# go-distributed/gossip_simulator

Hardware: AMD Instinct MI355X
Metric: gossip messages delivered/sec (node) at N=1e9; rounds-to-coverage parity (higher is better)
Workload: dtype u32; 1 GPU; C5-reference-model: single push-flood broadcast per GPU; n=1000000000, fanout=5, fanin=6, delaylow=10, delayhigh=20, ticks=290, status=quiescent, parallelism=trials1

## Files before the change

gossip_simulator_amd/_lib.py:

```python
from __future__ import annotations

import ctypes as C
import os

PKG_DIR = os.path.dirname(os.path.abspath(__file__))
LIB_PATH = os.environ.get("GS_LIB_PATH") or os.path.join(PKG_DIR, "libgossip_hip.so")
CLI_PATH = os.path.join(PKG_DIR, "bin", "gossip_sim")

GS_OK, GS_EINVAL, GS_ELIVELOCK, GS_EREJECT, GS_ENOMEM, GS_EDEVICE, GS_EOVERFLOW = (
    0, -1, -2, -3, -4, -5, -6)
GS_FLAG_TIMING = 1
GS_FLAG_TICK_ENGINE = 2
GS_FLAG_PP_L2_ONLY = 4
GS_FLAG_PP_DENSE = 8
GS_FLAG_PP_EARLY = 16
GS_FLAG_PP_TOPDOWN = 32
GS_FLAG_PP_BOTTOM = 64
GS_FLAG_PP_ANSWER = 128
GS_MODEL_FLOOD, GS_MODEL_PUSHPULL, GS_MODEL_RUMOR = 0, 1, 2
GS_RUMOR_BLIND, GS_RUMOR_COIN, GS_RUMOR_PULL = 1, 2, 4
GS_RUN_COVERED, GS_RUN_QUIESCENT, GS_RUN_MAX_TICKS, GS_RUN_RUNNING = 0, 1, 2, -1
GS_COMM_ID_BYTES = 128

EXPORTS = (
    "gs_version", "gs_strerror", "gs_create", "gs_destroy", "gs_last_error",
    "gs_load_peers", "gs_load_peers_device", "gs_read_peers", "gs_build_overlay",
    "gs_set_failed", "gs_broadcast_begin", "gs_step", "gs_run", "gs_totals",
    "gs_read_received", "gs_read_crashed", "gs_timing_get", "gs_format_float32",
    "gs_format_float64", "gs_format_duration", "gs_threshold", "gs_philox",
    "gs_set_flags", "gs_reset", "gs_set_stream", "gs_create_multi", "gs_comm_unique_id",
    "gs_create_rank", "gs_shard_info", "gs_trial_results", "gs_set_trial",
    "gs_create_rank_exchange", "gs_shard_timing", "gs_trim", "gs_memory_stats",
    "gs_pp_trials_max_n", "gs_pp_trials_max_n_masked", "gs_read_removed",
    "gs_create_trials", "gs_rumor_trials_max_n",
)


class GossipError(RuntimeError):
    def __init__(self, code: int, msg: str):
        super().__init__(f"{msg} [code {code}]")
        self.code = code


class Params(C.Structure):
    _fields_ = [
        ("n", C.c_uint64),
        ("fanout", C.c_int32),
        ("fanin", C.c_int32),
        ("delay_low", C.c_int32),
        ("delay_high", C.c_int32),
        ("drop_rate", C.c_double),
        ("crash_rate", C.c_double),
        ("seed", C.c_uint64),
        ("trial", C.c_uint32),
        ("device", C.c_int32),
        ("flags", C.c_uint32),
        ("model", C.c_uint32),
        ("trials", C.c_uint32),
        ("rumor_k", C.c_uint32),
        ("rumor_mode", C.c_uint32),
        ("reserved32_", C.c_uint32),
        ("reserved_", C.c_uint64 * 4),
    ]


class TickStats(C.Structure):
    _fields_ = [(f, C.c_uint64) for f in
                ("tick", "fired", "sent", "messages", "received", "crashed", "pending")]


class TrialStats(C.Structure):
    _fields_ = [(f, C.c_uint64) for f in
                ("trial", "tick_99", "tick", "fired", "sent", "messages", "received", "crashed")] + \
        [("status", C.c_int32), ("reserved_", C.c_int32)]


class Window(C.Structure):
    _fields_ = [(f, C.c_uint64) for f in ("tick", "makeups", "breakups")]


class Timing(C.Structure):
    _fields_ = [("deliver_ms", C.c_double), ("resolve_ms", C.c_double),
                ("deliver_launches", C.c_uint64), ("resolve_launches", C.c_uint64),
                ("overlay_ms", C.c_double), ("expand_ms", C.c_double),
                ("part_ms", C.c_double), ("windows", C.c_uint64), ("exact_redos", C.c_uint64),
                ("prep_ms", C.c_double),
                ("pp_early_rounds", C.c_uint64), ("pp_bottom_rounds", C.c_uint64),
                ("pp_answer_rounds", C.c_uint64), ("dd_fallbacks", C.c_uint64), ("pp_rev_part", C.c_uint64),
                ("ov_part_ticks", C.c_uint64), ("ov_sort_ticks", C.c_uint64), ("ov_part_fallbacks", C.c_uint64),
                ("alloc_ms", C.c_double), ("largest_alloc_ms", C.c_double), ("free_ms", C.c_double),
                ("alloc_calls", C.c_uint64), ("alloc_cache_hits", C.c_uint64), ("cached_bytes", C.c_uint64),
                ("coarse_redos", C.c_uint64)]


ALL_GATHER_FN = C.CFUNCTYPE(C.c_int, C.c_void_p, C.c_void_p, C.c_void_p, C.c_size_t)
ALL_REDUCE_FN = C.CFUNCTYPE(C.c_int, C.c_void_p, C.POINTER(C.c_uint64), C.c_size_t)


ALL_TO_ALLV_FN = C.CFUNCTYPE(C.c_int, C.c_void_p, C.c_void_p, C.POINTER(C.c_size_t), C.c_void_p,
                             C.POINTER(C.c_size_t))


class Exchange(C.Structure):
    _fields_ = [("user", C.c_void_p), ("all_gather", ALL_GATHER_FN), ("all_reduce_sum_u64", ALL_REDUCE_FN),
                ("all_to_allv", ALL_TO_ALLV_FN)]


_lib = None


def load():
    global _lib
    if _lib is not None:
        return _lib
    if not os.path.exists(LIB_PATH):
        raise OSError(f"{LIB_PATH} is missing: run `python -c 'import __graft_entry__ as g; g.build()'`")
    L = C.CDLL(LIB_PATH)
    P, vp, sz = C.POINTER, C.c_void_p, C.c_size_t
    ctx = vp
    sig = {
        "gs_version": ([], C.c_int),
        "gs_strerror": ([C.c_int], C.c_char_p),
        "gs_create": ([P(Params), P(vp)], C.c_int),
        "gs_create_trials": ([P(Params), P(vp)], C.c_int),
        "gs_destroy": ([ctx], None),
        "gs_last_error": ([ctx], C.c_char_p),
        "gs_load_peers": ([ctx, vp, vp, C.c_uint32], C.c_int),
        "gs_load_peers_device": ([ctx, vp, vp, C.c_uint32], C.c_int),
        "gs_read_peers": ([ctx, vp, vp, P(C.c_uint32)], C.c_int),
        "gs_build_overlay": ([ctx, C.c_uint64, P(Window), sz, P(sz), P(C.c_uint64)], C.c_int),
        "gs_set_failed": ([ctx, vp, sz], C.c_int),
        "gs_broadcast_begin": ([ctx, C.c_int64], C.c_int),
        "gs_step": ([ctx, C.c_uint32, P(TickStats)], C.c_int),
        "gs_run": ([ctx, C.c_uint32, C.c_uint64, P(TickStats), sz, P(sz), P(C.c_int32)], C.c_int),
        "gs_totals": ([ctx, P(TickStats)], C.c_int),
        "gs_read_received": ([ctx, vp, sz], C.c_int),
        "gs_read_crashed": ([ctx, vp, sz], C.c_int),
        "gs_read_removed": ([ctx, vp, sz], C.c_int),
        "gs_timing_get": ([ctx, P(Timing)], C.c_int),
        "gs_shard_timing": ([ctx, C.c_uint32, P(Timing)], C.c_int),
        "gs_format_float32": ([C.c_float, C.c_char_p, sz], sz),
        "gs_format_float64": ([C.c_double, C.c_char_p, sz], sz),
        "gs_format_duration": ([C.c_int64, C.c_char_p, sz], sz),
        "gs_threshold": ([C.c_double], C.c_int32),
        "gs_philox": ([P(C.c_uint32), P(C.c_uint32), P(C.c_uint32)], None),
        "gs_set_flags": ([ctx, C.c_uint32], C.c_int),
        "gs_reset": ([ctx], C.c_int),
        "gs_set_stream": ([ctx, vp], C.c_int),
        "gs_create_multi": ([P(Params), P(C.c_int), C.c_int, P(vp)], C.c_int),
        "gs_comm_unique_id": ([C.c_char_p], C.c_int),
        "gs_create_rank": ([P(Params), C.c_int, C.c_int, C.c_int, C.c_char_p, P(vp)], C.c_int),
        "gs_create_rank_exchange": ([P(Params), C.c_int, C.c_int, C.c_int, P(Exchange), P(vp)], C.c_int),
        "gs_shard_info": ([ctx, C.c_uint32, P(C.c_uint32), P(C.c_uint64), P(C.c_uint64)], C.c_int),
        "gs_trial_results": ([ctx, P(TrialStats), sz, P(sz)], C.c_int),
        "gs_set_trial": ([ctx, C.c_uint32], C.c_int),
        "gs_trim": ([C.c_int, P(sz)], C.c_int),
        "gs_memory_stats": ([P(Timing)], C.c_int),
        "gs_pp_trials_max_n": ([C.c_int, P(C.c_uint64)], C.c_int),
        "gs_pp_trials_max_n_masked": ([C.c_int, P(C.c_uint64)], C.c_int),
        "gs_rumor_trials_max_n": ([C.c_int, C.c_uint32, P(C.c_uint64)], C.c_int),
    }
    for name, (args, res) in sig.items():
        fn = getattr(L, name)
        fn.argtypes = args
        fn.restype = res
    _lib = L
    return L


def format_float32(x: float) -> str:
    b = C.create_string_buffer(64)
    load().gs_format_float32(x, b, 64)
    return b.value.decode()


def format_float64(x: float) -> str:
    b = C.create_string_buffer(64)
    load().gs_format_float64(x, b, 64)
    return b.value.decode()


def format_duration(ns: int) -> str:
    b = C.create_string_buffer(64)
    load().gs_format_duration(ns, b, 64)
    return b.value.decode("utf-8")


def threshold(rate: float) -> int:
    return int(load().gs_threshold(rate))


def philox(ctr, key):
    c = (C.c_uint32 * 4)(*[int(x) & 0xFFFFFFFF for x in ctr])
    k = (C.c_uint32 * 2)(*[int(x) & 0xFFFFFFFF for x in key])
    o = (C.c_uint32 * 4)()
    load().gs_philox(c, k, o)
    return [int(x) for x in o]
```

gossip_simulator_amd/csrc/gs_api.cpp:

```cpp
#include "gs_ctx.h"

using namespace gs;

namespace {

void fill_devmem(gs_timing* out) {
  DevMemStats d;
  gs_devmem_stats(&d);
  out->alloc_ms = d.alloc_ms;
  out->largest_alloc_ms = d.largest_alloc_ms;
  out->free_ms = d.free_ms;
  out->alloc_calls = d.hip_allocs;
  out->alloc_cache_hits = d.cache_hits;
  out->cached_bytes = d.cached_bytes;
}

int is_failed(gs_ctx* c, uint64_t u, bool* out) {
  *out = false;
  if (!c->failed) return GS_OK;
  unsigned long long w = 0;
  CK(c, hipMemcpyAsync(&w, c->st.crash + u / 64, 8, hipMemcpyDeviceToHost, c->stream));
  CK(c, hipStreamSynchronize(c->stream));
  *out = (w >> (u & 63)) & 1;
  return GS_OK;
}

uint64_t keyed_sender(const gs_ctx* c) {
  return uniform(draw0(c->st.key, K_SENDER, 0, 0, 0), (uint32_t)c->p.n);
}

int read_started(gs_ctx* c, const uint32_t* started, uint32_t* count) {
  if (started) CK(c, hipMemcpyAsync(c->bt.h_tstat, started, (size_t)c->trials * 4, hipMemcpyDeviceToHost, c->stream));
  CK(c, hipStreamSynchronize(c->stream));
  *count = 0;
  for (uint32_t t = 0; t < c->trials; ++t) {
    c->tacc[t].start = started ? c->bt.h_tstat[t] : 1;
    *count += (uint32_t)c->tacc[t].start;
  }
  return GS_OK;
}

int begin_one(gs_ctx* c, uint64_t s, uint32_t* sched) {
  *sched = 0;
  CK(c, hipSetDevice(c->dev));
  if (c->trials > 1) {
    uint32_t* started = c->failed ? c->bt.d_tstat : nullptr;
    CK(c, win_schedule(c->ws, (uint32_t)s, 0, c->trials, (uint32_t)c->p.n, c->stream, started));
    RC(read_started(c, started, sched));
    return GS_OK;
  }
  if (s < c->lo || s >= (c->shard ? c->hi : c->p.n)) return GS_OK;
  const uint64_t u = s - c->lo;
  bool dead = false;
  RC(is_failed(c, u, &dead));
  if (dead) return GS_OK;
  if (c->win) CK(c, win_schedule(c->ws, (uint32_t)u, 0, 1, (uint32_t)c->p.n, c->stream));
  else CK(c, launch_schedule_one(c->st, (uint32_t)u, 0, c->stream));
  CK(c, hipStreamSynchronize(c->stream));
  *sched = 1;
  return GS_OK;
}

int read_bits(gs_ctx* c, int which, uint64_t* words, size_t nwords) {
  const uint64_t Wn = (c->p.n + 63) / 64;
  if (c->group && c->gtrials) {
    if (nwords < Wn * c->trials) return fail(c, GS_EINVAL, "need ceil(n/64) words per trial");
    uint64_t off = 0;
    for (gs_ctx* m : c->gr.mem) {
      if (read_bits(m, which, words + off * Wn, nwords - off * Wn)) return fail(c, GS_EINVAL, m->err);
      off += m->trials;
    }
    return GS_OK;
  }
  if (c->group) {
    std::fill(words, words + Wn, 0ull);
    std::vector<uint64_t> tmp(Wn);
    for (gs_ctx* m : c->gr.mem) {
      if (read_bits(m, which, tmp.data(), Wn)) return fail(c, GS_EINVAL, m->err);
      for (uint64_t i = 0; i < Wn; ++i) words[i] |= tmp[i];
    }
    return GS_OK;
  }
  if (nwords < Wn * c->trials) return fail(c, GS_EINVAL, "need ceil(n/64) words per trial");
  CK(c, hipSetDevice(c->dev));
  const unsigned long long* src = which ? c->st.crash : c->st.recv;
  if (c->trials > 1) {
    CK(c, hipMemcpy2DAsync(words, Wn * 8, src, ((size_t)1 << c->tlog) / 8, Wn * 8, c->trials,
                           hipMemcpyDeviceToHost, c->stream));
  } else if (c->shard) {
    std::fill(words, words + Wn, 0ull);
    CK(c, hipMemcpyAsync(words + c->lo / 64, src, c->st.W * 8, hipMemcpyDeviceToHost, c->stream));
  } else {
    CK(c, hipMemcpyAsync(words, src, c->st.W * 8, hipMemcpyDeviceToHost, c->stream));
  }
  CK(c, hipStreamSynchronize(c->stream));
  return GS_OK;
}

}

extern "C" {

int gs_version(void) { return GS_ABI_VERSION; }

const char* gs_strerror(int code) {
  switch (code) {
    case GS_OK: return "ok";
    case GS_EINVAL: return "invalid argument";
    case GS_ELIVELOCK: return "overlay livelock";
    case GS_EREJECT: return "replacement rejection exhausted";
    case GS_ENOMEM: return "out of memory";
    case GS_EDEVICE: return "HIP device error";
    case GS_EOVERFLOW: return "counter overflow";
    default: return "unknown error";
  }
}

const char* gs_last_error(const gs_ctx* c) {
  if (c) return c->err.c_str();
  return g_create_err.empty() ? "NULL context" : g_create_err.c_str();
}

static int pp_trials_limit(int device, bool masked, uint64_t* n_max) {
  g_create_err.clear();
  if (!n_max) return GS_EINVAL;
  *n_max = 0;
  int ndev = 0;
  std::string why;
  const hipError_t ce = hipGetDeviceCount(&ndev);
  if (ce != hipSuccess) {
    why = std::string("hipGetDeviceCount: ") + hipGetErrorString(ce);
  } else if (device < 0 || device >= ndev) {
    why = "device " + std::to_string(device) + " of " + std::to_string(ndev) + " visible";
  } else {
    uint64_t lim = 0;
    why = ppt_limit_error(device, masked, &lim);
    if (why.empty()) {
      *n_max = masked ? ppt_max_n_masked(lim) : ppt_max_n(lim);
      return GS_OK;
    }
  }
  (void)hipGetLastError();
  fprintf(stderr, "%s: %s\n", masked ? "gs_pp_trials_max_n_masked" : "gs_pp_trials_max_n", why.c_str());
  g_create_err = why;
  return GS_EDEVICE;
}

int gs_pp_trials_max_n(int device, uint64_t* n_max) { return pp_trials_limit(device, false, n_max); }

int gs_pp_trials_max_n_masked(int device, uint64_t* n_max) { return pp_trials_limit(device, true, n_max); }

int gs_create(const gs_params* params, gs_ctx** out) {
  g_create_err.clear();
  if (!out) return GS_EINVAL;
  *out = nullptr;
  return create_one(params, params ? params->device : 0, false, 1, 0, out);
}

int gs_create_trials(const gs_params* params, gs_ctx** out) {
  g_create_err.clear();
  if (!out) return GS_EINVAL;
  *out = nullptr;
  return create_one(params, params ? params->device : 0, false, 1, 0, out, true);
}

int gs_rumor_trials_max_n(int device, uint32_t rumor_mode, uint64_t* n_max) {
  g_create_err.clear();
  if (!n_max) return GS_EINVAL;
  *n_max = 0;
  int ndev = 0;
  int rc = GS_EDEVICE;
  std::string why;
  const hipError_t ce = hipGetDeviceCount(&ndev);
  if (rumor_mode & ~(GS_RUMOR_BLIND | GS_RUMOR_COIN | GS_RUMOR_PULL)) {
    why = "rumor_mode " + std::to_string(rumor_mode) + " has a bit that is none of GS_RUMOR_BLIND, GS_RUMOR_COIN, "
          "GS_RUMOR_PULL";
    rc = GS_EINVAL;
  } else if (ce != hipSuccess) {
    why = std::string("hipGetDeviceCount: ") + hipGetErrorString(ce);
  } else if (device < 0 || device >= ndev) {
    why = "device " + std::to_string(device) + " of " + std::to_string(ndev) + " visible";
  } else {
    uint64_t lim = 0;
    why = rmt_limit_error(device, rumor_mode, &lim);
    if (why.empty()) {
      *n_max = rmt_max_n(rumor_mode, lim);
      return GS_OK;
    }
  }
  (void)hipGetLastError();
  fprintf(stderr, "gs_rumor_trials_max_n: %s\n", why.c_str());
  g_create_err = why;
  return rc;
}

int gs_create_multi(const gs_params* params, const int* devices, int ndev, gs_ctx** out) {
  g_create_err.clear();
  if (!out || !params || !devices || ndev < 1) return GS_EINVAL;
  *out = nullptr;
  return create_multi(params, devices, ndev, out);
}

int gs_comm_unique_id(uint8_t id[GS_COMM_ID_BYTES]) {
  if (!id) return GS_EINVAL;
  const Rccl& r = rccl();
  if (!r.ok) {
    fprintf(stderr, "gs_comm_unique_id: %s\n", r.why.c_str());
    return GS_EDEVICE;
  }
  ncclUniqueId u;
  if (r.get_unique_id(&u) != ncclSuccess) return GS_EDEVICE;
  static_assert(sizeof(ncclUniqueId) == GS_COMM_ID_BYTES, "RCCL unique id size");
  memcpy(id, &u, GS_COMM_ID_BYTES);
  return GS_OK;
}

int gs_create_rank(const gs_params* params, int device, int nranks, int rank, const uint8_t* id, gs_ctx** out) {
  g_create_err.clear();
  if (!out || !params || nranks < 1 || rank < 0 || rank >= nranks) return GS_EINVAL;
  *out = nullptr;
  RC(rumor_refuse(params, "gs_create_rank"));
  const uint32_t T = std::max<uint32_t>(1, params->trials);
  if (T > 1) {
    gs_params mp = *params;
    const uint32_t t0 = (uint32_t)((uint64_t)T * rank / nranks), t1 = (uint32_t)((uint64_t)T * (rank + 1) / nranks);
    if (t1 == t0) {
      fprintf(stderr, "gs_create_rank: %u trials leave rank %d none\n", T, rank);
      return GS_EINVAL;
    }
    mp.trial = params->trial + t0;
    mp.trials = t1 - t0;
    return create_one(&mp, device, false, 1, 0, out);
  }
  if (!id) return GS_EINVAL;
  const Rccl& r = rccl();
  if (!r.ok) {
    fprintf(stderr, "gs_create_rank: %s\n", r.why.c_str());
    return GS_EDEVICE;
  }
  gs_ctx* c = nullptr;
  int rc = create_one(params, device, true, (uint32_t)nranks, (uint32_t)rank, &c);
  if (rc) return rc;
  ncclUniqueId u;
  memcpy(&u, id, GS_COMM_ID_BYTES);
  (void)hipSetDevice(device);
  ncclResult_t nr = r.comm_init_rank(&c->xc.comm, nranks, u, rank);
  if (nr != ncclSuccess) {
    fprintf(stderr, "gs_create_rank: ncclCommInitRank: %s\n", rccl_error((int)nr).c_str());
    c->xc.comm = nullptr;
    destroy_one(c);
    return GS_EDEVICE;
  }
  return finish_rank(c, out);
}

int gs_create_rank_exchange(const gs_params* params, int device, int nranks, int rank, const gs_exchange* ex,
                            gs_ctx** out) {
  g_create_err.clear();
  if (!out || !params || !ex || !ex->all_gather || !ex->all_reduce_sum_u64 || nranks < 1 || rank < 0 ||
      rank >= nranks)
    return GS_EINVAL;
  RC(rumor_refuse(params, "gs_create_rank_exchange"));
  if (params->model == GS_MODEL_FLOOD && std::max<uint32_t>(1, params->trials) == 1 && !ex->all_to_allv) {
    fprintf(stderr, "gs_create_rank_exchange: flood shards need the all_to_allv callback\n");
    return GS_EINVAL;
  }
  *out = nullptr;
  if (std::max<uint32_t>(1, params->trials) > 1) return gs_create_rank(params, device, nranks, rank, nullptr, out);
  gs_ctx* c = nullptr;
  int rc = create_one(params, device, true, (uint32_t)nranks, (uint32_t)rank, &c);
  if (rc) return rc;
  c->xc.hx = *ex;
  c->xc.has_hx = true;
  return finish_rank(c, out);
}

int gs_shard_info(const gs_ctx* c, uint32_t index, uint32_t* nshards, uint64_t* lo, uint64_t* hi) {
  if (!c) return GS_EINVAL;
  const bool sg = c->group && !c->gtrials;
  const uint32_t ns = sg ? (uint32_t)c->gr.mem.size() : c->shard ? c->G : 1u;
  if (nshards) *nshards = ns;
  if (index >= ns) return GS_EINVAL;
  const gs_ctx* s = sg ? c->gr.mem[0] : c;
  uint64_t a = 0, b = c->p.n;
  if (s->shard) {
    a = std::min<uint64_t>(index * s->seg_per, c->p.n);
    b = std::min<uint64_t>(a + s->seg_per, c->p.n);
  }
  if (lo) *lo = a;
  if (hi) *hi = b;
  return GS_OK;
}

void gs_destroy(gs_ctx* c) { destroy_one(c); }

int gs_load_peers(gs_ctx* c, const uint8_t* deg, const uint32_t* ids, uint32_t stride) {
  if (!c || !deg || !ids || stride == 0 || stride > 255) return fail(c, GS_EINVAL, "bad peer table");
  if (c->begun) return fail(c, GS_EINVAL, "peers must be loaded before gs_broadcast_begin");
  if (c->group && c->gtrials) {
    uint64_t off = 0;
    for (gs_ctx* m : c->gr.mem) {
      RC(gs_load_peers(m, deg + off * c->p.n, ids + off * c->p.n * stride, stride) ? fail(c, GS_EINVAL, m->err) : 0);
      off += m->trials;
    }
    c->peers = true;
    return GS_OK;
  }
  if (c->group) {
    for (size_t d = 0; d < c->gr.devs.size(); ++d) {
      std::vector<gs_ctx*> ms = on_device(c, d);
      int rc = upload_table(ms[0], deg, ids, stride);
      if (!rc) rc = seal_rows(ms[0], ms[0]->d_deg, ms[0]->d_ids, c->p.n);
      if (!rc) rc = partition_from(ms[0], ms);
      if (rc) return fail(c, rc, ms[0]->err);
    }
    c->peers = true;
    return GS_OK;
  }
  RC(upload_table(c, deg, ids, stride));
  RC(seal_rows(c, c->d_deg, c->d_ids, table_n(c)));
  if (c->shard) RC(partition_from(c, {c}));
  c->peers = true;
  return GS_OK;
}

int gs_load_peers_device(gs_ctx* c, const void* d_deg, const void* d_ids, uint32_t stride) {
  if (!c || !d_deg || !d_ids || stride < 2 || stride > 255)
    return fail(c, GS_EINVAL, "bad device peer table (stride must be in [2,255])");
  if (c->begun) return fail(c, GS_EINVAL, "peers must be loaded before gs_broadcast_begin");
  if (c->group || c->trials > 1)
    return fail(c, GS_EINVAL, "device tables load into one-device, one-trial contexts");
  CK(c, hipSetDevice(c->dev));
  c->row_slots = 0;
  RC(alloc_table(c, stride));
  const uint64_t n = table_n(c);
  CK(c, hipMemcpyAsync(c->d_deg, d_deg, n, hipMemcpyDeviceToDevice, c->stream));
  CK(c, hipMemcpyAsync(c->d_ids, d_ids, n * stride * 4ull, hipMemcpyDeviceToDevice, c->stream));
  RC(validate_table(c, c->d_deg, c->d_ids, n, c->p.n));
  RC(seal_rows(c, c->d_deg, c->d_ids, n));
  if (c->shard) RC(partition_from(c, {c}));
  c->peers = true;
  return GS_OK;
}

int gs_read_peers(gs_ctx* c, uint8_t* deg, uint32_t* ids, uint32_t* stride_out) {
  if (!c || !c->peers) return fail(c, GS_EINVAL, "no peer table");
  if (c->group && c->gtrials) {
    uint32_t s = 0;
    uint64_t off = 0;
    for (gs_ctx* m : c->gr.mem) {
      if (gs_read_peers(m, deg ? deg + off * c->p.n : nullptr, nullptr, &s)) return fail(c, GS_EINVAL, m->err);
      if (ids && gs_read_peers(m, nullptr, ids + off * c->p.n * s, &s)) return fail(c, GS_EINVAL, m->err);
      off += m->trials;
    }
    if (stride_out) *stride_out = s;
    return GS_OK;
  }
  if (c->group || c->shard)
    return fail(c, GS_EINVAL, "a sharded context keeps only its partition of the table");
  const uint32_t S = c->st.stride, So = c->row_slots && c->row_slots < S ? c->row_slots : S;
  if (stride_out) *stride_out = So;
  CK(c, hipSetDevice(c->dev));
  if (c->trials > 1) {
    const uint64_t np = c->p.n, per = 1ull << c->tlog;
    std::vector<uint8_t> hd(c->ntot);
    std::vector<uint32_t> hi;
    CK(c, hipMemcpyAsync(hd.data(), c->d_deg, c->ntot, hipMemcpyDeviceToHost, c->stream));
    if (ids) {
      hi.resize(c->ntot * S);
      CK(c, hipMemcpyAsync(hi.data(), c->d_ids, c->ntot * S * 4ull, hipMemcpyDeviceToHost, c->stream));
    }
    CK(c, hipStreamSynchronize(c->stream));
    for (uint32_t t = 0; t < c->trials; ++t)
      for (uint64_t v = 0; v < np; ++v) {
        const uint64_t src = t * per + v, dst = t * np + v;
        if (deg) deg[dst] = hd[src];
        if (ids)
          for (uint32_t j = 0; j < So; ++j) {
            const uint32_t x = hi[src * S + j];
            ids[dst * So + j] = x == kEmptyMsg ? x : (x & ((uint32_t)per - 1));
          }
      }
    return GS_OK;
  }
  if (deg) CK(c, hipMemcpyAsync(deg, c->d_deg, c->p.n, hipMemcpyDeviceToHost, c->stream));
  if (ids && So == S) CK(c, hipMemcpyAsync(ids, c->d_ids, c->p.n * S * 4ull, hipMemcpyDeviceToHost, c->stream));
  if (ids && So != S)
    CK(c, hipMemcpy2DAsync(ids, So * 4ull, c->d_ids, S * 4ull, So * 4ull, c->p.n, hipMemcpyDeviceToHost, c->stream));
  CK(c, hipStreamSynchronize(c->stream));
  return GS_OK;
}

int gs_build_overlay(gs_ctx* c, uint64_t max_ticks, gs_window* win, size_t cap, size_t* nwin,
                     uint64_t* final_tick) {
  if (!c) return GS_EINVAL;
  if (c->begun) return fail(c, GS_EINVAL, "overlay must be built before gs_broadcast_begin");
  if (c->group && c->gtrials) {
    std::vector<uint64_t> ft(c->gr.mem.size(), 0);
    std::vector<size_t> nw(c->gr.mem.size(), 0);
    RC(par_members(c, [&](gs_ctx* m, size_t i) {
      return gs_build_overlay(m, max_ticks, i == 0 ? win : nullptr, i == 0 ? cap : 0, &nw[i], &ft[i]);
    }));
    if (nwin) *nwin = nw[0];
    if (final_tick) *final_tick = *std::max_element(ft.begin(), ft.end());
    c->timing.overlay_ms = c->gr.mem[0]->timing.overlay_ms;
    c->peers = true;
    return GS_OK;
  }
  if (c->group) {
    for (size_t d = 0; d < c->gr.devs.size(); ++d) {
      std::vector<gs_ctx*> ms = on_device(c, d);
      int rc = overlay_into(ms[0], max_ticks, d == 0 ? win : nullptr, d == 0 ? cap : 0,
                            d == 0 ? nwin : nullptr, d == 0 ? final_tick : nullptr);
      if (!rc) rc = partition_from(ms[0], ms);
      if (rc) return fail(c, rc, ms[0]->err);
    }
    c->timing.overlay_ms = c->gr.mem[0]->timing.overlay_ms;
    c->peers = true;
    return GS_OK;
  }
  RC(overlay_into(c, max_ticks, win, cap, nwin, final_tick));
  if (c->shard) RC(partition_from(c, {c}));
  c->peers = true;
  return GS_OK;
}

int gs_set_failed(gs_ctx* c, const uint64_t* words, size_t nwords) { return set_failed(c, words, nwords); }


int gs_broadcast_begin(gs_ctx* c, int64_t sender) {
  if (!c) return GS_EINVAL;
  if (c->aborted) return fail(c, GS_EDEVICE, "this rank's exchange failed earlier; the run is over");
  if (!c->peers) return fail(c, GS_EINVAL, "load peers or build the overlay first");
  if (c->begun) return fail(c, GS_EINVAL, "broadcast already begun");
  if (sender >= 0 && (uint64_t)sender >= c->p.n) return fail(c, GS_EINVAL, "sender out of range");
  reset_counters(c);
  if (c->group && c->gtrials) {
    for (gs_ctx* m : c->gr.mem) {
      if (gs_broadcast_begin(m, sender)) return fail(c, GS_EINVAL, m->err);
      c->recv += m->recv;
      c->pending += m->pending;
    }
    c->begun = true;
    return GS_OK;
  }
  const bool batched = c->trials > 1;
  const uint64_t s = sender >= 0 ? (uint64_t)sender : batched ? ~0ull : keyed_sender(c->group ? c->gr.mem[0] : c);
  if (c->ppt) {
    CK(c, hipSetDevice(c->dev));
    uint32_t* started = c->failed ? c->bt.d_tstat : nullptr;
    uint32_t k = 0;
    CK(c, ppt_seed(c->pt, (uint32_t)s, started, c->stream));
    RC(read_started(c, started, &k));
    for (TrialAcc& a : c->tacc) a.recv = a.start;
    c->recv = c->pending = k;
    c->begun = true;
    return GS_OK;
  }
  if (c->rumor) return rumor_begin(c, s);
  if (c->pp && (c->group || c->pp_shard)) return pp_shard_begin(c, s);
  if (c->pp) {
    CK(c, hipSetDevice(c->dev));
    RC(pp_prepare(c));
    const uint64_t n = c->st.n;
    const unsigned long long thr = (c->p.flags & GS_FLAG_PP_EARLY) ? n : (n >> pp_shift());
    RC(pp_seed_ctx(c, c->d_next, (uint32_t)s, thr, pp_bottom_thr(c), pp_answer_thr(c)));
    uint32_t ok = 0;
    CK(c, hipMemcpyAsync(&ok, c->d_flag, 4, hipMemcpyDeviceToHost, c->stream));
    CK(c, hipStreamSynchronize(c->stream));
    c->recv = c->pending = ok;
    c->begun = true;
    return GS_OK;
  }
  unsigned long long scheduled = 0;
  if (c->group) {
    for (gs_ctx* m : c->gr.mem) {
      reset_counters(m);
      uint32_t k = 0;
      if (int rc = begin_one(m, s, &k)) return fail(c, rc, m->err);
      scheduled += k;
      m->begun = true;
    }
  } else {
    uint32_t k = 0;
    RC(begin_one(c, s, &k));
    scheduled = k;
    if (is_rank(c)) RC(rank_sum(c, &scheduled));
  }
  c->pending = scheduled;
  for (TrialAcc& a : c->tacc) a.sched = 0;
  c->begun = true;
  return GS_OK;
}

int gs_set_stream(gs_ctx* c, void* hip_stream) {
  if (!c) return GS_EINVAL;
  if (c->group || is_rank(c)) return fail(c, GS_EINVAL, "multi-device contexts keep their own streams");
  CK(c, hipSetDevice(c->dev));
  CK(c, hipStreamSynchronize(c->stream));
  c->stream = hip_stream ? (hipStream_t)hip_stream : c->own;
  return GS_OK;
}

int gs_memory_stats(gs_timing* out) {
  if (!out) return GS_EINVAL;
  *out = gs_timing{};
  fill_devmem(out);
  return GS_OK;
}

int gs_trim(int device, size_t* released) {
  const size_t b = gs_devmem_trim(device);
  if (released) *released = b;
  return GS_OK;
}

int gs_step(gs_ctx* c, uint32_t ticks, gs_tick_stats* out) {
  if (!c) return GS_EINVAL;
  if (c->aborted) return fail(c, GS_EDEVICE, "this rank's exchange failed earlier; the run is over");
  if (!c->begun) return fail(c, GS_EINVAL, "gs_broadcast_begin first");
  if (c->group && c->gtrials) {
    std::vector<std::vector<gs_tick_stats>> rows(c->gr.mem.size(), std::vector<gs_tick_stats>(ticks));
    RC(par_members(c, [&](gs_ctx* m, size_t i) {
      return gs_step(m, ticks, rows[i].data());
    }));
    std::vector<unsigned long long> s(kStatFields);
    for (uint32_t k = 0; k < ticks; ++k) {
      std::fill(s.begin(), s.end(), 0ull);
      uint64_t pend = 0;
      for (auto& r : rows) {
        s[ST_FIRED] += r[k].fired;
        s[ST_SENT] += r[k].sent;
        s[ST_MSGS] += r[k].messages;
        pend += r[k].pending;
      }
      uint64_t recv = 0, cr = 0;
      for (auto& r : rows) { recv += r[k].received; cr += r[k].crashed; }
      c->t = rows[0][k].tick;
      c->fired += s[ST_FIRED]; c->sent += s[ST_SENT]; c->msgs += s[ST_MSGS];
      c->recv = recv; c->crashed = cr; c->pending = pend;
      if (out) out[k] = gs_tick_stats{c->t, s[ST_FIRED], s[ST_SENT], s[ST_MSGS], recv, cr, pend};
    }
    return GS_OK;
  }
  if (c->rumor) return rumor_step(c, ticks, out, true);
  if (c->pp && (c->group || c->pp_shard)) return pp_shard_step(c, ticks, out);
  if (c->group) return shard_step(c, c->gr.mem, ticks, out);
  if (c->shard) return abort_rank(c, shard_step(c, {c}, ticks, out));
  if (c->ppt) return ppt_step(c, ticks, out);
  return plain_step(c, ticks, out);
}

int gs_run(gs_ctx* c, uint32_t poll, uint64_t max_ticks, gs_tick_stats* out, size_t cap,
           size_t* nout, int32_t* status) {
  if (!c || poll == 0) return fail(c, GS_EINVAL, "poll must be >= 1");
  if (c->group && c->gtrials) {
    std::vector<int32_t> sts(c->gr.mem.size(), 0);
    RC(par_members(c, [&](gs_ctx* m, size_t i) {
      return gs_run(m, poll, max_ticks, nullptr, 0, nullptr, &sts[i]);
    }));
    gs_tick_stats tot{};
    uint64_t recv = 0, cr = 0, t = 0, pend = 0;
    c->fired = c->sent = c->msgs = 0;
    for (gs_ctx* m : c->gr.mem) {
      c->fired += m->fired; c->sent += m->sent; c->msgs += m->msgs;
      recv += m->recv; cr += m->crashed; pend += m->pending; t = std::max(t, m->t);
    }
    c->t = t; c->recv = recv; c->crashed = cr; c->pending = pend;
    tot = gs_tick_stats{t, c->fired, c->sent, c->msgs, recv, cr, pend};
    if (out && cap) out[0] = tot;
    if (nout) *nout = 1;
    if (status) *status = *std::max_element(sts.begin(), sts.end());
    return GS_OK;
  }
  if (c->rumor) return rumor_run(c, poll, max_ticks, out, cap, nout, status);
  size_t k = 0;
  int32_t st = GS_RUN_MAX_TICKS;
  const bool trials = c->trials > 1 && !c->group;
  const bool flood = !c->pp;
  const uint64_t pbase = c->t;
  uint64_t f0 = c->fired, s0 = c->sent, m0 = c->msgs;
  std::function<int(const OnTick&, uint32_t*, bool*)> dd;
  std::vector<gs_ctx*> ms;
  if (!c->pp && !c->gtrials && (c->group || c->shard) && dd_ok(c, shards_of(c))) {
    if (c->aborted) return fail(c, GS_EDEVICE, "this rank's exchange failed earlier; the run is over");
    if (!c->begun) return fail(c, GS_EINVAL, "gs_broadcast_begin first");
    ms = shards_of(c);
    for (gs_ctx* m : ms) {
      CK(m, hipSetDevice(m->dev));
      RC(expand_view(m));
    }
    dd = [&](const OnTick& on_tick, uint32_t* stop, bool* fallback) {
      const int rc = dd_run(c, ms, ~0ull, poll, max_ticks, on_tick, stop, fallback);
      return c->group ? rc : abort_rank(c, rc);
    };
  } else if (async_ok(c)) {
    dd = [&](const OnTick& on_tick, uint32_t* stop, bool* fallback) {
      return run_async(c, ~0ull, poll, max_ticks, on_tick, stop, fallback);
    };
  }
  if (dd) {
    uint32_t stop = 0;
    bool fallback = false;
    RC(dd(
        [&](uint64_t tick, const unsigned long long* row) {
          account_tick(c, tick, row, nullptr);
          if ((tick - pbase) % poll) return;
          if (out && k < cap)
            out[k] = gs_tick_stats{c->t, c->fired - f0, c->sent - s0, c->msgs - m0, c->recv, c->crashed, c->pending};
          ++k;
          f0 = c->fired; s0 = c->sent; m0 = c->msgs;
        },
        &stop, &fallback));
    if (!fallback) {
      st = stop ? (int32_t)stop - 1 : GS_RUN_MAX_TICKS;
      if (c->tacc.size() == 1) snap_trial(c, 0, st);
      if (nout) *nout = k;
      if (status) *status = st;
      return GS_OK;
    }
  }
  std::vector<uint64_t> tr0;
  for (;;) {
    const uint64_t r0 = c->recv;
    if (trials && c->ppt) {
      tr0.resize(c->trials);
      for (uint32_t tr = 0; tr < c->trials; ++tr) tr0[tr] = c->tacc[tr].recv;
    }
    RC(gs_step(c, (uint32_t)(poll - (c->t - pbase) % poll), nullptr));
    if (out && k < cap)
      out[k] = gs_tick_stats{c->t, c->fired - f0, c->sent - s0, c->msgs - m0, c->recv, c->crashed, c->pending};
    ++k;
    f0 = c->fired; s0 = c->sent; m0 = c->msgs;
    if (trials && c->ppt) {
      uint32_t running = 0;
      RC(ppt_poll_stops(c, tr0, max_ticks, &running));
      if (trials_stopped(c, running, &st)) break;
      continue;
    }
    if (trials) {
      uint32_t running = 0;
      for (uint32_t tr = 0; tr < c->trials; ++tr) {
        TrialAcc& a = c->tacc[tr];
        if (a.status != GS_RUN_RUNNING) continue;
        const uint64_t pend = a.start + a.sched - a.fired;
        if (covered(a.recv, c->p.n)) snap_trial(c, tr, GS_RUN_COVERED);
        else if (pend == 0) snap_trial(c, tr, GS_RUN_QUIESCENT);
        else if (c->t >= max_ticks) snap_trial(c, tr, GS_RUN_MAX_TICKS);
        else ++running;
      }
      if (trials_stopped(c, running, &st)) break;
      continue;
    }
    if (covered(c->recv, c->p.n)) { st = GS_RUN_COVERED; break; }
    if (flood && c->pending == 0) { st = GS_RUN_QUIESCENT; break; }
    if (!flood && c->recv == r0) {
      bool stalled = false;
      RC(pp_stalled(c, &stalled));
      if (stalled) { st = GS_RUN_QUIESCENT; break; }
    }
    if (c->t >= max_ticks) { st = GS_RUN_MAX_TICKS; break; }
  }
  if (!trials && c->tacc.size() == 1) snap_trial(c, 0, st);
  if (nout) *nout = k;
  if (status) *status = st;
  return GS_OK;
}

int gs_trial_results(gs_ctx* c, gs_trial_stats* out, size_t cap, size_t* nout) {
  if (!c) return GS_EINVAL;
  size_t k = 0;
  auto one = [&](const gs_ctx* x) {
    for (size_t i = 0; i < x->tacc.size(); ++i, ++k) {
      if (!out || k >= cap) continue;
      const TrialAcc& a = x->tacc[i];
      if (a.status != GS_RUN_RUNNING) {
        out[k] = a.snap;
      } else {
        out[k] = gs_trial_stats{(uint64_t)x->p.trial + i, a.tick99, x->t, a.fired, a.sent, a.msgs, a.recv,
                                a.crash, GS_RUN_RUNNING, 0};
      }
    }
  };
  if (c->group && c->gtrials) for (gs_ctx* m : c->gr.mem) one(m);
  else one(c);
  if (nout) *nout = k;
  return GS_OK;
}

int gs_totals(gs_ctx* c, gs_tick_stats* out) {
  if (!c || !out) return GS_EINVAL;
  *out = gs_tick_stats{c->t, c->fired, c->sent, c->msgs, c->recv, c->crashed, c->pending};
  return GS_OK;
}

int gs_read_received(gs_ctx* c, uint64_t* words, size_t nwords) {
  if (!c || !words || nwords < (c->p.n + 63) / 64) return fail(c, GS_EINVAL, "need ceil(n/64) words");
  return read_bits(c, 0, words, nwords);
}

int gs_read_crashed(gs_ctx* c, uint64_t* words, size_t nwords) {
  if (!c || !words || nwords < (c->p.n + 63) / 64) return fail(c, GS_EINVAL, "need ceil(n/64) words");
  return read_bits(c, 1, words, nwords);
}

int gs_read_removed(gs_ctx* c, uint64_t* words, size_t nwords) {
  if (!c) return GS_EINVAL;
  return rumor_read_removed(c, words, nwords);
}

int gs_timing_get(gs_ctx* c, gs_timing* out) {
  if (!c || !out) return GS_EINVAL;
  *out = c->group ? c->gr.mem[0]->timing : c->timing;
  if (c->group) out->overlay_ms = c->timing.overlay_ms;
  out->pp_early_rounds = out->pp_bottom_rounds = out->pp_answer_rounds = 0;
  gs_ctx* pc = c->group ? c->gr.mem[0] : c;
  if (c->pp && pc->sp.ctl && c->begun) {
    CK(pc, hipSetDevice(pc->dev));
    PPCtl h;
    CK(pc, hipMemcpyAsync(&h, pc->sp.ctl, offsetof(PPCtl, segcnt), hipMemcpyDeviceToHost, pc->stream));
    CK(pc, hipStreamSynchronize(pc->stream));
    out->pp_early_rounds = h.nearly;
    out->pp_bottom_rounds = h.nbottom;
    out->pp_answer_rounds = h.nanswer;
  }
  if (c->pp && c->begun) out->pp_early_rounds += c->rs.rep_rounds;
  fill_devmem(out);
  return GS_OK;
}

int gs_shard_timing(gs_ctx* c, uint32_t index, gs_timing* out) {
  if (!c || !out) return GS_EINVAL;
  if (!c->group) return index == 0 ? gs_timing_get(c, out) : fail(c, GS_EINVAL, "no such shard");
  if (index >= c->gr.mem.size()) return fail(c, GS_EINVAL, "no such shard");
  *out = c->gr.mem[index]->timing;
  fill_devmem(out);
  return GS_OK;
}

int gs_set_trial(gs_ctx* c, uint32_t trial) {
  if (!c) return GS_EINVAL;
  if (c->begun) return fail(c, GS_EINVAL, "gs_reset before gs_set_trial");
  if (c->group) {
    uint32_t t = trial;
    for (gs_ctx* m : c->gr.mem) {
      RC(gs_set_trial(m, c->gtrials ? t : trial) ? fail(c, GS_EINVAL, m->err) : 0);
      t += m->trials;
    }
    c->p.trial = trial;
    c->peers = false;
    return GS_OK;
  }
  c->p.trial = trial;
  c->st.key.trial = trial;
  c->ws.key.trial = trial;
  c->pt.key.trial = trial;
  c->peers = false;
  reset_counters(c);
  return GS_OK;
}

int gs_set_flags(gs_ctx* c, uint32_t flags) {
  if (!c) return GS_EINVAL;
  c->p.flags = flags;
  for (gs_ctx* m : c->gr.mem) m->p.flags = flags;
  return GS_OK;
}

int gs_reset(gs_ctx* c) {
  if (!c) return GS_EINVAL;
  for (gs_ctx* m : c->gr.mem) RC(gs_reset(m) ? fail(c, GS_EDEVICE, m->err) : 0);
  if (!c->group) {
    CK(c, hipSetDevice(c->dev));
    CK(c, hipMemsetAsync(c->d_state, 0, (char*)c->st.stats - (char*)c->d_state, c->stream));
    if (c->d_err) CK(c, hipMemsetAsync(c->d_err, 0, 4, c->stream));
    if (c->d_cnt) CK(c, hipMemsetAsync(c->d_cnt, 0, c->st.n * 4, c->stream));
    if (c->win) CK(c, hipMemsetAsync(c->ws.fcount, 0, c->wn.fcount_bytes, c->stream));
    if (c->failed && !c->pp_shard)
      CK(c, hipMemcpyAsync(c->st.crash, c->d_failed, c->st.W * 8, hipMemcpyDeviceToDevice, c->stream));
    if (c->pp_shard)
      CK(c, hipMemsetAsync(c->st.recv, 0, c->st.W * 8, c->stream));
    CK(c, hipStreamSynchronize(c->stream));
  }
  reset_counters(c);
  c->begun = false;
  return GS_OK;
}

void gs_philox(const uint32_t ctr[4], const uint32_t key[2], uint32_t out[4]) {
  const u32x4 r = philox(ctr[0], ctr[1], ctr[2], ctr[3], key[0], key[1]);
  out[0] = r.x; out[1] = r.y; out[2] = r.z; out[3] = r.w;
}

}
```

gossip_simulator_amd/csrc/gs_ctx.cpp:

```cpp
#include "gs_ctx.h"

namespace gs {

namespace {

uint32_t ring_slots(const gs_params& p) { return p.delay_high > 2 ? (uint32_t)p.delay_high : 2u; }

uint32_t ceil_log2(uint64_t x) {
  uint32_t b = 0;
  while ((1ull << b) < x) ++b;
  return b;
}

int check_params(const gs_params* p, bool rumor_trials, std::string& why) {
  if (!p) { why = "params is NULL"; return GS_EINVAL; }
  if (p->n == 0) { why = "n must be >= 1 (simulator.go:240 panics on rand.Intn(0))"; return GS_EINVAL; }
  if (p->n > 0x7FFFFFFFull) { why = "n must be < 2^31"; return GS_EINVAL; }
  if (p->delay_high <= p->delay_low) {
    why = "delayhigh must exceed delaylow (simulator.go:167 panics on rand.Intn(<=0))";
    return GS_EINVAL;
  }
  if (p->fanout < 0 || p->fanin < 0 || p->fanout > 255 || p->fanin > 255) {
    why = "fanout/fanin must be in [0, 255]";
    return GS_EINVAL;
  }
  if (ring_slots(*p) > 4096) { why = "delayhigh must be <= 4096"; return GS_EINVAL; }
  if (p->model > GS_MODEL_RUMOR) {
    why = "model must be GS_MODEL_FLOOD, GS_MODEL_PUSHPULL or GS_MODEL_RUMOR";
    return GS_EINVAL;
  }
  if (p->model == GS_MODEL_RUMOR && (p->rumor_k < 1 || p->rumor_k > 255)) {
    why = "GS_MODEL_RUMOR needs 1 <= rumor_k <= 255, not " + std::to_string(p->rumor_k);
    return GS_EINVAL;
  }
  if (p->model == GS_MODEL_RUMOR && (p->rumor_mode & ~(GS_RUMOR_BLIND | GS_RUMOR_COIN | GS_RUMOR_PULL))) {
    why = "GS_MODEL_RUMOR: rumor_mode " + std::to_string(p->rumor_mode) +
          " has a bit that is none of GS_RUMOR_BLIND, GS_RUMOR_COIN, GS_RUMOR_PULL";
    return GS_EINVAL;
  }
  if (p->model == GS_MODEL_RUMOR && p->trials > 1 && !rumor_trials) {
    why = "GS_MODEL_RUMOR with trials > 1: the rumor model runs one trial per context (gs_create_trials makes a batch)";
    return GS_EINVAL;
  }
  if (p->trials > 1 && ((uint64_t)p->trials << std::max<uint32_t>(kFineLog, ceil_log2(p->n))) > 0x7FFFFFFFull) {
    why = "trials x 2^ceil(log2 n) must be < 2^31 (batch fewer trials per context)";
    return GS_EINVAL;
  }
  return GS_OK;
}

bool alloc_trial_rows(gs_ctx* c, size_t tb, size_t cb) {
  return dev_malloc((void**)&c->bt.d_tstat, tb) == hipSuccess &&
         hipHostMalloc((void**)&c->bt.h_tstat, tb) == hipSuccess && grow(c->bt.chk, cb);
}

void release_trials(gs_ctx* c) {
  if (c->bt.d_tstat) (void)dev_free(c->bt.d_tstat);
  if (c->bt.h_tstat) (void)hipHostFree(c->bt.h_tstat);
  release(c->bt.chk);
}

int alloc_window(gs_ctx* c) {
  const DevState& s = c->st;
  WinState& w = c->ws;
  w.n = s.n;
  w.W = s.W;
  w.nfine = (uint32_t)((s.n + kFineNodes - 1) >> kFineLog);
  w.ncoarse = (w.nfine + 255) / 256;
  w.R = s.R;
  w.delay_low = s.delay_low;
  w.delay_span = s.delay_span;
  w.kd = s.kd;
  w.kc = s.kc;
  w.key = s.key;
  w.base = (uint32_t)c->lo;
  w.tlog = c->tlog;
  w.tmask = c->tlog >= 32 ? ~0u : (1u << c->tlog) - 1;
  w.tnodes = c->trials > 1 && c->tlog <= kCoarseShift && !c->shard ? (uint32_t)c->p.n : 0u;
  w.G = c->G;
  w.rank = c->rank;
  w.seg_per = (uint32_t)c->seg_per;
  w.csub = kCoarseSub;
  w.noxcd = getenv("GS_PART2_NOXCD") ? 1u : 0u;
  {
    const char* xp = getenv("GS_XPAIR");
    w.nopair = xp && atoi(xp) == 0 ? 1u : 0u;
  }
  w.ccap_end = nullptr;
  w.csrc = nullptr;
  if (c->shard) {
    w.owner = 1;
    w.obins = 256 / c->G;
    w.oseg_q = (uint32_t)(c->seg_per >> kFineLog);
    w.oseg_magic = 0xFFFFFFFFu / w.oseg_q;
    if (dev_malloc(&c->wn.d_rtab, kRtabWords * 8) != hipSuccess ||
        hipHostMalloc((void**)&c->wn.h_rtab, kRtabWords * 8) != hipSuccess)
      return fail(c, GS_ENOMEM, "cannot allocate the shard's receive layout");
  }
  auto al = [](size_t b) { return (b + 255) & ~(size_t)255; };
  const size_t units = (size_t)kMaxWindow * w.nfine + 1;
  const size_t b_fc = al((size_t)w.R * w.nfine * 4), b_units = al(units * 8),
               b_small = al(kRegions * 8) * 2 + al((kRegions + 1) * 8) + al((kRegions + 1) * 4) + al(kMaxWindow * 8),
               b_fhist = al(((size_t)w.ncoarse * 256 + 1) * 8), b_fbase = al(((size_t)w.nfine + 1) * 8),
               b_ffill = al((size_t)w.nfine * 8),
               b_sst = al((size_t)kStatShards * kMaxWindow * kStatFields * 8),
               b_rlcnt = al((size_t)w.nfine * 4),
               b_tsum = al((size_t)w.ncoarse * kMaxWindow * 8) + al(((size_t)w.ncoarse + 1) * 8);
  const size_t total = b_fc + 2 * b_units + b_small + b_fhist + b_fbase + b_ffill + b_sst + b_rlcnt + b_tsum;
  if (dev_malloc(&c->wn.d_win, total) != hipSuccess)
    return fail(c, GS_ENOMEM, "cannot allocate window-engine buffers");
  const size_t flist = (size_t)w.R * w.nfine * kFineNodes * 2;
  if (dev_malloc(&c->wn.d_flist, flist) != hipSuccess)
    return fail(c, GS_ENOMEM, "cannot allocate " + std::to_string(flist >> 20) + " MiB of fire lists");
  char* q = (char*)c->wn.d_win;
  w.fcount = (uint32_t*)q; q += b_fc;
  w.usize = (unsigned long long*)q; q += b_units;
  w.unit_off = (unsigned long long*)q; q += b_units;
  w.chist = (unsigned long long*)q; q += al(kRegions * 8);
  w.cfill = (unsigned long long*)q; q += al(kRegions * 8);
  w.ccap = (unsigned long long*)q; q += al((kRegions + 1) * 8);
  w.tprefix = (uint32_t*)q; q += al((kRegions + 1) * 4);
  w.tfires = (unsigned long long*)q;
  q = (char*)c->wn.d_win + b_fc + 2 * b_units + b_small;
  w.fhist = (unsigned long long*)q; q += b_fhist;
  w.fstart = (unsigned long long*)q; q += b_fbase;
  w.ffill = (unsigned long long*)q; q += b_ffill;
  w.sstats = (unsigned long long*)q; q += b_sst;
  w.rlcnt = (uint32_t*)q; q += b_rlcnt;
  w.tsum = (unsigned long long*)q; q += al((size_t)w.ncoarse * kMaxWindow * 8);
  w.toff = (unsigned long long*)q; q += al(((size_t)w.ncoarse + 1) * 8);
  if (dev_malloc(&c->wn.d_rlmsg, (size_t)w.nfine * kRolledCap * 4) != hipSuccess)
    return fail(c, GS_ENOMEM, "cannot allocate the rolled-receipt lists");
  w.rlmsg = (uint32_t*)c->wn.d_rlmsg;
  w.dbg = nullptr;
  if (getenv("GS_STAMPS") && dev_malloc(&w.dbg, kDbgWords * 8) == hipSuccess)
    (void)hipMemset(w.dbg, 0, kDbgWords * 8);
  w.flist = (uint16_t*)c->wn.d_flist;
  c->wn.fcount_bytes = (size_t)w.R * w.nfine * 4;
  if (hipMemsetAsync(c->wn.d_win, 0, total, c->stream) != hipSuccess)
    return fail(c, GS_EDEVICE, "memset of window buffers failed");
  c->wn.misc_words = std::max<size_t>(4096, (size_t)c->G * kMaxWindow + 64);
  if (hipHostMalloc((void**)&c->wn.h_cap, (kRegions + 1) * 8) != hipSuccess ||
      hipHostMalloc((void**)&c->wn.h_misc, c->wn.misc_words * 8) != hipSuccess ||
      hipHostMalloc((void**)&c->wn.h_err, 64) != hipSuccess)
    return fail(c, GS_ENOMEM, "cannot allocate pinned window buffers");
  if (c->trials > 1) {
    if (!alloc_trial_rows(c, (size_t)c->trials * kMaxWindow * kTStatFields * 4, 0))
      return fail(c, GS_ENOMEM, "cannot allocate per-trial counters");
    w.tstat = c->bt.d_tstat;
  }
  return GS_OK;
}

void release_window(gs_ctx* c) {
  WinEngine& e = c->wn;
  for (void* p : {e.d_win, e.d_flist, e.d_rlmsg, (void*)e.d_rtab, (void*)c->ws.dbg})
    if (p) (void)dev_free(p);
  for (Buf* b : {&e.gmap, &e.cmsg, &e.fmsg, &e.tmp}) release(*b);
  for (void* p : {(void*)e.h_cap, (void*)e.h_misc, (void*)e.h_err, (void*)e.h_rtab})
    if (p) (void)hipHostFree(p);
}

int ctx_setup(gs_ctx* c, const gs_params* params, int device, bool shard, uint32_t G, uint32_t rank,
              std::string& why) {
  c->p = *params;
  c->p.device = device;
  c->dev = device;
  int ndev = 0;
  if (hipGetDeviceCount(&ndev) != hipSuccess || ndev <= 0) {
    why = "no HIP device visible (libgossip_hip needs an MI355X)";
    return GS_EDEVICE;
  }
  if (c->dev < 0 || c->dev >= ndev) {
    why = "device " + std::to_string(c->dev) + " out of range (" + std::to_string(ndev) + " visible)";
    return GS_EDEVICE;
  }
  hipDeviceProp_t prop;
  if (hipSetDevice(c->dev) != hipSuccess || hipGetDeviceProperties(&prop, c->dev) != hipSuccess ||
      strncmp(prop.gcnArchName, "gfx950", 6) != 0) {
    why = "device " + std::to_string(c->dev) + " is not gfx950";
    return GS_EDEVICE;
  }
  if (hipStreamCreateWithFlags(&c->own, hipStreamNonBlocking) != hipSuccess) {
    why = "cannot create a stream";
    return GS_EDEVICE;
  }
  c->stream = c->own;
  DevState& s = c->st;
  const uint32_t stride0 = (uint32_t)std::max(c->p.fanout, c->p.fanin);
  c->pp = c->p.model == GS_MODEL_PUSHPULL;
  c->rumor = c->p.model == GS_MODEL_RUMOR;
  c->pp_l2_only = (c->p.flags & GS_FLAG_PP_L2_ONLY) != 0;
  c->trials = std::max<uint32_t>(1, c->p.trials);
  c->ntot = c->p.n;
  if (c->trials > 1) {
    c->tlog = std::max<uint32_t>(kFineLog, ceil_log2(c->p.n));
    c->ntot = (uint64_t)c->trials << c->tlog;
  }
  c->shard = shard;
  c->G = G;
  c->rank = rank;
  if (shard && c->rumor) {
    why = "GS_MODEL_RUMOR runs on one device: no node-range shards";
    return GS_EINVAL;
  }
  if (shard) {
    if (c->pp && !pp_rslot_packed(stride0)) {
      why = "push-pull node-range shards need rows of at most 16 slots (bottom-up rounds)";
      return GS_EINVAL;
    }
    c->seg_per = (((c->p.n + G - 1) / G) + kFineNodes - 1) & ~(uint64_t)(kFineNodes - 1);
    if ((uint64_t)(G - 1) * c->seg_per >= c->p.n) {
      why = "n = " + std::to_string(c->p.n) + " is too small for " + std::to_string(G) +
            " shards of whole 16384-node buckets";
      return GS_EINVAL;
    }
    c->pp_shard = c->pp;
    c->rs.segw = c->seg_per / 64;
    c->lo = rank * c->seg_per;
    c->hi = std::min<uint64_t>(c->lo + c->seg_per, c->p.n);
    c->ntot = c->hi - c->lo;
  }
  s.lo = 0;
  s.hi = (uint32_t)c->ntot;
  s.n = c->ntot;
  s.W = (s.n + 63) / 64;
  s.C = (uint32_t)((s.n + (1ull << kChunkNodesLog) - 1) >> kChunkNodesLog);
  s.CS = (s.C + kShards - 1) / kShards;
  s.chunk_lo = 0;
  s.chunk_hi = s.C;
  s.sharded = 0;
  s.R = ring_slots(c->p);
  s.delay_low = c->p.delay_low;
  s.delay_span = (uint32_t)(c->p.delay_high - c->p.delay_low);
  s.kd = gs_threshold(c->p.drop_rate);
  s.kc = gs_threshold(c->p.crash_rate);
  s.key = Key{(uint32_t)c->p.seed, (uint32_t)(c->p.seed >> 32), c->p.trial};
  c->win = !c->pp && !c->rumor && s.R <= kWinMaxRing && !(c->p.flags & GS_FLAG_TICK_ENGINE) && stride0 <= kWinMaxStride &&
           s.n <= (1ull << (kCoarseShift + 8));
  if (((c->trials > 1 && !c->ppt && !c->rmt) || (shard && !c->pp)) && !c->win) {
    why = "batched trials and node-range shards run on the window engine (delayhigh <= 256, "
          "fanout/fanin <= 32, no GS_FLAG_TICK_ENGINE, at most 2^30 nodes per context or shard)";
    return GS_EINVAL;
  }
  static_assert(kSrcShift + 8 == 64, "8-bit source index in the receive layout");
  if (shard && !c->pp && (G > 255 || ((c->seg_per + (1ull << kCoarseShift) - 1) >> kCoarseShift) > 256 / G)) {
    why = "flood node-range shards: each of the G <= 255 shards' ranges must fit 256 / G bins of 2^22 nodes "
          "(n up to about 2^30)";
    return GS_EINVAL;
  }
  auto al = [](size_t b) { return (b + 255) & ~(size_t)255; };
  const bool tick = !c->win && !c->pp && !c->rumor;
  const size_t b_sum = c->pp && !c->ppt ? al(pp_summary_total_words(s.W) * 8) : 0;
  const size_t b_next = (c->pp && !c->ppt) || (c->rumor && !c->rmt) ? al(s.W * 8) + b_sum : 0;
  const size_t b_bits = al(s.W * 8), b_ring = tick ? al((size_t)s.R * s.W * 8) : 0,
               b_cflag = tick ? al((size_t)s.R * s.C * 4) : 0,
               b_clist = tick ? al((size_t)s.R * kShards * s.CS * 4) : 0,
               b_ccount = tick ? al((size_t)s.R * kShards * kCounterStride * 4) : 0,
               b_stats = al((size_t)kStatSlots * kStatFields * 8);
  const size_t b_roll = c->win ? b_bits : 0;
  const size_t total = 2 * b_bits + b_roll + b_next + b_ring + b_cflag + b_clist + b_ccount + b_stats + 256;
  c->state_bytes = total;
  if (dev_malloc(&c->d_state, total) != hipSuccess) {
    why = "cannot allocate " + std::to_string(total) + " bytes of device state";
    return GS_ENOMEM;
  }
  char* q = (char*)c->d_state;
  s.recv = (unsigned long long*)q; q += b_bits;
  s.crash = (unsigned long long*)q; q += b_bits;
  s.rollw = b_roll ? (uint32_t*)q : nullptr; q += b_roll;
  c->d_next = b_next ? (unsigned long long*)q : nullptr;
  c->d_ppsum = b_sum ? (unsigned long long*)(q + al(s.W * 8)) : nullptr;
  q += b_next;
  s.ring = (unsigned long long*)q; q += b_ring;
  s.cflag = (uint32_t*)q; q += b_cflag;
  s.clist = (uint32_t*)q; q += b_clist;
  s.ccount = (uint32_t*)q; q += b_ccount;
  s.stats = (unsigned long long*)q; q += b_stats;
  c->d_err = (uint32_t*)q;
  c->d_flag = c->d_err + 1;
  s.err = c->d_err;
  s.grecv = s.recv;
  s.gcrash = s.crash;
  s.gbase = 0;
  if (tick && s.kc > 0 && dev_malloc(&c->d_cnt, s.n * 4) != hipSuccess) {
    why = "cannot allocate arrival counters";
    return GS_ENOMEM;
  }
  s.cnt = c->d_cnt;
  if (c->win) {
    int rc = alloc_window(c);
    if (rc) { why = c->err; return rc; }
  }
  if (c->rumor) {
    int rc = rumor_alloc(c);
    if (rc) { why = c->err; return rc; }
  }
  if (c->ppt) {
    const size_t tb = (size_t)c->trials * kMaxWindow * kTStatFields * 4;
    const size_t cb = (((size_t)c->trials + 3) & ~(size_t)3) + (size_t)c->trials * 4;
    if (!alloc_trial_rows(c, tb, cb)) {
      why = "cannot allocate the per-trial counters";
      return GS_ENOMEM;
    }
    PptState& pt = c->pt;
    pt.recv = s.recv;
    pt.tstat = c->bt.d_tstat;
    pt.n = (uint32_t)c->p.n;
    pt.trials = c->trials;
    pt.tlog = c->tlog;
    pt.kd = s.kd;
    pt.key = s.key;
  }
  if (c->rmt && !alloc_trial_rows(c, (size_t)c->trials * kMaxWindow * kTStatFields * 4, 0)) {
    why = "cannot allocate the per-trial counters";
    return GS_ENOMEM;
  }
  c->tacc.assign(c->trials, TrialAcc{});
  c->async_off = getenv("GS_SYNC_WINDOWS") != nullptr;
  c->winlog = getenv("GS_WINLOG") != nullptr;
  if (hipMemsetAsync(c->d_state, 0, total, c->stream) != hipSuccess ||
      (c->d_cnt && hipMemsetAsync(c->d_cnt, 0, s.n * 4, c->stream) != hipSuccess) ||
      hipHostMalloc((void**)&c->h_stats, (size_t)kStatSlots * kStatFields * 8) != hipSuccess ||
      hipStreamSynchronize(c->stream) != hipSuccess) {
    why = "device initialisation failed";
    return GS_EDEVICE;
  }
  return GS_OK;
}

void release_state(gs_ctx* c) {
  for (void* p : {c->d_state, (void*)c->d_cnt, (void*)c->d_failed})
    if (p) (void)dev_free(p);
  if (c->h_stats) (void)hipHostFree(c->h_stats);
}

int check_ppt_n(const gs_params* p, int device, std::string& why, PptPlan* pl) {
  *pl = PptPlan{};
  if (p->trials <= 1 || p->model != GS_MODEL_PUSHPULL) return GS_OK;
  int ndev = 0;
  uint64_t lim = 0;
  const bool asked = hipGetDeviceCount(&ndev) == hipSuccess && device >= 0 && device < ndev &&
                     ppt_lds_limit(device, false, &lim) == hipSuccess;
  if (!asked) {
    (void)hipGetLastError();
    why = "batched push-pull trials need n within the device's LDS per workgroup (gs_pp_trials_max_n), and HIP "
          "device " + std::to_string(device) + " is not visible: n = " + std::to_string(p->n) + " is not accepted";
    return GS_EINVAL;
  }
  const PptPlan plan = ppt_plan(p->n, lim);
  if (!plan.fits) {
    why = "batched push-pull trials keep a trial's informed set in one workgroup's LDS: n must be <= " +
          std::to_string(ppt_max_n(lim)) + " on this device (gs_pp_trials_max_n), not " + std::to_string(p->n);
    return GS_EINVAL;
  }
  if (plan.lds_bytes > 65536 && ppt_prepare(device, false, (uint32_t)plan.lds_bytes) != hipSuccess) {
    why = "cannot raise the trial-resident kernel's dynamic LDS limit";
    return GS_EDEVICE;
  }
  *pl = plan;
  return GS_OK;
}

void attach_pp_sets(gs_ctx* c, unsigned long long* ig, unsigned long long* fg, unsigned long long* gn) {
  c->rs.d_ig = ig;
  c->rs.d_fg = fg;
  c->rs.d_gn = gn;
  DevState& s = c->st;
  s.grecv = ig;
  s.gcrash = fg;
  s.gbase = c->lo;
  s.recv = ig + (size_t)c->rank * c->rs.segw;
  s.crash = fg + (size_t)c->rank * c->rs.segw;
}

int alloc_pp_sets(gs_ctx* c, uint64_t words, unsigned long long** ig, unsigned long long** fg,
                  unsigned long long** gn) {
  for (unsigned long long** q : {ig, fg, gn}) {
    if (!q) continue;
    *q = nullptr;
    if (dev_malloc(q, words * 8) != hipSuccess)
      return fail(c, GS_ENOMEM, "cannot allocate the replicated informed / failed sets");
    CK(c, hipMemsetAsync(*q, 0, words * 8, c->stream));
  }
  CK(c, hipStreamSynchronize(c->stream));
  return GS_OK;
}

void release_sets(gs_ctx* c) {
  if (!c->rs.own_ig) return;
  for (unsigned long long* q : {c->rs.d_ig, c->rs.d_fg, c->rs.d_gn, c->rs.d_gst})
    if (q) (void)dev_free(q);
}

int make_replica(const gs_params* params, int dev, unsigned long long* ig, unsigned long long* fg, gs_ctx** out) {
  *out = nullptr;
  if (getenv("GS_PP_NO_REPLICA")) return GS_OK;
  gs_params rp = *params;
  rp.trials = 1;
  gs_ctx* r = nullptr;
  RC(create_one(&rp, dev, false, 1, 0, &r));
  r->st.recv = r->st.grecv = ig;
  r->st.crash = r->st.gcrash = fg;
  r->st.gbase = 0;
  *out = r;
  return GS_OK;
}

void print_stamps(gs_ctx* c) {
  if (!c->ws.dbg) return;
  unsigned long long h[kDbgWords];
  if (hipMemcpy(h, c->ws.dbg, sizeof h, hipMemcpyDeviceToHost) == hipSuccess && h[kXStamp0]) {
    const double r = 1e-3 / h[kXStamp0];
    fprintf(stderr, "[stamps] k_expand: %llu rounds (wave 0), mean kcycles per round: lookup %.2f rows %.2f "
            "draws %.2f scan+scatter %.2f barrier %.2f writeout %.2f\n", h[kXStamp0], h[kXStamp0 + 1] * r,
            h[kXStamp0 + 2] * r, h[kXStamp0 + 3] * r, h[kXStamp0 + 4] * r, h[kXStamp0 + 5] * r, h[kXStamp0 + 6] * r);
  }
  if (hipMemcpy(h, c->ws.dbg, sizeof h, hipMemcpyDeviceToHost) == hipSuccess)
    for (int cls = 0; cls < 2; ++cls) {
      const unsigned long long* d = h + cls * kStampPhases;
      if (!d[0]) continue;
      fprintf(stderr, "[stamps] k_resolve %s: %llu buckets, mean kcycles per bucket per phase:",
              cls ? "M>=1024" : "M<1024", d[0]);
      for (uint32_t i = 1; i < kStampPhases; ++i) fprintf(stderr, " %.2f", d[i] * 1e-3 / d[0]);
      fprintf(stderr, "\n");
    }
}

void release_group(gs_ctx* g) {
  Group& r = g->gr;
  for (size_t i = 0; i < r.devs.size(); ++i) {
    (void)hipSetDevice(r.devs[i]);
    if (i < r.buf.size()) release(r.buf[i]);
    for (auto* sets : {&r.ig, &r.fg, &r.gn})
      if (i < sets->size() && (*sets)[i]) (void)dev_free((*sets)[i]);
  }
  for (hipEvent_t e : r.ev_c) (void)hipEventDestroy(e);
  for (hipEvent_t e : r.ev_x) (void)hipEventDestroy(e);
  for (gs_ctx* rep : r.reps) destroy_one(rep);
  if (!r.devs.empty()) (void)hipSetDevice(r.devs[0]);
}

void release_exchange(gs_ctx* c) {
  Exchange& x = c->xc;
  if (x.d_gcounts) (void)dev_free(x.d_gcounts);
  if (x.d_glay) (void)dev_free(x.d_glay);
  if (x.h_glay) (void)hipHostFree(x.h_glay);
  release(x.xsend);
  release(x.xrecv);
  if (x.h_xbuf) (void)hipHostFree(x.h_xbuf);
}

}

int finish_rank(gs_ctx* c, gs_ctx** out) {
  (void)hipSetDevice(c->dev);
  if (dev_malloc(&c->xc.d_gcounts, (size_t)c->G * kMaxWindow * 8 + (size_t)kMaxWindow * 8) != hipSuccess ||
      (!c->pp_shard && (dev_malloc(&c->xc.d_glay, (size_t)c->G * (kRegions + 1) * 8) != hipSuccess ||
                        hipHostMalloc((void**)&c->xc.h_glay, (size_t)c->G * (kRegions + 1) * 8) != hipSuccess))) {
    destroy_one(c);
    return GS_ENOMEM;
  }
  if (c->pp_shard) {
    unsigned long long *ig = nullptr, *fg = nullptr, *gn = nullptr, *gst = nullptr;
    if (alloc_pp_sets(c, (uint64_t)c->G * c->rs.segw, &ig, &fg, &gn) ||
        alloc_pp_sets(c, (uint64_t)c->G * c->rs.segw, &gst, nullptr, nullptr)) {
      fprintf(stderr, "gs_create_rank: %s\n", c->err.c_str());
      for (unsigned long long* q : {ig, fg, gn, gst})
        if (q) (void)dev_free(q);
      destroy_one(c);
      return GS_ENOMEM;
    }
    c->rs.own_ig = true;
    c->rs.d_gst = gst;
    attach_pp_sets(c, ig, fg, gn);
    if (make_replica(&c->p, c->dev, ig, fg, &c->rs.rep)) {
      destroy_one(c);
      return GS_ENOMEM;
    }
    c->rs.own_rep = c->rs.rep != nullptr;
  }
  *out = c;
  return GS_OK;
}

int create_multi(const gs_params* params, const int* devices, int ndev, gs_ctx** out) {
  RC(rumor_refuse(params, "gs_create_multi"));
  gs_ctx* g = new gs_ctx();
  g->group = true;
  g->p = *params;
  g->dev = devices[0];
  g->trials = std::max<uint32_t>(1, params->trials);
  g->gtrials = g->trials > 1;
  if (g->gtrials && (uint32_t)ndev > g->trials) ndev = (int)g->trials;
  for (int i = 0; i < ndev; ++i) {
    gs_params mp = *params;
    gs_ctx* m = nullptr;
    int rc;
    if (g->gtrials) {
      const uint32_t t0 = (uint32_t)((uint64_t)g->trials * i / ndev), t1 = (uint32_t)((uint64_t)g->trials * (i + 1) / ndev);
      mp.trial = params->trial + t0;
      mp.trials = t1 - t0;
      rc = create_one(&mp, devices[i], false, 1, 0, &m);
    } else {
      rc = create_one(&mp, devices[i], true, (uint32_t)ndev, (uint32_t)i, &m);
    }
    if (rc) {
      destroy_one(g);
      return rc;
    }
    g->gr.mem.push_back(m);
    auto it = std::find(g->gr.devs.begin(), g->gr.devs.end(), devices[i]);
    if (it == g->gr.devs.end()) {
      g->gr.devs.push_back(devices[i]);
      g->gr.dev_of.push_back((int)g->gr.devs.size() - 1);
    } else {
      g->gr.dev_of.push_back((int)(it - g->gr.devs.begin()));
    }
  }
  g->gr.buf.resize(g->gr.devs.size());
  g->pp = params->model == GS_MODEL_PUSHPULL;
  if (g->pp && !g->gtrials) {
    g->gr.ig.assign(g->gr.devs.size(), nullptr);
    g->gr.fg.assign(g->gr.devs.size(), nullptr);
    g->gr.gn.assign(g->gr.devs.size(), nullptr);
    for (size_t d = 0; d < g->gr.devs.size(); ++d) {
      std::vector<gs_ctx*> ms;
      for (size_t i = 0; i < g->gr.mem.size(); ++i)
        if ((size_t)g->gr.dev_of[i] == d) ms.push_back(g->gr.mem[i]);
      (void)hipSetDevice(g->gr.devs[d]);
      if (alloc_pp_sets(ms[0], (uint64_t)g->gr.mem.size() * ms[0]->rs.segw, &g->gr.ig[d], &g->gr.fg[d], &g->gr.gn[d])) {
        fprintf(stderr, "gs_create_multi: %s\n", ms[0]->err.c_str());
        destroy_one(g);
        return GS_ENOMEM;
      }
      for (gs_ctx* m : ms) attach_pp_sets(m, g->gr.ig[d], g->gr.fg[d], g->gr.gn[d]);
      gs_ctx* r = nullptr;
      if (make_replica(params, g->gr.devs[d], g->gr.ig[d], g->gr.fg[d], &r)) {
        destroy_one(g);
        return GS_ENOMEM;
      }
      g->gr.reps.push_back(r);
      for (gs_ctx* m : ms) m->rs.rep = r;
    }
  }
  for (size_t i = 0; i < g->gr.mem.size(); ++i) {
    hipEvent_t e;
    (void)hipSetDevice(g->gr.mem[i]->dev);
    if (hipEventCreateWithFlags(&e, hipEventDisableTiming) != hipSuccess) {
      destroy_one(g);
      return GS_EDEVICE;
    }
    g->gr.ev_c.push_back(e);
  }
  for (size_t d = 0; d < g->gr.devs.size(); ++d) {
    hipEvent_t e;
    (void)hipSetDevice(g->gr.devs[d]);
    if (hipEventCreateWithFlags(&e, hipEventDisableTiming) != hipSuccess) {
      destroy_one(g);
      return GS_EDEVICE;
    }
    g->gr.ev_x.push_back(e);
  }
  g->tacc.assign(g->gtrials ? 0 : 1, TrialAcc{});
  *out = g;
  return GS_OK;
}

void refresh_state(gs_ctx* c) {
  DevState& s = c->st;
  s.deg = c->d_deg;
  s.ids = c->d_ids;
  if (c->win) refresh_window(c);
  if (c->ppt) {
    c->pt.deg = c->d_deg;
    c->pt.ids = c->d_ids;
    c->pt.stride = s.stride;
  }
}

bool covered(uint64_t recv, uint64_t n) {
  volatile float a = (float)recv, b = (float)n;
  volatile float pct = a / b;
  return pct >= 0.99f;
}

void reset_counters(gs_ctx* c) {
  c->t = c->fired = c->sent = c->msgs = c->recv = c->crashed = c->pending = 0;
  for (TrialAcc& a : c->tacc) a = TrialAcc{};
}

void account_tick(gs_ctx* c, uint64_t tick, const unsigned long long* s, gs_tick_stats* o) {
  c->t = tick;
  c->fired += s[ST_FIRED];
  c->sent += s[ST_SENT];
  c->msgs += s[ST_MSGS];
  c->recv += s[ST_RECV];
  c->crashed += s[ST_CRASH];
  c->pending = c->pp ? c->recv : c->pending + s[ST_SCHED] - s[ST_FIRED];
  if (c->tacc.size() == 1 && c->trials == 1) {
    TrialAcc& a = c->tacc[0];
    a.fired = c->fired; a.sent = c->sent; a.msgs = c->msgs; a.recv = c->recv; a.crash = c->crashed;
    if (!a.tick99 && covered(a.recv, c->p.n)) a.tick99 = tick;
  }
  if (o) *o = gs_tick_stats{c->t, s[ST_FIRED], s[ST_SENT], s[ST_MSGS], c->recv, c->crashed, c->pending};
}

void account_members(gs_ctx* acc, const std::vector<gs_ctx*>& ms, uint64_t t0, uint32_t batch, gs_tick_stats* out) {
  for (uint32_t i = 0; i < batch; ++i) {
    const size_t row = (size_t)((t0 + i) % kStatSlots) * kStatFields;
    unsigned long long sum[kStatFields] = {0};
    for (uint32_t f = 0; f < kStatFields; ++f)
      for (gs_ctx* m : ms) sum[f] += m->h_stats[row + f];
    account_tick(acc, t0 + i, sum, out ? &out[i] : nullptr);
  }
}

std::string ppt_limit_error(int device, bool masked, uint64_t* lim) {
  const char* where = "";
  const hipError_t e = ppt_lds_limit(device, masked, lim, &where);
  if (e == hipSuccess) return std::string();
  return std::string(where) + " on device " + std::to_string(device) + ": " + hipGetErrorString(e) + " (hipError_t " +
         std::to_string((int)e) + ")";
}

int ppt_masked_plan(const gs_ctx* c, PptPlan* plan, std::string& why) {
  uint64_t lim = 0;
  why = ppt_limit_error(c->dev, true, &lim);
  if (!why.empty()) return GS_EDEVICE;
  *plan = ppt_plan_masked(c->p.n, lim);
  if (plan->fits) return GS_OK;
  why = "batched push-pull trials with failure masks keep a third bitset in one workgroup's LDS: n must be <= " +
        std::to_string(ppt_max_n_masked(lim)) + " on device " + std::to_string(c->dev) +
        " (gs_pp_trials_max_n_masked), not " + std::to_string(c->p.n);
  return GS_EINVAL;
}

thread_local std::string g_create_err;

int create_one(const gs_params* params, int device, bool shard, uint32_t G, uint32_t rank, gs_ctx** out,
               bool rumor_trials) {
  std::string why;
  PptPlan pl;
  RmtPlan rpl;
  int rc = check_params(params, rumor_trials, why);
  if (!rc) rc = check_ppt_n(params, device, why, &pl);
  if (!rc) rc = check_rmt_n(params, device, why, &rpl);
  if (!rc) {
    gs_ctx* c = new gs_ctx();
    if (rpl.block) {
      c->rmt = true;
      c->rplan = rpl;
    }
    if (pl.block) {
      c->ppt = true;
      c->pt.block = pl.block;
      c->pt.lds_bytes = (uint32_t)pl.lds_bytes;
    }
    rc = ctx_setup(c, params, device, shard, G, rank, why);
    if (!rc) {
      *out = c;
      return GS_OK;
    }
    destroy_one(c);
  }
  fprintf(stderr, "gs_create: %s\n", why.c_str());
  g_create_err = why;
  return rc;
}

void destroy_one(gs_ctx* c) {
  if (!c) return;
  for (gs_ctx* m : c->gr.mem) destroy_one(m);
  if (c->rs.own_rep) destroy_one(c->rs.rep);
  (void)hipSetDevice(c->dev);
  if (c->stream) (void)hipStreamSynchronize(c->stream);
  if (c->xc.comm && rccl().ok) (void)rccl().comm_destroy(c->xc.comm);
  print_stamps(c);
  release_group(c);
  for (hipEvent_t e : c->ev) (void)hipEventDestroy(e);
  overlay_free(&c->ovw, c->stream);
  release_sets(c);
  release_exchange(c);
  release_table(c);
  release_state(c);
  release_window(c);
  release_trials(c);
  release_sparse(c);
  release_rumor(c);
  release_async(c);
  release_dd(c);
  if (c->own) (void)hipStreamDestroy(c->own);
  delete c;
}

}
```

gossip_simulator_amd/csrc/gs_ctx.h:

```cpp
#pragma once
#include <hip/hip_runtime.h>

#include <algorithm>
#include <chrono>
#include <cstdio>
#include <cstdlib>
#include <cstring>
#include <functional>
#include <string>
#include <thread>
#include <vector>

#include "gossip.h"
#include "gs_comm.h"
#include "gs_internal.h"
#include "gs_ppt_plan.h"
#include "gs_rmt_plan.h"

namespace gs {

struct Buf {
  void* p = nullptr;
  size_t bytes = 0;
};

struct TrialAcc {
  uint64_t fired = 0, sent = 0, msgs = 0, recv = 0, crash = 0, sched = 0, tick99 = 0;
  uint64_t start = 1;
  int32_t status = GS_RUN_RUNNING;
  gs_trial_stats snap{};
};

struct WinEngine {
  void* d_win = nullptr;
  void* d_flist = nullptr;
  void* d_rlmsg = nullptr;
  size_t fcount_bytes = 0;
  Buf gmap, cmsg, fmsg, tmp;
  unsigned long long* h_cap = nullptr;
  unsigned long long* h_misc = nullptr;
  size_t misc_words = 0;
  uint32_t* h_err = nullptr;
  unsigned long long* d_rtab = nullptr;
  unsigned long long* h_rtab = nullptr;
};

struct AsyncWin {
  WinCtl* d_ctl = nullptr;
  unsigned long long* d_stage = nullptr;
  unsigned long long* h_stage = nullptr;
  std::vector<hipEvent_t> wev;
};

struct DdWin {
  void* mem = nullptr;
  unsigned long long* gcnt = nullptr;
  unsigned long long* glay = nullptr;
  unsigned long long* wstat = nullptr;
  WinCtl* ctl = nullptr;
  void** ptrs = nullptr;
  void** h_ptrs = nullptr;
  WinState* wsm = nullptr;
  unsigned long long* h_lay = nullptr;
};

struct PpSparseBufs {
  Buf rend, rsrc, rslot, ilist, fmask, scan, ctlb;
  Buf rfail;
  Buf dset, dcnt;
  Buf rend16;
  bool rend16_ok = false;
  uint64_t rev_ver = ~0ull, fm_tver = ~0ull, fm_fver = ~0ull;
  uint64_t cl_tver = ~0ull, cl_fver = ~0ull;
  unsigned long long cl_counts[2] = {0, 0};
};

struct RumorBufs {
  Buf list[2], hot, served, vain, miss, ctlb, removed, tri;
  std::vector<uint32_t> hotn;
  uint32_t cur = 0;
  uint32_t grid = 0;
  RumorCtl* h_ctl = nullptr;
};

struct TrialRows {
  uint32_t* d_tstat = nullptr;
  uint32_t* h_tstat = nullptr;
  Buf chk;
};

struct Exchange {
  uint64_t rtotal = 0;
  Buf xsend, xrecv;
  unsigned long long* d_gcounts = nullptr;
  unsigned long long* d_glay = nullptr;
  unsigned long long* h_glay = nullptr;
  ncclComm_t comm = nullptr;
  gs_exchange hx{};
  bool has_hx = false;
  char* h_xbuf = nullptr;
  size_t h_xbytes = 0;
};

struct PpSets {
  bool own_ig = false;
  unsigned long long* d_ig = nullptr;
  unsigned long long* d_fg = nullptr;
  unsigned long long* d_gn = nullptr;
  unsigned long long* d_gst = nullptr;
  bool pp_answer = false;
  bool pp_gn_ok = false;
  uint64_t segw = 0;
  gs_ctx* rep = nullptr;
  bool own_rep = false;
  bool rep_live = false;
  uint32_t rep_rounds = 0;
};

struct Group {
  std::vector<gs_ctx*> mem;
  std::vector<int> devs;
  std::vector<int> dev_of;
  std::vector<Buf> buf;
  std::vector<hipEvent_t> ev_c, ev_x;
  std::vector<unsigned long long*> ig, fg, gn;
  std::vector<gs_ctx*> reps;
};

}

struct gs_ctx {
  gs_params p{};
  int dev = 0;
  hipStream_t stream = nullptr;
  hipStream_t own = nullptr;
  std::string err;
  gs::DevState st{};
  uint8_t* d_deg = nullptr;
  uint32_t* d_ids = nullptr;
  uint32_t tab_stride = 0;
  uint32_t* d_pk = nullptr;
  size_t pk_bytes = 0;
  uint64_t pk_ver = ~0ull;
  uint32_t row_slots = 0;
  void* d_state = nullptr;
  uint32_t* d_cnt = nullptr;
  uint32_t* d_err = nullptr;
  unsigned long long* d_failed = nullptr;
  size_t state_bytes = 0;
  unsigned long long* h_stats = nullptr;
  bool peers = false, begun = false, failed = false;
  uint64_t t = 0, fired = 0, sent = 0, msgs = 0, recv = 0, crashed = 0, pending = 0;
  std::vector<hipEvent_t> ev;
  gs_timing timing{};
  bool pp = false, pp_l2_only = false;
  unsigned long long* d_next = nullptr;
  unsigned long long* d_ppsum = nullptr;
  uint32_t* d_flag = nullptr;
  uint64_t table_ver = 0, fail_ver = 0;
  gs::PPSparse sp{};
  gs::PpSparseBufs sr;
  bool rumor = false;
  gs::RumorBufs rm;
  bool rmt = false;
  gs::RmtPlan rplan{};
  bool win = false;
  gs::WinState ws{};
  gs::WinEngine wn;
  gs::AsyncWin aw;
  bool async_off = false;
  bool winlog = false;
  uint32_t trials = 1, tlog = 32;
  uint64_t ntot = 0;
  std::vector<gs::TrialAcc> tacc;
  gs::TrialRows bt;
  bool ppt = false;
  gs::PptState pt{};
  bool shard = false;
  uint32_t G = 1, rank = 0;
  uint64_t lo = 0, hi = 0, seg_per = 0;
  gs::WinState wr{};
  gs::Exchange xc;
  bool pp_shard = false;
  bool aborted = false;
  gs::PpSets rs;
  bool group = false, gtrials = false;
  gs::Group gr;
  gs::OverlayWork ovw;
  gs::DdWin dd;
};

#define CK(c, expr)                                                                   \
  do {                                                                                \
    hipError_t e_ = (expr);                                                           \
    if (e_ != hipSuccess)                                                             \
      return fail((c), GS_EDEVICE, std::string(#expr) + ": " + hipGetErrorString(e_)); \
  } while (0)

#define NCK(c, expr)                                                                  \
  do {                                                                                \
    ncclResult_t r_ = (expr);                                                         \
    if (r_ != ncclSuccess)                                                            \
      return fail((c), GS_EDEVICE, std::string(#expr) + ": " + rccl_error((int)r_));  \
  } while (0)

#define RC(expr)              \
  do {                        \
    int rc_ = (expr);         \
    if (rc_) return rc_;      \
  } while (0)

namespace gs {

inline int fail(gs_ctx* c, int code, const std::string& msg) {
  if (c) c->err = msg;
  return code;
}

inline bool grow(Buf& b, size_t bytes) {
  if (b.bytes >= bytes) return true;
  const size_t nb = std::max(bytes, b.bytes + b.bytes / 4);
  if (b.p) (void)dev_free(b.p);
  b.p = nullptr;
  b.bytes = 0;
  if (dev_malloc(&b.p, nb) != hipSuccess) return false;
  b.bytes = nb;
  return true;
}

inline void release(Buf& b) {
  if (b.p) (void)dev_free(b.p);
  b = Buf{};
}

inline bool is_rank(const gs_ctx* c) { return c->xc.comm != nullptr || c->xc.has_hx; }

inline std::vector<gs_ctx*> shards_of(gs_ctx* c) { return c->group ? c->gr.mem : std::vector<gs_ctx*>{c}; }

template <class F>
int par_members(gs_ctx* g, F f) {
  std::vector<int> rcs(g->gr.mem.size(), 0);
  std::vector<std::thread> th;
  for (size_t i = 0; i < g->gr.mem.size(); ++i)
    th.emplace_back([&, i] {
      (void)hipSetDevice(g->gr.mem[i]->dev);
      rcs[i] = f(g->gr.mem[i], i);
    });
  for (auto& t : th) t.join();
  for (size_t i = 0; i < rcs.size(); ++i)
    if (rcs[i]) return fail(g, rcs[i], "member " + std::to_string(i) + ": " + g->gr.mem[i]->err);
  return GS_OK;
}

struct StatSpans {
  size_t off[2], words[2];
  int n;
};
inline StatSpans stat_spans(uint64_t t0, uint32_t batch) {
  const uint32_t i0 = (uint32_t)(t0 % kStatSlots), first = std::min<uint32_t>(batch, kStatSlots - i0);
  return StatSpans{{(size_t)i0 * kStatFields, 0}, {(size_t)first * kStatFields, (size_t)(batch - first) * kStatFields},
                   first < batch ? 2 : 1};
}

using OnTick = std::function<void(uint64_t tick, const unsigned long long* row)>;
constexpr uint32_t kSlots = 4;

extern thread_local std::string g_create_err;
int create_one(const gs_params* params, int device, bool shard, uint32_t G, uint32_t rank, gs_ctx** out,
               bool rumor_trials = false);
int create_multi(const gs_params* params, const int* devices, int ndev, gs_ctx** out);
int finish_rank(gs_ctx* c, gs_ctx** out);
void destroy_one(gs_ctx* c);
std::string ppt_limit_error(int device, bool masked, uint64_t* lim);
int ppt_masked_plan(const gs_ctx* c, PptPlan* plan, std::string& why);
void refresh_state(gs_ctx* c);
void reset_counters(gs_ctx* c);
void account_tick(gs_ctx* c, uint64_t tick, const unsigned long long* s, gs_tick_stats* o);
bool covered(uint64_t recv, uint64_t n);
void account_members(gs_ctx* acc, const std::vector<gs_ctx*>& ms, uint64_t t0, uint32_t batch, gs_tick_stats* out);

uint64_t table_n(const gs_ctx* c);
int alloc_table(gs_ctx* c, uint32_t stride);
void release_table(gs_ctx* c);
int validate_table(gs_ctx* c, const uint8_t* deg, const uint32_t* ids, uint64_t n, uint64_t bound);
int seal_rows(gs_ctx* c, const uint8_t* deg, uint32_t* ids, uint64_t n);
int expand_view(gs_ctx* c);
int upload_table(gs_ctx* c, const uint8_t* deg, const uint32_t* ids, uint32_t stride);
int partition_from(gs_ctx* leader, const std::vector<gs_ctx*>& ms);
std::vector<gs_ctx*> on_device(gs_ctx* g, size_t d);
int overlay_into(gs_ctx* c, uint64_t max_ticks, gs_window* win, size_t cap, size_t* nwin, uint64_t* final_tick);
int set_failed(gs_ctx* c, const uint64_t* words, size_t nwords);

void refresh_window(gs_ctx* c);
bool async_ok(const gs_ctx* c);
uint64_t cover_threshold(uint64_t n);
int alloc_stage(gs_ctx* c);
void release_async(gs_ctx* c);
int run_async(gs_ctx* c, uint64_t tend, uint32_t poll, uint64_t max_ticks, const OnTick& on_tick, uint32_t* stop,
              bool* fallback);
OnTick step_sink(gs_ctx* acc, gs_tick_stats* out, uint32_t* k);
int plain_step(gs_ctx* c, uint32_t ticks, gs_tick_stats* out);

bool grow_pinned(gs_ctx* c, size_t bytes);
int x_all_gather(gs_ctx* c, void* dbuf, size_t bytes);
int x_all_reduce(gs_ctx* c, unsigned long long* dbuf, size_t count);
int abort_rank(gs_ctx* c, int rc);
int rank_sum(gs_ctx* c, unsigned long long* v);
bool dd_ok(const gs_ctx* acc, const std::vector<gs_ctx*>& ms);
void release_dd(gs_ctx* c);
int dd_run(gs_ctx* acc, const std::vector<gs_ctx*>& ms, uint64_t tend, uint32_t poll, uint64_t max_ticks,
           const OnTick& on_tick, uint32_t* stop, bool* fallback);
int shard_step(gs_ctx* acc, const std::vector<gs_ctx*>& ms, uint32_t ticks, gs_tick_stats* out);

int pp_seed_ctx(gs_ctx* c, unsigned long long* next, uint32_t node, unsigned long long thr, unsigned long long bthr,
                unsigned long long athr);
int pp_prepare(gs_ctx* c);
void release_sparse(gs_ctx* c);
uint32_t pp_shift();
unsigned long long pp_bottom_thr(const gs_ctx* c);
unsigned long long pp_answer_thr(const gs_ctx* c);
int pp_shard_begin(gs_ctx* acc, uint64_t sender);
int pp_shard_step(gs_ctx* acc, uint32_t ticks, gs_tick_stats* out);
int pp_stalled(gs_ctx* c, bool* stalled);
void account_trials(gs_ctx* c, uint64_t t0, uint32_t nt, unsigned long long* sums = nullptr);
int ppt_step(gs_ctx* c, uint32_t ticks, gs_tick_stats* out);
int ppt_poll_stops(gs_ctx* c, const std::vector<uint64_t>& r0, uint64_t max_ticks, uint32_t* running);
void snap_trial(gs_ctx* c, uint32_t tr, int32_t status);
bool trials_stopped(const gs_ctx* c, uint32_t running, int32_t* st);

int rumor_refuse(const gs_params* params, const char* what);
int rumor_alloc(gs_ctx* c);
void release_rumor(gs_ctx* c);
int rumor_begin(gs_ctx* c, uint64_t sender);
int rumor_step(gs_ctx* c, uint32_t ticks, gs_tick_stats* out, bool every_tick_polls);
int rumor_run(gs_ctx* c, uint32_t poll, uint64_t max_ticks, gs_tick_stats* out, size_t cap, size_t* nout,
              int32_t* status);
int rumor_read_removed(gs_ctx* c, uint64_t* words, size_t nwords);
std::string rmt_limit_error(int device, uint32_t mode, uint64_t* lim);
int check_rmt_n(const gs_params* p, int device, std::string& why, RmtPlan* pl);

}
```

gossip_simulator_amd/csrc/gs_internal.h:

```cpp
#pragma once
#include <stdint.h>
#include <hip/hip_runtime.h>

#include <algorithm>
#include <vector>

#include "gs_devmem.h"
#include "gs_rng.h"

namespace gs {

inline uint32_t grid_for(uint64_t items, uint32_t per_block, uint32_t cap) {
  return (uint32_t)std::min<uint64_t>((items + per_block - 1) / per_block, cap);
}

constexpr uint32_t kWave = 64;
constexpr uint32_t kChunkNodesLog = 12;
constexpr uint32_t kChunkWords = 64;
constexpr uint32_t kShards = 32;
constexpr uint32_t kCounterStride = 16;
constexpr uint32_t kStatFields = 8;
constexpr uint32_t kStatSlots = 4096;
constexpr uint32_t kListCap = 1024;
constexpr uint32_t kTickBlock = 256;
constexpr uint32_t kTickGridMax = 2048;

enum Stat : uint32_t {
  ST_FIRED = 0, ST_SENT = 1, ST_MSGS = 2, ST_RECV = 3, ST_CRASH = 4, ST_SCHED = 5,
  ST_ERR = 6, ST_RSVD = 7
};

enum Mode : int {
  MODE_FLOOD = 0,
  MODE_COUNT = 1,
  MODE_RESOLVE = 2
};

struct DevState {
  const uint8_t* deg;
  const uint32_t* ids;
  unsigned long long* recv;
  unsigned long long* crash;
  uint32_t* rollw;
  uint32_t* cnt;
  unsigned long long* ring;
  uint32_t* cflag;
  uint32_t* clist;
  uint32_t* ccount;
  unsigned long long* stats;
  uint32_t* err;
  unsigned long long* grecv;
  unsigned long long* gcrash;
  uint64_t gbase;
  uint64_t n, W;
  uint32_t C, CS, R, stride;
  uint32_t stride_magic;
  int32_t delay_low;
  uint32_t delay_span;
  int32_t kd, kc;
  int32_t check_crashed;
  int32_t sharded;
  uint32_t lo, hi;
  uint32_t chunk_lo, chunk_hi;
  Key key;
};

constexpr uint32_t kFineLog = 14;
constexpr uint32_t kFineNodes = 1u << kFineLog;
constexpr uint32_t kCoarseShift = kFineLog + 8;
constexpr uint32_t kMaxWindow = 16;
constexpr uint32_t kCoarseSub = 8;
constexpr uint32_t kRegions = 256 * kCoarseSub;
constexpr uint32_t kWinMaxRing = 256;
constexpr uint32_t kWinMaxStride = 32;
constexpr uint32_t kEmptyMsg = 0xFFFFFFFFu;
constexpr uint32_t kSrcShift = 56;
constexpr unsigned long long kSrcMask = (1ull << kSrcShift) - 1;
#ifndef GS_PART_TILE
#define GS_PART_TILE 16384
#endif
constexpr uint32_t kPartTile = GS_PART_TILE;
constexpr uint32_t kRolledCap = 1024;
constexpr uint32_t kBitTicks = 10;
constexpr uint32_t kXRoundNodes = 2048;
constexpr uint32_t kWinSlotsPerBucket = 1u << 16;

struct WinCtl {
  uint32_t t, L, tnext, tend;
  uint32_t poll, pbase, stop, lmax;
  unsigned long long Tn, T;
  unsigned long long recv, crashed, pending, cover, max_ticks;
  unsigned long long cmsg_cap, fmsg_cap;
  unsigned long long xs_cap, xr_cap;
};
constexpr uint32_t kStageWords = 8 + 16 * 8;

struct WinState {
  const uint8_t* deg;
  const uint32_t* ids;
  unsigned long long* recv;
  unsigned long long* crash;
  uint32_t* rollw;
  uint32_t* rlmsg;
  uint32_t* rlcnt;
  unsigned long long* stats;
  uint32_t* err;
  uint32_t* fcount;
  uint16_t* flist;
  unsigned long long* usize;
  unsigned long long* unit_off;
  unsigned long long* tfires;
  uint32_t* gmap;
  const uint32_t* pk;
  uint32_t noxcd;
  uint32_t nopair;
  uint32_t* cmsg;
  uint32_t* fmsg;
  unsigned long long* chist;
  unsigned long long* ccap;
  const unsigned long long* ccap_end;
  unsigned long long* cfill;
  uint32_t* tprefix;
  unsigned long long* fhist;
  unsigned long long* fstart;
  unsigned long long* ffill;
  unsigned long long* tsum;
  unsigned long long* toff;
  unsigned long long* sstats;
  unsigned long long* dbg;
  uint32_t* tstat;
  uint32_t tofs;
  WinCtl* ctl;
  unsigned long long* stage;
  uint32_t lstride;
  uint32_t slots;
  uint32_t csub;
  const uint32_t* const* csrc;
  uint32_t owner;
  uint32_t obins;
  uint32_t oseg_q, oseg_magic;
  uint32_t abort_on_err;
  uint32_t G, rank;
  uint32_t seg_per;
  uint32_t dd;
  uint32_t guard;
  uint32_t solo;
  unsigned long long* gcnt;
  unsigned long long* glay;
  unsigned long long* wstat;
  uint64_t nglob;
  uint64_t n, W;
  uint32_t nfine, ncoarse, R, stride, stride_magic;
  int32_t delay_low;
  uint32_t delay_span;
  int32_t kd, kc;
  uint32_t base;
  uint32_t tlog, tmask;
  uint32_t tnodes;
  Key key;
};
constexpr uint32_t kStatShards = 32;
constexpr uint32_t kStampPhases = 10;
constexpr uint32_t kXStamp0 = 2 * kStampPhases;
constexpr uint32_t kDbgWords = kXStamp0 + 8;
enum TStat : uint32_t { TS_FIRED = 0, TS_SENT = 1, TS_DEAD = 2, TS_RECV = 3, TS_CRASH = 4, TS_HOT = 5 };
constexpr uint32_t kTStatFields = 8;

__host__ __device__ __forceinline__ void node_key(uint32_t tlog, uint32_t tmask, const Key& key,
                                                  uint64_t g, uint32_t kind, uint32_t& node,
                                                  uint32_t& c3) {
  node = (uint32_t)(g & tmask);
  c3 = ctr3(kind, key.trial + (uint32_t)(g >> tlog));
}

constexpr uint32_t kErrArrivals = 4;
constexpr uint32_t kErrCoarse = 8;
constexpr uint32_t kErrFine = 16;
constexpr uint32_t kErrAbort = 32;
constexpr uint32_t kErrNoMem = 64;
constexpr uint32_t kDDRow = kRegions + 4;
constexpr uint32_t kDDWStat = kMaxWindow * kStatFields + 8;
constexpr size_t kRtabWords = 4 * (kRegions + 1) + 260;
constexpr size_t kRtabTotal = kRtabWords - 1;

hipError_t win_units(const WinState& w, uint32_t t0, uint32_t L, hipStream_t s);
hipError_t win_cut(const WinState& w, unsigned long long budget, hipStream_t s);
hipError_t win_unitscan(const WinState& w, hipStream_t s);
hipError_t win_close(const WinState& w, uint32_t slot, hipStream_t s);
hipError_t win_scan_units(const WinState& w, uint32_t L, void* tmp, size_t& tmp_bytes, hipStream_t s);
hipError_t win_groupmap(const WinState& w, uint32_t L, hipStream_t s);
hipError_t win_expand(const WinState& w, uint32_t t0, uint32_t L, uint64_t Tn, int mode,
                      hipStream_t s);
uint32_t win_expand_geometry(const WinState& w, uint64_t Tn, uint32_t* per_round, uint32_t* bsz,
                             uint32_t* npt);
hipError_t win_plan(const WinState& w, bool exact, hipStream_t s);
hipError_t win_scan_fine(const WinState& w, void* tmp, size_t& tmp_bytes, hipStream_t s);
hipError_t win_part2(const WinState& w, uint64_t T, bool scatter, hipStream_t s);
hipError_t win_resolve(const WinState& w, uint32_t t0, uint32_t L, hipStream_t s);
hipError_t win_pack_rows(const uint32_t* ids, uint64_t n, uint32_t* pk, hipStream_t s);
hipError_t win_seal_rows(const uint8_t* deg, uint32_t* ids, uint64_t n, uint32_t stride,
                         hipStream_t s);
hipError_t win_stats_reduce(const WinState& w, uint32_t t0, uint32_t L, hipStream_t s);
hipError_t win_consume_sh(const WinState& w, uint32_t t0, uint32_t L, hipStream_t s);
hipError_t win_rtab(const WinState& w, unsigned long long* rtab, const unsigned long long* const* ccaps,
                    const uint32_t* const* src, uint32_t nsrc, uint32_t travels, hipStream_t s);
hipError_t win_fine_redo(const WinState& w, uint64_t T, hipStream_t s);
hipError_t win_stats_dd(const WinState& w, uint32_t slot, hipStream_t s);
struct WinGroup {
  const WinState* ws;
  const WinState* wr;
  const WinState* wg;
  uint32_t M;
  uint32_t nfine_max;
  uint32_t ncoarse_max;
  uint32_t slots_max;
};
hipError_t win_units_g(const WinGroup& g, uint32_t L, hipStream_t s);
hipError_t win_cut_g(const WinGroup& g, unsigned long long budget, hipStream_t s);
hipError_t win_unitscan_g(const WinGroup& g, hipStream_t s);
hipError_t win_rtab_g(const WinGroup& g, const unsigned long long* const* ccaps, const uint32_t* const* src,
                      uint32_t nsrc, hipStream_t s);
hipError_t win_recv_g(const WinGroup& g, uint64_t T, hipStream_t s);
hipError_t win_stats_dd_g(const WinGroup& g, uint32_t slot, hipStream_t s);
hipError_t win_expand_g(const WinGroup& g, uint32_t L, hipStream_t s);
hipError_t win_resolve_g(const WinGroup& g, uint32_t L, hipStream_t s);
hipError_t win_close_dd(const WinState& w, const unsigned long long* const* wstats, WinCtl* const* ctls,
                        uint32_t n, uint32_t slot, hipStream_t s);
hipError_t win_pack(const WinState& w, const unsigned long long* poff, uint32_t nreg, uint32_t* out, hipStream_t s);
hipError_t win_schedule(const WinState& w, uint32_t node, uint32_t tick, uint32_t trials, uint32_t n,
                        hipStream_t s, uint32_t* started = nullptr);

inline uint64_t pp_summary_words(uint64_t W) { return (W + 63) / 64; }
inline uint64_t pp_summary2_words(uint64_t W) { return (pp_summary_words(W) + 63) / 64; }
inline uint64_t pp_summary_total_words(uint64_t W) { return 2 * pp_summary_words(W) + 2 * pp_summary2_words(W); }
enum PPMode : uint32_t { PP_DENSE = 0, PP_EARLY = 1, PP_BOTTOM = 2, PP_ANSWER = 3 };
__host__ __device__ inline bool pp_rslot_packed(uint32_t stride) { return stride <= 16; }
constexpr uint32_t kPPSegs = 256;
struct PPCtl {
  unsigned long long ninf;
  unsigned long long thr;
  unsigned long long bthr;
  unsigned long long athr;
  unsigned long long ncallers;
  unsigned long long nlive0;
  unsigned long long seg_cap;
  uint32_t nseg;
  uint32_t mode;
  uint32_t early_ok;
  uint32_t ovf;
  uint32_t nearly, nbottom;
  uint32_t nanswer, pad_;
  unsigned long long segcnt[kPPSegs];
  unsigned long long seglen[kPPSegs];
  unsigned long long segpre[kPPSegs + 1];
};
struct PPSparse {
  PPCtl* ctl;
  uint32_t* ilist;
  const unsigned long long* rend;
  const uint16_t* rend16;
  const unsigned long long* rbase;
  const uint32_t* rsrc;
  const uint8_t* rslot;
  const uint8_t* fmask;
  const unsigned long long* fany;
  const uint32_t* rfail;
  uint32_t* dset;
  unsigned long long* dcnt;
  uint64_t dcap, ccap, fcap;
  uint32_t nodeg;
  uint32_t pullfirst;
  uint32_t word_maxi;
  uint32_t word_maxu;
  uint32_t words;
};
constexpr uint32_t kPPDLists = 512;
constexpr uint32_t kPPDRegions = 2048;
hipError_t pp_round(const DevState& s, unsigned long long* next, unsigned long long* sum, uint32_t t,
                    bool l2_only, const PPSparse& sp, hipStream_t st);
hipError_t pp_live_edges(const DevState& s, uint32_t* out, hipStream_t st);
hipError_t pp_commit(const DevState& s, const unsigned long long* next, uint32_t t, const PPSparse& sp,
                     hipStream_t st);
hipError_t pp_seed(const DevState& s, unsigned long long* next, uint32_t node, uint32_t* flag,
                   const PPSparse& sp, unsigned long long thr, unsigned long long bthr, unsigned long long athr,
                   const unsigned long long* callers, hipStream_t st);
size_t pp_rev_scan_bytes(uint64_t n);
hipError_t pp_rev_build(const DevState& s, unsigned long long* rend, uint32_t* rsrc, uint8_t* rslot, void* tmp,
                        size_t tmp_bytes, hipStream_t st);
hipError_t pp_rev_compact(const unsigned long long* rend, uint64_t n, uint16_t* rend16, unsigned long long* rbase,
                          uint32_t* ovf, hipStream_t st);
hipError_t pp_rev_build_part(const DevState& s, unsigned long long* rend, uint32_t* rsrc, uint8_t* rslot,
                             hipStream_t st, uint32_t* passes_out);
hipError_t pp_fmask_build(const DevState& s, const unsigned long long* rend, const uint32_t* rsrc,
                          const uint8_t* rslot, uint8_t* fmask, hipStream_t st);
size_t pp_rev_range_scan_bytes(uint64_t n);
hipError_t pp_rev_count_range(const uint8_t* deg, const uint32_t* ids, uint64_t nfull, uint32_t stride, uint64_t lo,
                              uint64_t hi, unsigned long long* rend, void* tmp, size_t tmp_bytes, hipStream_t st);
hipError_t pp_rev_fill_range(const uint8_t* deg, const uint32_t* ids, uint64_t nfull, uint32_t stride, uint64_t lo,
                             uint64_t hi, unsigned long long* rend, uint32_t* rsrc, uint8_t* rslot, hipStream_t st);
hipError_t pp_fmask_rows(const DevState& s, uint8_t* fmask, hipStream_t st);
hipError_t pp_fmask_any(const uint8_t* fmask, uint64_t n, unsigned long long* fany, hipStream_t st);
hipError_t pp_rfail_build(const DevState& s, const unsigned long long* rend, const uint32_t* rsrc,
                          const uint8_t* rslot, uint32_t* rfail, hipStream_t st);
hipError_t pp_round_shard(const DevState& s, unsigned long long* next, unsigned long long* gnext, uint32_t t,
                          const PPSparse& sp, uint32_t mode, hipStream_t st);
hipError_t pp_count(const unsigned long long* words, uint64_t nwords, unsigned long long* out, hipStream_t st);
hipError_t pp_or_slices(unsigned long long* dst, const unsigned long long* src, uint32_t nslices, uint64_t words,
                        hipStream_t st);

struct PptState {
  const uint8_t* deg;
  const uint32_t* ids;
  unsigned long long* recv;
  const unsigned long long* crash;
  uint32_t* tstat;
  uint32_t n, trials, tlog, stride;
  uint32_t block, lds_bytes;
  uint32_t lds_masked;
  int32_t kd;
  Key key;
};
hipError_t ppt_lds_limit(int device, bool masked, uint64_t* limit, const char** where = nullptr);
hipError_t ppt_prepare(int device, bool masked, uint32_t lds_bytes);
hipError_t ppt_seed(const PptState& s, uint32_t node, uint32_t* started, hipStream_t st);
hipError_t ppt_rounds(const PptState& s, uint32_t t0, uint32_t rounds, hipStream_t st);
hipError_t ppt_stalled(const PptState& s, const uint8_t* need, uint32_t* live, hipStream_t st);

enum RumorAcc : uint32_t { RA_FIRED = 0, RA_SENT = 1, RA_MSGS = 2, RA_NEW = 3 };
constexpr uint32_t kRumorCovered = 1, kRumorQuiescent = 2;
constexpr uint32_t kRumorBlind = 1, kRumorCoin = 2, kRumorPull = 4;
struct RumorCtl {
  unsigned long long wlen;
  unsigned long long pad0_[31];
  unsigned long long acc[4];
  unsigned long long pad1_[28];
  unsigned long long rlen;
  unsigned long long received;
  unsigned long long cover;
  unsigned long long peak;
  uint32_t stop, pad2_;
  unsigned long long pad3_[27];
};
static_assert(sizeof(RumorCtl) == 3 * 256, "RumorCtl: three 256-byte blocks");
struct RumorState {
  RumorCtl* ctl;
  unsigned long long* next;
  uint8_t* miss;
  uint32_t k;
  uint32_t mode;
  unsigned long long* hot;
  unsigned long long* served;
  unsigned long long* vain;
};
uint32_t rumor_grid(uint64_t n, uint32_t want);
hipError_t rumor_seed(const DevState& s, const RumorState& r, uint32_t* list0, uint32_t node, unsigned long long cover,
                      hipStream_t st);
hipError_t rumor_round(const DevState& s, const RumorState& r, const uint32_t* rlist, uint32_t* wlist, uint32_t t,
                       uint32_t grid, hipStream_t st);
hipError_t rumor_commit(const DevState& s, const RumorState& r, uint32_t t, hipStream_t st);
hipError_t rumor_removed(const RumorState& r, const uint32_t* rlist, unsigned long long* out, uint32_t grid,
                         hipStream_t st);
hipError_t rumor_pull_seed(const DevState& s, const RumorState& r, uint32_t node, unsigned long long cover,
                           hipStream_t st);
hipError_t rumor_pull_round(const DevState& s, const RumorState& r, uint32_t t, uint32_t grid, hipStream_t st);
hipError_t rumor_pull_commit(const DevState& s, const RumorState& r, uint32_t t, hipStream_t st);
hipError_t rumor_pull_removed(const DevState& s, const RumorState& r, unsigned long long* out, hipStream_t st);

struct RmtState {
  const uint8_t* deg;
  const uint32_t* ids;
  unsigned long long* recv;
  unsigned long long* hot;
  uint8_t* miss;
  const unsigned long long* crash;
  uint32_t* tstat;
  uint32_t* nhot;
  uint32_t n, trials, tlog, stride;
  uint32_t block, lds_bytes;
  uint32_t k, mode;
  int32_t kd;
  Key key;
};
hipError_t rmt_lds_limit(int device, uint32_t mode, uint64_t* limit, const char** where = nullptr);
hipError_t rmt_prepare(int device, uint32_t mode, uint32_t lds_bytes);
hipError_t rmt_seed(const RmtState& s, uint32_t node, uint32_t* started, hipStream_t st);
hipError_t rmt_rounds(const RmtState& s, uint32_t t0, uint32_t rounds, hipStream_t st);

hipError_t launch_tick(const DevState& st, uint32_t tick, int mode, hipStream_t s);
hipError_t launch_slot_reset(const DevState& st, uint32_t slot, hipStream_t s);
hipError_t launch_schedule_one(const DevState& st, uint32_t node, uint32_t tick, hipStream_t s);
uint32_t tick_grid(const DevState& st);

struct OverlayResult {
  uint64_t final_tick;
  int rc;
  char msg[160];
};
struct OverlayWindowSink {
  void (*push)(void* self, uint64_t tick, uint64_t makeups, uint64_t breakups);
  void* self;
};
struct OverlayWork {
  struct Buf { void* p = nullptr; size_t bytes = 0; void* raw = nullptr; size_t off = 0; };
  std::vector<Buf> bucket;
  Buf scratch, outb, oslotb, cub_tmp, meta;
  Buf fine, ovp;
  uint64_t part_ticks = 0, sort_ticks = 0, part_fallbacks = 0;
  uint64_t pick_fallbacks = 0;
};
void overlay_free(OverlayWork* ws, hipStream_t st);
int overlay_build(uint64_t n, uint32_t trials, uint32_t tlog, int32_t fanout, int32_t fanin,
                  int32_t delay_low, int32_t delay_high, Key key, uint8_t* d_deg, uint32_t* d_ids,
                  uint32_t stride, uint64_t max_ticks, hipStream_t stream, OverlayWindowSink sink,
                  OverlayResult* res, OverlayWork* ws);

}
```

gossip_simulator_amd/csrc/gs_win_dev.h:

```cpp
#pragma once
#include <cstdlib>

#include "gossip.h"
#include "gs_internal.h"
#include "gs_wave.h"

namespace gs {
namespace {

constexpr uint32_t kExpandBlock = 256;
constexpr uint32_t kExpandBlock6 = 512;
constexpr uint32_t kExpandNpt = 4;
constexpr uint32_t kResolveBlock = 512;
#ifndef GS_RESOLVE_WAVES
#define GS_RESOLVE_WAVES 4
#endif
constexpr uint32_t kRoll0Coarse = kCoarseShift + 4;
constexpr uint32_t kRoll0Fine = kFineLog + 4;

inline uint32_t device_cus() {
  static const uint32_t cus = [] {
    int dev = 0, v = 0;
    if (hipGetDevice(&dev) == hipSuccess &&
        hipDeviceGetAttribute(&v, hipDeviceAttributeMultiprocessorCount, dev) == hipSuccess && v > 0)
      return (uint32_t)v;
    return 256u;
  }();
  return cus;
}

__device__ __forceinline__ uint32_t stop_bits(const WinState& w) {
  return w.dd && !w.solo ? kErrAbort : (kErrCoarse | kErrFine | kErrAbort);
}
__device__ __forceinline__ bool win_abort(const WinState& w) {
  return (*w.err & stop_bits(w)) != 0;
}
struct CtlView {
  uint32_t t, L, tnext, tend, poll, pbase, stop, lmax, err;
};
__device__ __forceinline__ CtlView ctl_view(const WinState& w) {
  static_assert(offsetof(WinCtl, t) == 0 && offsetof(WinCtl, lmax) == 28, "WinCtl's first 32 bytes");
  const uint4* p = reinterpret_cast<const uint4*>(w.ctl);
  const uint4 a = p[0], b = p[1];
  const uint32_t e = *w.err;
  return CtlView{a.x, a.y, a.z, a.w, b.x, b.y, b.z, b.w, e};
}
__device__ __forceinline__ uint32_t win_open(const WinState& w, uint32_t& t) {
  const CtlView c = ctl_view(w);
  t = c.tnext;
  const bool dead = (c.err & stop_bits(w)) || c.stop || t >= c.tend;
  uint32_t Lw = min(c.lmax, c.tend - t);
  if (c.poll) {
    const uint32_t P = c.pbase + c.poll * ((t - c.pbase + c.poll - 1) / c.poll);
    Lw = min(Lw, P - t + 1);
  }
  return dead ? 0u : Lw;
}
__device__ __forceinline__ uint32_t win_live(const WinState& w, uint32_t& t0, uint32_t L) {
  if (!w.ctl) return w.abort_on_err && win_abort(w) ? 0u : L;
  const CtlView c = ctl_view(w);
  t0 = c.t;
  const bool off = (c.err & stop_bits(w)) || (w.guard && !(c.err & kErrFine));
  return off ? 0u : c.L;
}

__device__ __forceinline__ unsigned long long* shard_row(const WinState& w, uint32_t k) {
  return w.sstats + ((size_t)(blockIdx.x & (kStatShards - 1)) * kMaxWindow + k) * kStatFields;
}

constexpr uint32_t kCloseLanes = 8;
__device__ __forceinline__ unsigned long long stat_shard_sum(const WinState& w, uint32_t i, uint32_t part) {
  constexpr uint32_t kPer = kStatShards / kCloseLanes;
  unsigned long long x[kPer], sum = 0;
#pragma unroll
  for (uint32_t j = 0; j < kPer; ++j) x[j] = w.sstats[(size_t)(j * kCloseLanes + part) * kMaxWindow * kStatFields + i];
#pragma unroll
  for (uint32_t j = 0; j < kPer; ++j) {
    sum += x[j];
    if (x[j]) w.sstats[(size_t)(j * kCloseLanes + part) * kMaxWindow * kStatFields + i] = 0;
  }
#pragma unroll
  for (uint32_t o = 1; o < kCloseLanes; o <<= 1) sum += __shfl_xor(sum, o, 64);
  return sum;
}

__device__ __forceinline__ void block_scan256(uint32_t* cnt, uint32_t* off) {
  if (threadIdx.x < 64) {
    const uint32_t l = threadIdx.x;
    const uint32_t a = cnt[4 * l], b = cnt[4 * l + 1], c = cnt[4 * l + 2], d = cnt[4 * l + 3];
    const uint32_t sum = a + b + c + d;
    const uint32_t x = wave_inscan(sum);
    const uint32_t ex = x - sum;
    off[4 * l] = ex;
    off[4 * l + 1] = ex + a;
    off[4 * l + 2] = ex + a + b;
    off[4 * l + 3] = ex + a + b + c;
    if (l == 63) off[256] = x;
  }
}

__device__ __forceinline__ unsigned long long region_end(const WinState& w, uint32_t r) {
  return w.ccap_end ? w.ccap_end[r] : w.ccap[r + 1];
}
__device__ __forceinline__ unsigned long long region_fill(const WinState& w, uint32_t r) {
  const unsigned long long room = region_end(w, r) - w.ccap[r];
  return w.cfill[r] < room ? w.cfill[r] : room;
}

__device__ __forceinline__ bool tiles_by_xcd(const WinState& w) {
  return w.csub == kCoarseSub && !w.csrc && !w.noxcd;
}
__device__ __forceinline__ uint32_t xcd_bin_pos(uint32_t c) { return (c & 7) * 32 + (c >> 3); }
__device__ __forceinline__ uint32_t xcd_bin_of(uint32_t pc) { return (pc & 31) * 8 + (pc >> 5); }

__device__ __forceinline__ uint32_t msg_loc(uint32_t m) { return m & (kFineNodes - 1); }
__device__ __forceinline__ uint32_t msg_tick(uint32_t m) { return (m >> kFineLog) & (kMaxWindow - 1); }

}
}
```

gossip_simulator_amd/csrc/gs_win_resolve.hip:

```cpp
#include <algorithm>

#include "gs_win_dev.h"

namespace gs {
namespace {

constexpr uint32_t kResolveMaxBuckets = 256;
constexpr uint32_t kSmallMax = 256;
#ifndef GS_SMALL_BLOCK
#define GS_SMALL_BLOCK 512
#endif
constexpr uint32_t kSmallBlock = GS_SMALL_BLOCK;
#ifndef GS_ROLLED_BLOCK
#define GS_ROLLED_BLOCK 256
#endif
constexpr uint32_t kRolledBlock = GS_ROLLED_BLOCK;

constexpr uint32_t kBitWords = kFineNodes / 32;
struct ResolveLds {
  union {
    struct {
      uint32_t b1[kBitTicks][kBitWords];
      uint2 cr0[kBitWords];
    };
    struct {
      uint32_t cnt[kFineNodes];
      uint32_t recv[kBitWords];
      uint32_t crash[kBitWords];
      uint32_t nrecv[kBitWords];
      uint32_t ncrash[kBitWords];
    };
  };
  uint32_t fc[kWinMaxRing];
  uint32_t st[kMaxWindow][4];
  uint32_t dead[kMaxWindow];
  uint32_t blist[kResolveMaxBuckets];
  unsigned long long bstart[kResolveMaxBuckets];
  uint32_t bcnt[kResolveMaxBuckets];
  uint32_t ndup;
  uint32_t ninf;
  uint32_t err;
  uint32_t nb;
  uint32_t cls;
  unsigned long long stamp[2][kStampPhases];
  unsigned long long tlast;
};
static_assert(kBitTicks <= kMaxWindow, "window ticks fit the message format");
static_assert(sizeof(uint32_t) * kFineNodes <= sizeof(((ResolveLds*)0)->cnt), "the infection list fits");

__device__ __forceinline__ void stamp(const WinState& w, ResolveLds& sm, uint32_t i) {
  if (w.dbg && threadIdx.x == 0) {
    const unsigned long long t = __builtin_amdgcn_s_memtime();
    if (i) sm.stamp[sm.cls][i] += t - sm.tlast;
    sm.tlast = t;
  }
}

#if defined(GS_RESOLVE_PROBE) && GS_RESOLVE_PROBE == 1
#define GS_RESOLVE_CR0(loc) make_uint2(0u, 0u)
#else
#define GS_RESOLVE_CR0(loc) sm.cr0[(loc) >> 5]
#endif


__device__ __forceinline__ void resolve_node(const WinState& w, ResolveLds& sm, uint32_t f,
                                             uint32_t loc, uint32_t kk, uint32_t ones, uint32_t t,
                                             uint32_t& cm, uint32_t& cr, uint32_t& cc, uint32_t& cs) {
  const uint32_t bit = 1u << (loc & 31), wi = loc >> 5;
  if (sm.crash[wi] & bit) return;
  const uint64_t g = (uint64_t)w.base + (f << kFineLog) + loc;
  uint32_t u, c3order;
  node_key(w.tlog, w.tmask, w.key, g, K_ORDER, u, c3order);
  const uint32_t pos = ones ? first_crash(u, t, kk, ones, c3order, w.key.k0, w.key.k1) : kk + 1;
  cm += pos <= kk ? pos : kk;
  if (pos > 1 && !(sm.recv[wi] & bit)) {
    atomicOr(&sm.recv[wi], bit);
    ++cr;
    uint32_t c3delay;
    node_key(w.tlog, w.tmask, w.key, g, K_DELAY, u, c3delay);
    const uint32_t off = fire_offset(w.delay_low, w.delay_span,
                                     philox(u, t, 0, c3delay, w.key.k0, w.key.k1).x);
    const uint32_t s = (t + off) % w.R;
    const uint32_t at = atomicAdd(&sm.fc[s], 1u);
    w.flist[((size_t)s * w.nfine + f) * kFineNodes + at] = (uint16_t)loc;
    ++cs;
  }
  if (pos <= kk) {
    atomicOr(&sm.crash[wi], bit);
    ++cc;
  }
}

template <class Src>
__device__ __forceinline__ void resolve_tick(const WinState& w, ResolveLds& sm, uint32_t f,
                                             const Src& src, uint32_t lo, uint32_t hi, uint32_t k,
                                             uint32_t t) {
  const uint32_t tid = threadIdx.x;
  for (uint32_t p = lo + tid; p < hi; p += kResolveBlock) {
    const uint32_t m = src[p];
    if (msg_tick(m) != k) continue;
    const uint32_t old = atomicAdd(&sm.cnt[msg_loc(m)], 1u + (((m >> kRoll0Fine) & 1u) << 16));
    if ((old & 0xFFFFu) == 0xFFFFu) sm.err = 1;
  }
  __syncthreads();
  uint32_t arr = 0, cm = 0, cr = 0, cc = 0, cs = 0;
  for (uint32_t p = lo + tid; p < hi; p += kResolveBlock) {
    const uint32_t m = src[p];
    if (msg_tick(m) != k) continue;
    const uint32_t loc = msg_loc(m);
    const uint32_t kk = atomicExch(&sm.cnt[loc], 0u);
    arr += kk & 0xFFFFu;
    if (kk) resolve_node(w, sm, f, loc, kk & 0xFFFFu, kk >> 16, t, cm, cr, cc, cs);
  }
  if (arr != cm) atomicAdd(&sm.st[k][0], arr - cm);
  if (cr) atomicAdd(&sm.st[k][1], cr);
  if (cc) atomicAdd(&sm.st[k][2], cc);
  (void)cs;
  __syncthreads();
}

__device__ __forceinline__ void flush_counts(const WinState& w, ResolveLds& sm, uint32_t (&acc_ni)[kBitTicks / 2],
                                             uint32_t L, uint32_t trial) {
#pragma unroll
  for (uint32_t k = 0; k < kBitTicks; ++k) {
    if (k >= L) continue;
    const uint32_t sr = wave_sum((acc_ni[k / 2] >> (16 * (k & 1))) & 0xFFFFu);
    if (lane_id() == 0 && sr) atomicAdd(&sm.st[k][1], sr);
  }
#pragma unroll
  for (uint32_t k = 0; k < kBitTicks / 2; ++k) acc_ni[k] = 0;
  __syncthreads();
  const uint32_t tid = threadIdx.x;
  if (tid < L * 3) {
    const uint32_t k = tid / 3, fld = tid - k * 3;
    const uint32_t v = sm.st[k][fld];
    unsigned long long* row = shard_row(w, k);
    if (v && fld == 0) atomicAdd(&row[ST_MSGS], 0ull - (unsigned long long)v);
    if (v && fld == 1) {
      atomicAdd(&row[ST_RECV], (unsigned long long)v);
      atomicAdd(&row[ST_SCHED], (unsigned long long)v);
    }
    if (v && fld == 2) atomicAdd(&row[ST_CRASH], (unsigned long long)v);
    if (v && trial != ~0u) atomicAdd(&w.tstat[((size_t)trial * kMaxWindow + w.tofs + k) * kTStatFields + TS_DEAD + fld], v);
    sm.st[k][fld] = 0;
  }
  __syncthreads();
}

__device__ __forceinline__ void resolve_body(const WinState& w, uint32_t t0, uint32_t L) {
  __shared__ ResolveLds sm;
  const uint32_t tid = threadIdx.x, G = gridDim.x;
  L = win_live(w, t0, L);
  if (!L) return;
  static_assert(kBitWords == kResolveBlock, "one bit word per thread");
  static_assert(kWinMaxRing <= kResolveBlock, "one ring slot per thread");
  if (tid < kMaxWindow * 4) (&sm.st[0][0])[tid] = 0;
  if (tid == 0) { sm.nb = 0; sm.cls = 0; }
  if (tid < 2 * kStampPhases) (&sm.stamp[0][0])[tid] = 0;
  __syncthreads();
  {
    const uint32_t f = blockIdx.x + tid * G;
    const unsigned long long fl = tid < kResolveMaxBuckets && f < w.nfine ? w.ffill[f] : 0ull;
    const bool ne = fl > kSmallMax;
    const uint32_t at = wave_append(&sm.nb, ne);
    if (ne) {
      sm.blist[at] = f;
      sm.bstart[at] = w.fstart[f];
      sm.bcnt[at] = (uint32_t)fl;
    }
  }
  __syncthreads();
  const uint32_t nb = sm.nb;
  stamp(w, sm, 0);
  uint32_t fB = 0, MB = 0;
  unsigned long long mbB = 0;
  auto next_bucket = [&](uint32_t j) { fB = sm.blist[j]; mbB = sm.bstart[j]; MB = sm.bcnt[j]; };
  if (nb > 0) next_bucket(0);
  uint32_t* rwg = (uint32_t*)w.recv;
  uint32_t* cwg = (uint32_t*)w.crash;
  uint32_t acc_ni[kBitTicks / 2];
#pragma unroll
  for (uint32_t k = 0; k < kBitTicks / 2; ++k) acc_ni[k] = 0;
  static_assert(kBitTicks % 2 == 0 && 32 * kResolveMaxBuckets < 65536, "two 16-bit counts per register");
  constexpr uint32_t kU = 8;
  constexpr uint32_t kBatch = kResolveBlock * kU;
  auto ld = [&](const uint32_t* gm, uint32_t M, uint32_t p0, uint32_t (&m)[kU]) {
#pragma unroll
    for (uint32_t u = 0; u < kU; ++u) {
      const uint32_t p = p0 + u * kResolveBlock + tid;
      m[u] = *reinterpret_cast<const uint32_t*>(reinterpret_cast<const char*>(gm) + ((p < M ? p : M - 1) << 2));
    }
  };
  uint32_t pm[kU], p_recv0 = 0, p_crash0 = 0, p_roll0 = 0, p_fcv = 0;
  bool p_in = false;
  auto prefetch = [&](uint32_t f, uint32_t M, unsigned long long mb) {
    const uint64_t wi = ((uint64_t)(f << kFineLog) >> 5) + tid;
    const bool in = wi < w.W * 2;
    const uint64_t wc = in ? wi : w.W * 2 - 1;
    p_in = in;
    p_recv0 = rwg[wc];
    p_crash0 = cwg[wc];
    p_roll0 = w.rollw[wc];
    p_fcv = w.fcount[(size_t)(tid < w.R ? tid : 0u) * w.nfine + f];
    ld(w.fmsg + mb, M, 0, pm);
  };
  if (nb > 0) prefetch(fB, MB, mbB);
  for (uint32_t i = 0; i < nb; ++i) {
    const uint32_t f = fB, M = MB;
    const unsigned long long mb = mbB;
    const uint32_t node0 = f << kFineLog;
    const uint64_t wi = ((uint64_t)node0 >> 5) + tid;
    uint32_t knode0, c3order;
    node_key(w.tlog, w.tmask, w.key, (uint64_t)w.base + node0, K_ORDER, knode0, c3order);
    const uint32_t c3delay = (c3order & 0xFFFFFFu) | (K_DELAY << 24);
    const bool in = wi < w.W * 2;
    const uint32_t recv0 = p_in ? p_recv0 : 0u, crash0 = p_in ? p_crash0 : 0u, roll0 = p_in ? p_roll0 : 0u;
    const uint32_t fcv = tid < w.R ? p_fcv : 0u;
    if (i + 1 < nb) next_bucket(i + 1);
    if (roll0) w.rollw[wi] = 0u;
    const uint32_t rollw = roll0 & ~crash0;
#pragma unroll
    for (uint32_t k = 0; k < kBitTicks; ++k)
      if (k < L) sm.b1[k][tid] = 0;
    sm.cr0[tid] = make_uint2(crash0, rollw);
    if (tid < w.R) sm.fc[tid] = fcv;
    if (tid < kMaxWindow) sm.dead[tid] = 0;
    if (tid == 0) { sm.ndup = 0; sm.ninf = 0; sm.err = M >= (1u << 28) ? 3 : 0; sm.cls = M >= 1024 ? 1 : 0; }
    __syncthreads();
    stamp(w, sm, 1);
    const uint32_t* gm = w.fmsg + mb;
    unsigned long long dlo = 0, dhi = 0;
    auto flush_dead = [&]() {
      while (dlo) {
        const uint32_t b = __builtin_ctzll(dlo) >> 3;
        atomicAdd(&sm.dead[b], (uint32_t)(dlo >> (8 * b)) & 255u);
        dlo &= ~(255ull << (8 * b));
      }
      while (dhi) {
        const uint32_t b = __builtin_ctzll(dhi) >> 3;
        atomicAdd(&sm.dead[8 + b], (uint32_t)(dhi >> (8 * b)) & 255u);
        dhi &= ~(255ull << (8 * b));
      }
    };
#define GS_RESOLVE_BATCH(m, VALID)                                                                \
    {                                                                                             \
      uint2 sp[kU];                                                                               \
      _Pragma("unroll") for (uint32_t u = 0; u < kU; ++u) {                                       \
        sp[u] = make_uint2(0, 0);                                                                 \
        if (VALID) {                                                                              \
          const uint32_t loc = msg_loc(m[u]);                                                     \
          atomicOr(&sm.b1[msg_tick(m[u])][loc >> 5], 1u << (loc & 31));          \
          sp[u] = GS_RESOLVE_CR0(loc);                                                            \
        }                                                                                         \
      }                                                                                           \
      uint32_t dm = 0;                                  \
      _Pragma("unroll") for (uint32_t u = 0; u < kU; ++u) {                                       \
        const uint32_t sh = msg_loc(m[u]) & 31, k = msg_tick(m[u]);                               \
        if ((sp[u].x >> sh) & 1u) {            \
          if (k < 8) dlo += 1ull << (8 * k);                                                      \
          else dhi += 1ull << (8 * (k - 8));                                                      \
        }                                                                                         \
        if ((sp[u].y >> sh) & 1u) dm |= 1u << u;                                                  \
      }                                                                                           \
      if (nbat % 31 == 30) flush_dead();                                                          \
      const uint32_t nd = __popc(dm);                                                             \
      if (__ballot(nd != 0)) {                                                                    \
        uint32_t pre = 0, tot = 0;                                  \
        _Pragma("unroll") for (uint32_t bb = 0; bb < 4; ++bb) {                                   \
          const unsigned long long bal = __ballot((nd >> bb) & 1u);                               \
          pre += lanes_below(bal) << bb;                                                                \
          tot += (uint32_t)__popcll(bal) << bb;                                                   \
        }                                                                                         \
        uint32_t base = 0;                                                                        \
        if (lane_id() == 0) base = atomicAdd(&sm.ndup, tot);                                      \
        uint32_t at = __builtin_amdgcn_readfirstlane(base) + pre;                                 \
        _Pragma("unroll") for (uint32_t u = 0; u < kU; ++u) if ((dm >> u) & 1u) {                 \
          if (at < kRolledCap) w.rlmsg[(size_t)f * kRolledCap + at] = m[u] & ((1u << 19) - 1);    \
          else sm.err = 3;                                                                        \
          ++at;                                                                                   \
        }                                                                                         \
      }                                                                                           \
    }
    {
      uint32_t m[kU];
#pragma unroll
      for (uint32_t u = 0; u < kU; ++u) m[u] = pm[u];
      for (uint32_t p0 = 0, nbat = 0; p0 < (sm.err == 3 ? 0u : M); p0 += kBatch, ++nbat) {
        uint32_t mn[kU];
        if (p0 + kBatch < M) ld(gm, M, p0 + kBatch, mn);
        GS_RESOLVE_BATCH(m, p0 + u * kResolveBlock + tid < M)
#pragma unroll
        for (uint32_t u = 0; u < kU; ++u) m[u] = mn[u];
      }
    }
#undef GS_RESOLVE_BATCH
    flush_dead();
    stamp(w, sm, 2);
    __syncthreads();
    if (i + 1 < nb) prefetch(fB, MB, mbB);
    if (tid == 0) w.rlcnt[f] = sm.err == 3 ? 0u : min(sm.ndup, kRolledCap);
    stamp(w, sm, 3);
    uint32_t rw = recv0, cw = crash0;
    if (sm.err != 3) {
      if (tid < L && sm.dead[tid]) atomicAdd(&sm.st[tid][0], sm.dead[tid]);
      uint32_t infk[kBitTicks], ninf = 0;
      const uint32_t plain = ~(crash0 | rollw);
#pragma unroll
      for (uint32_t k = 0; k < kBitTicks; ++k) {
        infk[k] = 0;
        if (k >= L) continue;
        const uint32_t infS = sm.b1[k][tid] & plain & ~rw;
        rw |= infS;
        infk[k] = infS;
      }
      stamp(w, sm, 4);
#pragma unroll
      for (uint32_t k = 0; k < kBitTicks; ++k) {
        const uint32_t ni = __popc(infk[k]);
        acc_ni[k / 2] += ni << (16 * (k & 1));
        ninf += ni;
      }
      stamp(w, sm, 5);
      __syncthreads();
      stamp(w, sm, 6);
      auto bcast = [&](uint32_t x) {
        const uint32_t loc = msg_loc(x), t = t0 + msg_tick(x);
        const uint32_t off = fire_offset(w.delay_low, w.delay_span,
                                         philox(knode0 + loc, t, 0, c3delay, w.key.k0, w.key.k1).x);
        const uint32_t slot = (t + off) % w.R;
        const uint32_t pos = atomicAdd(&sm.fc[slot], 1u);
        w.flist[((size_t)slot * w.nfine + f) * kFineNodes + pos] = (uint16_t)loc;
      };
      uint32_t* inf = &sm.cnt[0];
      {
        uint32_t pre = 0, tot = 0;
#pragma unroll
        for (uint32_t b = 0; b < 9; ++b) {
          const unsigned long long bal = __ballot((ninf >> b) & 1u);
          pre += lanes_below(bal) << b;
          tot += (uint32_t)__popcll(bal) << b;
        }
        uint32_t base = 0;
        if (tot && lane_id() == 0) base = atomicAdd(&sm.ninf, tot);
        uint32_t at = __builtin_amdgcn_readfirstlane(base) + pre;
#pragma unroll
        for (uint32_t k = 0; k < kBitTicks; ++k)
          for (uint32_t x = k < L ? infk[k] : 0u; x; x &= x - 1)
            inf[at++] = (tid * 32 + __builtin_ctz(x)) | (k << kFineLog);
      }
      __syncthreads();
      stamp(w, sm, 7);
      const uint32_t ni_all = sm.ninf;
      for (uint32_t q = tid; q < ni_all; q += kResolveBlock) bcast(inf[q]);
    } else {
      __syncthreads();
      uint4* c4 = reinterpret_cast<uint4*>(sm.cnt);
      for (uint32_t q = tid; q < kFineNodes / 4; q += kResolveBlock) c4[q] = make_uint4(0, 0, 0, 0);
      sm.recv[tid] = recv0;
      sm.crash[tid] = crash0;
      sm.nrecv[tid] = 0;
      sm.ncrash[tid] = 0;
      __syncthreads();
      for (uint32_t k = 0; k < L; ++k) resolve_tick(w, sm, f, gm, 0, M, k, t0 + k);
      rw = sm.recv[tid] | sm.nrecv[tid];
      cw = sm.crash[tid] | sm.ncrash[tid];
      if (tid == 0 && sm.err == 1) atomicOr(w.err, kErrArrivals);
    }
    __syncthreads();
    stamp(w, sm, 8);
    if (in) {
      if (rw != recv0) rwg[wi] = rw;
      if (cw != crash0) cwg[wi] = cw;
    }
    if (tid < w.R) w.fcount[(size_t)tid * w.nfine + f] = sm.fc[tid];
    stamp(w, sm, 9);
    if (w.dbg && tid == 0) sm.stamp[sm.cls][0] += 1;
    if (w.tstat) flush_counts(w, sm, acc_ni, L, (uint32_t)(((uint64_t)w.base + node0) >> w.tlog));
  }
  if (w.dbg && tid < 2 * kStampPhases) atomicAdd(&w.dbg[tid], (&sm.stamp[0][0])[tid]);
  if (!w.tstat) flush_counts(w, sm, acc_ni, L, ~0u);
}
__global__ __launch_bounds__(kResolveBlock, GS_RESOLVE_WAVES) void k_resolve(const WinState w, uint32_t t0, uint32_t L) {
  resolve_body(w, t0, L);
}
__global__ __launch_bounds__(kResolveBlock, GS_RESOLVE_WAVES) void k_resolve_m(const WinState* __restrict__ ws,
                                                                                uint32_t L) {
  resolve_body(ws[blockIdx.y], 0u, L);
}

template <uint32_t E, bool ROLLED>
__device__ __forceinline__ void resolve_small_bucket(const WinState& w, uint32_t t0, uint32_t L, uint32_t f,
                                                     const uint32_t* gm, unsigned long long M,
                                                     uint32_t (*st)[kMaxWindow][4], uint32_t* skw,
                                                     uint32_t* fcw) {
  constexpr uint32_t N = 64 * E;
  const uint32_t lane = threadIdx.x & 63, wv = threadIdx.x >> 6;
  {
    const bool consume = !ROLLED && w.ctl;
    const uint32_t s0 = t0 % w.R;
    for (uint32_t s = lane; s < w.R; s += 64)
      fcw[s] = consume && (s + w.R - s0) % w.R < L ? 0u : w.fcount[(size_t)s * w.nfine + f];
    uint32_t knode0, c3order;
    node_key(w.tlog, w.tmask, w.key, (uint64_t)w.base + (f << kFineLog), K_ORDER, knode0, c3order);
    const uint32_t c3delay = (c3order & 0xFFFFFFu) | (K_DELAY << 24);
    uint32_t key[E];
#pragma unroll
    for (uint32_t r = 0; r < E; ++r) {
      const uint32_t i = lane * E + r;
      key[r] = ~0u;
      if (i < M) {
        const uint32_t m = gm[i];
        key[r] = (msg_loc(m) << 5) | (msg_tick(m) << 1) | ((m >> kRoll0Fine) & 1u);
        if (!ROLLED && ((m >> kRoll0Fine) & 1u)) w.rollw[((f << kFineLog) + msg_loc(m)) >> 5] = 0u;
      }
    }
#pragma unroll
    for (uint32_t k = 2; k <= N; k <<= 1)
#pragma unroll
      for (uint32_t j = k >> 1; j > 0; j >>= 1) {
        if (j >= E) {
#pragma unroll
          for (uint32_t r = 0; r < E; ++r) {
            const uint32_t i = lane * E + r;
            const uint32_t o = __shfl_xor(key[r], j / E, 64);
            const bool keep_min = ((i & j) == 0) == ((i & k) == 0);
            key[r] = keep_min ? min(key[r], o) : max(key[r], o);
          }
        } else {
#pragma unroll
          for (uint32_t r = 0; r < E; ++r) {
            if (r & j) continue;
            const bool up = ((lane * E + r) & k) == 0;
            const uint32_t a = key[r], b = key[r | j];
            key[r] = up ? min(a, b) : max(a, b);
            key[r | j] = up ? max(a, b) : min(a, b);
          }
        }
      }
#pragma unroll
    for (uint32_t r = 0; r < E; ++r) skw[lane * E + r] = key[r];
    wave_lds_sync();
    uint32_t* rwg = (uint32_t*)w.recv;
    uint32_t* cwg = (uint32_t*)w.crash;
    bool any_inf = false;
    uint32_t head = 0;
#pragma unroll
    for (uint32_t r = 0; r < E; ++r) {
      const uint32_t i = lane * E + r;
      if (key[r] != ~0u && !(i > 0 && (skw[i - 1] >> 5) == (key[r] >> 5))) head |= 1u << r;
    }
#pragma unroll 1
    for (uint32_t r = 0; r < E; ++r) {
      if (!((head >> r) & 1u)) continue;
      const uint32_t i = lane * E + r;
      const uint32_t loc = skw[i] >> 5;
      const uint32_t wi = ((f << kFineLog) + loc) >> 5, bit = 1u << (loc & 31), u = knode0 + loc;
      const uint32_t cw = cwg[wi];
      bool rv = (rwg[wi] & bit) != 0, cr = (cw & bit) != 0, inf = false;
      uint32_t tinf = 0;
      for (uint32_t q = i; q < N;) {
        const uint32_t e = skw[q];
        if ((e >> 5) != loc) break;
        const uint32_t k = (e >> 1) & (kMaxWindow - 1), t = t0 + k;
        uint32_t c = 0, ones = 0;
        for (; q < N && (skw[q] >> 1) == (e >> 1); ++q) {
          ++c;
          ones += skw[q] & 1u;
        }
        if (cr) {
          atomicAdd(&st[wv][k][0], c);
          continue;
        }
        const uint32_t g = ones ? first_crash(u, t, c, ones, c3order, w.key.k0, w.key.k1) : c + 1;
        if (g > 1 && !rv) {
          rv = inf = true;
          tinf = t;
          atomicAdd(&st[wv][k][1], 1u);
        }
        if (g <= c) {
          cr = true;
          atomicAdd(&st[wv][k][2], 1u);
          if (c > g) atomicAdd(&st[wv][k][0], c - g);
        }
      }
      if (cr && !(cw & bit)) atomicOr(&cwg[wi], bit);
      if (inf) {
        any_inf = true;
        atomicOr(&rwg[wi], bit);
        const uint32_t off = fire_offset(w.delay_low, w.delay_span,
                                         philox(u, tinf, 0, c3delay, w.key.k0, w.key.k1).x);
        const uint32_t slot = (tinf + off) % w.R;
        const uint32_t pos = atomicAdd(&fcw[slot], 1u);
        w.flist[((size_t)slot * w.nfine + f) * kFineNodes + pos] = (uint16_t)loc;
      }
    }
    wave_lds_sync();
    if (__ballot(any_inf)) {
      for (uint32_t s = lane; s < w.R; s += 64) w.fcount[(size_t)s * w.nfine + f] = fcw[s];
    } else if (consume && lane < L) {
      w.fcount[(size_t)((t0 + lane) % w.R) * w.nfine + f] = 0;
    }
    if (w.tstat) {
      wave_lds_sync();
      if (lane < L * 3) {
        const uint32_t k = lane / 3, fld = lane - k * 3;
        const uint32_t v = st[wv][k][fld];
        const uint32_t trial = (uint32_t)(((uint64_t)w.base + (f << kFineLog)) >> w.tlog);
        if (v) atomicAdd(&w.tstat[((size_t)trial * kMaxWindow + w.tofs + k) * kTStatFields + TS_DEAD + fld], v);
      }
    }
  }
}

template <bool ROLLED>
__device__ __forceinline__ void resolve_small_body(const WinState& w, uint32_t t0, uint32_t L) {
  constexpr uint32_t kWaves = (ROLLED ? kRolledBlock : kSmallBlock) / 64;
  constexpr uint32_t kEmax = ROLLED ? 16 : 4;
  __shared__ uint32_t st[kWaves][kMaxWindow][4];
  __shared__ uint32_t sk[kWaves][64 * kEmax];
  __shared__ uint32_t fcw[kWaves][kWinMaxRing];
  const uint32_t tid = threadIdx.x, wv = tid >> 6;
  static_assert(kWaves * kMaxWindow * 4 == kWaves * 64, "one counter per thread");
  static_assert(kRolledCap == 64 * 16, "the rolled bodies cover 1..kRolledCap");
  const uint32_t f = __builtin_amdgcn_readfirstlane(blockIdx.x * kWaves + wv);
  unsigned long long M = 0;
  const uint32_t* gm = nullptr;
  if (f < w.nfine) {
    if (ROLLED) {
      M = w.rlcnt[f];
      gm = w.rlmsg + (size_t)f * kRolledCap;
    } else {
      M = w.ffill[f];
      gm = w.fmsg + w.fstart[f];
    }
  }
  L = win_live(w, t0, L);
  if (!L) return;
  (&st[0][0][0])[tid] = 0;
  __syncthreads();
  if (M > 0 && M <= 64) resolve_small_bucket<1, ROLLED>(w, t0, L, f, gm, M, st, sk[wv], fcw[wv]);
  else if (M > 64 && M <= 256) resolve_small_bucket<4, ROLLED>(w, t0, L, f, gm, M, st, sk[wv], fcw[wv]);
  else if (ROLLED && M > 256 && M <= 512)
    resolve_small_bucket<ROLLED ? 8 : 1, ROLLED>(w, t0, L, f, gm, M, st, sk[wv], fcw[wv]);
  else if (ROLLED && M > 512 && M <= kRolledCap)
    resolve_small_bucket<ROLLED ? 16 : 1, ROLLED>(w, t0, L, f, gm, M, st, sk[wv], fcw[wv]);
  if (ROLLED && M && (threadIdx.x & 63) == 0) w.rlcnt[f] = 0;
  if (!ROLLED && w.ctl && !(M > 0 && M <= 256) && f < w.nfine && (threadIdx.x & 63) < L)
    w.fcount[(size_t)((t0 + (threadIdx.x & 63)) % w.R) * w.nfine + f] = 0;
  __syncthreads();
  if (tid < L * 3) {
    const uint32_t k = tid / 3, fld = tid - k * 3;
    uint32_t v = 0;
    for (uint32_t q = 0; q < kWaves; ++q) v += st[q][k][fld];
    unsigned long long* row = shard_row(w, k);
    if (v && fld == 0) atomicAdd(&row[ST_MSGS], 0ull - (unsigned long long)v);
    if (v && fld == 1) {
      atomicAdd(&row[ST_RECV], (unsigned long long)v);
      atomicAdd(&row[ST_SCHED], (unsigned long long)v);
    }
    if (v && fld == 2) atomicAdd(&row[ST_CRASH], (unsigned long long)v);
  }
}
template <bool ROLLED>
__global__ __launch_bounds__(ROLLED ? kRolledBlock : kSmallBlock) void k_resolve_small(const WinState w, uint32_t t0,
                                                                                       uint32_t L) {
  resolve_small_body<ROLLED>(w, t0, L);
}
template <bool ROLLED>
__global__ __launch_bounds__(ROLLED ? kRolledBlock : kSmallBlock) void k_resolve_small_m(
    const WinState* __restrict__ ws, uint32_t L) {
  resolve_small_body<ROLLED>(ws[blockIdx.y], 0u, L);
}

}

hipError_t win_resolve(const WinState& w, uint32_t t0, uint32_t L, hipStream_t s) {
  const uint32_t cus = device_cus();
  static const uint32_t per_cu = [] { const char* e = getenv("GS_RESOLVE_PER_CU"); return e ? (uint32_t)std::max(atoi(e), 1) : 2u; }();
  uint32_t G = std::min<uint32_t>(w.nfine, per_cu * cus);
  G = std::max<uint32_t>(G, (w.nfine + kResolveMaxBuckets - 1) / kResolveMaxBuckets);
  const uint32_t gs = (w.nfine + kSmallBlock / 64 - 1) / (kSmallBlock / 64);
  hipLaunchKernelGGL(k_resolve_small<false>, dim3(gs), dim3(kSmallBlock), 0, s, w, t0, L);
  static_assert(kSmallMax == 64 * 4, "the two bodies cover 1..kSmallMax");
  hipLaunchKernelGGL(k_resolve, dim3(G), dim3(kResolveBlock), 0, s, w, t0, L);
  hipLaunchKernelGGL(k_resolve_small<true>, dim3((w.nfine + kRolledBlock / 64 - 1) / (kRolledBlock / 64)),
                     dim3(kRolledBlock), 0, s, w, t0, L);
  return hipGetLastError();
}

hipError_t win_resolve_g(const WinGroup& g, uint32_t L, hipStream_t s) {
  const uint32_t cus = device_cus();
  uint32_t G = std::min<uint32_t>(g.nfine_max, (2 * cus + g.M - 1) / g.M);
  G = std::max<uint32_t>(G, (g.nfine_max + kResolveMaxBuckets - 1) / kResolveMaxBuckets);
  const uint32_t gs = (g.nfine_max + kSmallBlock / 64 - 1) / (kSmallBlock / 64);
  hipLaunchKernelGGL(k_resolve_small_m<false>, dim3(gs, g.M), dim3(kSmallBlock), 0, s, g.wr, L);
  hipLaunchKernelGGL(k_resolve_m, dim3(G, g.M), dim3(kResolveBlock), 0, s, g.wr, L);
  hipLaunchKernelGGL(k_resolve_small_m<true>, dim3((g.nfine_max + kRolledBlock / 64 - 1) / (kRolledBlock / 64), g.M),
                     dim3(kRolledBlock), 0, s, g.wr, L);
  return hipGetLastError();
}

}
```

gossip_simulator_amd/csrc/gs_win_units.hip:

```cpp
#include <hipcub/hipcub.hpp>

#include "gs_win_dev.h"

namespace gs {
namespace {

__device__ __forceinline__ void units_body(const WinState& w, uint32_t t0, uint32_t L) {
  __shared__ uint32_t s_t[kMaxWindow];
  uint32_t Ls = L;
  if (w.ctl) {
    L = win_open(w, t0);
    if (!L) return;
    Ls = w.lstride;
  }
  const uint32_t units = Ls * w.nfine;
  const uint32_t tid = blockIdx.x * blockDim.x + threadIdx.x, nth = gridDim.x * blockDim.x;
  __shared__ uint32_t s_tile[256 * (kMaxWindow + 1)];
  uint32_t acc[kMaxWindow];
#pragma unroll
  for (uint32_t k = 0; k < kMaxWindow; ++k) acc[k] = 0;
  if (threadIdx.x < kMaxWindow) s_t[threadIdx.x] = 0;
  if (tid == 0) w.usize[units] = 0;
  __syncthreads();
  __shared__ uint32_t s_ts[kMaxWindow];
  uint32_t slot[kMaxWindow];
#pragma unroll
  for (uint32_t k = 0; k < kMaxWindow; ++k) slot[k] = k < L ? (t0 + k) % w.R : 0u;
  for (uint32_t f0 = blockIdx.x * 256; f0 < w.nfine; f0 += gridDim.x * 256) {
    const uint32_t f = f0 + threadIdx.x;
    if (threadIdx.x < kMaxWindow) s_ts[threadIdx.x] = 0;
    uint32_t cv[kMaxWindow];
#pragma unroll
    for (uint32_t k = 0; k < kMaxWindow; ++k)
      cv[k] = k < L && k < Ls && f < w.nfine ? w.fcount[(size_t)slot[k] * w.nfine + f] : 0u;
#pragma unroll
    for (uint32_t k = 0; k < kMaxWindow; ++k) {
      if (k < Ls) {
        s_tile[threadIdx.x * (kMaxWindow + 1) + k] = cv[k];
        acc[k] += cv[k];
      }
    }
    __syncthreads();
#pragma unroll
    for (uint32_t k = 0; k < kMaxWindow; ++k) {
      if (k < Ls) {
        const uint32_t c = wave_sum(s_tile[threadIdx.x * (kMaxWindow + 1) + k]);
        if ((threadIdx.x & 63) == 0 && c) atomicAdd(&s_ts[k], c);
      }
    }
    __syncthreads();
    if (threadIdx.x < Ls) w.tsum[(size_t)(f0 >> 8) * kMaxWindow + threadIdx.x] = s_ts[threadIdx.x];
    const uint32_t nb = min(256u, w.nfine - f0), base = f0 * Ls;
    for (uint32_t i = threadIdx.x; i < nb * Ls; i += 256) {
      const uint32_t b = i / Ls, k = i - b * Ls;
      w.usize[base + i] = s_tile[b * (kMaxWindow + 1) + k];
    }
    __syncthreads();
  }
#pragma unroll
  for (uint32_t k = 0; k < kMaxWindow; ++k)
    if (acc[k]) atomicAdd(&s_t[k], acc[k]);
  __syncthreads();
  if (threadIdx.x < L && s_t[threadIdx.x]) atomicAdd(&w.tfires[threadIdx.x], (unsigned long long)s_t[threadIdx.x]);
  for (uint32_t i = tid; i < kRegions; i += nth) { w.chist[i] = 0; w.cfill[i] = 0; }
  for (uint32_t i = tid; i < w.nfine; i += nth) w.ffill[i] = 0;
  if (w.dd && tid == 0) {
    w.cfill[kRegions] = 0;
    w.cfill[kRegions + 1] = w.ctl->fmsg_cap;
    w.cfill[kRegions + 2] = w.ctl->xs_cap;
    w.cfill[kRegions + 3] = w.ctl->xr_cap;
  }
  if (tid == 0 && !w.ctl && !w.abort_on_err) *w.err &= ~(kErrCoarse | kErrFine);
}
__global__ __launch_bounds__(256) void k_units(const WinState w, uint32_t t0, uint32_t L) { units_body(w, t0, L); }

__global__ __launch_bounds__(256) void k_units_m(const WinState* __restrict__ ws, uint32_t t0, uint32_t L) {
  units_body(ws[blockIdx.y], t0, L);
}

__device__ __forceinline__ void cut_body(const WinState& w, unsigned long long budget) {
  __shared__ unsigned long long s_sz[256];
  __shared__ unsigned long long s_T;
  __shared__ uint32_t s_go, s_L;
  WinCtl* c = w.ctl;
  const uint32_t b = threadIdx.x;
  __shared__ unsigned long long s_tf[kMaxWindow];
  if (win_abort(w)) return;
  uint32_t t = 0;
  const uint32_t Lw = win_open(w, t);
  const unsigned long long cap = c->cmsg_cap;
  __shared__ unsigned long long s_own[kMaxWindow];
  if (b < kMaxWindow) {
    if (w.dd) {
      unsigned long long g = 0;
      for (uint32_t r = 0; r < w.G; ++r) g += w.gcnt[(size_t)r * kMaxWindow + b];
      s_tf[b] = g;
      s_own[b] = w.tfires[b];
    } else {
      s_tf[b] = w.tfires[b];
    }
  }
  unsigned long long ts[4][kMaxWindow];
#pragma unroll
  for (uint32_t j = 0; j < 4; ++j)
#pragma unroll
    for (uint32_t k = 0; k < kMaxWindow; ++k)
      ts[j][k] = Lw && b * 4 + j < w.ncoarse ? w.tsum[(size_t)(b * 4 + j) * kMaxWindow + k] : 0ull;
  __syncthreads();
  if (b == 0) {
    s_go = Lw != 0;
    if (!Lw) {
      c->L = 0;
      c->Tn = 0;
    } else {
      uint32_t L = 1;
      unsigned long long Tn = s_tf[0];
      while (L < Lw && (Tn + s_tf[L]) * w.stride <= budget) Tn += s_tf[L++];
      if (w.dd) {
        Tn = 0;
        for (uint32_t k = 0; k < L; ++k) Tn += s_own[k];
      } else {
        for (uint32_t k = 0; k < kMaxWindow; ++k) w.tfires[k] = 0;
      }
      c->t = t;
      c->L = L;
      s_L = L;
      c->tnext = t + L;
      c->Tn = Tn;
      c->T = Tn * (w.owner ? w.slots : w.stride);
      s_T = c->T;
    }
  }
  __syncthreads();
  if (!s_go) return;
  {
    const uint32_t L = s_L, nt = w.ncoarse;
    unsigned long long v[4], sum = 0;
#pragma unroll
    for (uint32_t j = 0; j < 4; ++j) {
      v[j] = 0;
#pragma unroll
      for (uint32_t k = 0; k < kMaxWindow; ++k) v[j] += k < L ? ts[j][k] : 0ull;
      sum += v[j];
    }
    unsigned long long tot;
    unsigned long long pre = block_exscan_u64<4>(sum, &s_sz[0], &tot);
#pragma unroll
    for (uint32_t j = 0; j < 4; ++j) {
      const uint32_t tile = b * 4 + j;
      if (tile < nt) w.toff[tile] = pre;
      pre += v[j];
    }
    if (b == 0) w.toff[nt] = tot;
    __syncthreads();
  }
  unsigned long long sub = 0;
  if (!w.owner) {
    const unsigned long long lo = (unsigned long long)b << kCoarseShift;
    const unsigned long long hi = min((unsigned long long)w.n, lo + (1ull << kCoarseShift));
    const double xr = (double)kXRoundNodes * w.stride;
    sub = b < w.ncoarse
              ? (unsigned long long)(((double)s_T / kCoarseSub + xr) * (double)(hi - lo) / (double)w.n) + 512
              : 0ull;
  } else {
    const uint32_t d = b / w.obins, k = b % w.obins;
    unsigned long long cnt = 0;
    if (d < w.G) {
      const unsigned long long dlo = (unsigned long long)d * w.seg_per;
      const unsigned long long dhi = min(dlo + w.seg_per, (unsigned long long)w.nglob);
      const unsigned long long lo = dlo + ((unsigned long long)k << kCoarseShift);
      const unsigned long long hi = min(dhi, lo + (1ull << kCoarseShift));
      cnt = hi > lo ? hi - lo : 0ull;
    }
    const double xr = (double)kXRoundNodes * w.slots;
    sub = cnt ? (unsigned long long)(((double)s_T / kCoarseSub + xr) * (double)cnt / (double)w.nglob) + 512 : 0ull;
  }
  unsigned long long total;
  const unsigned long long base = block_exscan_u64<4>(sub * kCoarseSub, &s_sz[0], &total);
  if (total > cap) {
    for (uint32_t x = 0; x < kCoarseSub; ++x) w.ccap[b * kCoarseSub + x] = 0;
    if (b == 0) {
      w.ccap[kRegions] = 0;
      atomicOr(w.err, kErrCoarse);
      if (w.dd) atomicOr(reinterpret_cast<unsigned int*>(&w.cfill[kRegions]), kErrCoarse);
    }
    return;
  }
  for (uint32_t x = 0; x < kCoarseSub; ++x) w.ccap[b * kCoarseSub + x] = base + x * sub;
  if (b == 255) w.ccap[kRegions] = total;
}
__global__ __launch_bounds__(256) void k_cut(const WinState w, unsigned long long budget) { cut_body(w, budget); }
__global__ __launch_bounds__(256) void k_cut_m(const WinState* __restrict__ ws, unsigned long long budget) {
  cut_body(ws[blockIdx.x], budget);
}

__device__ __forceinline__ void unitscan_body(const WinState& w) {
  __shared__ unsigned long long s_x[4];
  if (blockIdx.x >= w.ncoarse) return;
  uint32_t t0;
  const uint32_t L = win_live(w, t0, 0);
  if (!L) return;
  const uint32_t Ls = w.lstride, tile = blockIdx.x, f = tile * 256 + threadIdx.x;
  if (w.dd && tile == 0 && threadIdx.x < kMaxWindow) w.tfires[threadIdx.x] = 0;
  unsigned long long sz[kMaxWindow], sum = 0;
#pragma unroll
  for (uint32_t k = 0; k < kMaxWindow; ++k)
    sz[k] = k < L && f < w.nfine ? w.usize[(size_t)f * Ls + k] : 0ull;
#pragma unroll
  for (uint32_t k = 0; k < kMaxWindow; ++k) sum += sz[k];
  unsigned long long tot;
  unsigned long long a = w.toff[tile] + block_exscan_u64<4>(sum, s_x, &tot);
  if (f >= w.nfine) return;
#pragma unroll
  for (uint32_t k = 0; k < kMaxWindow; ++k) {
    if (k >= Ls) break;
    const uint32_t u = f * Ls + k;
    w.unit_off[u] = a;
    const unsigned long long b = a + sz[k];
    for (unsigned long long q = (a + 63) >> 6; (q << 6) < b; ++q) w.gmap[q] = u;
    a = b;
  }
  if (f == w.nfine - 1) w.unit_off[(size_t)w.nfine * Ls] = a;
}
__global__ __launch_bounds__(256) void k_unitscan(const WinState w) { unitscan_body(w); }
__global__ __launch_bounds__(256) void k_unitscan_m(const WinState* __restrict__ ws) { unitscan_body(ws[blockIdx.y]); }

__global__ void k_groupmap(const WinState w, uint32_t L) {
  if (w.ctl) {
    uint32_t t0;
    if (!win_live(w, t0, 0)) return;
    L = w.lstride;
  }
  const uint32_t units = L * w.nfine;
  for (uint32_t u = blockIdx.x * blockDim.x + threadIdx.x; u < units; u += gridDim.x * blockDim.x) {
    const unsigned long long a = w.unit_off[u], b = w.unit_off[u + 1];
    for (unsigned long long q = (a + 63) >> 6; (q << 6) < b; ++q) w.gmap[q] = u;
  }
}

__global__ void k_stats_reduce(const WinState w, uint32_t t0, uint32_t L) {
  if (w.abort_on_err && win_abort(w)) return;
  const uint32_t i = threadIdx.x / kCloseLanes, part = threadIdx.x % kCloseLanes;
  const uint32_t k = i / kStatFields, fld = i % kStatFields;
  if (k >= L) return;
  const unsigned long long sum = stat_shard_sum(w, i, part);
  if (part == 0 && sum) w.stats[(size_t)((t0 + k) % kStatSlots) * kStatFields + fld] += sum;
}

__global__ void k_close(const WinState w, uint32_t slot) {
  __shared__ unsigned long long rows[kMaxWindow][kStatFields];
  WinCtl* c = w.ctl;
  unsigned long long* st = w.stage + (size_t)slot * kStageWords;
  uint32_t t0 = 0;
  const uint32_t L = win_live(w, t0, 0);
  const uint32_t i = threadIdx.x / kCloseLanes, part = threadIdx.x % kCloseLanes, tid = threadIdx.x;
  const uint32_t k = i / kStatFields, fld = i % kStatFields;
  if (k < L) {
    const unsigned long long sum = stat_shard_sum(w, i, part);
    if (part == 0) {
      rows[k][fld] = sum;
      w.stats[(size_t)((t0 + k) % kStatSlots) * kStatFields + fld] = sum;
      st[8 + k * kStatFields + fld] = sum;
    }
  }
  __syncthreads();
  if (tid != 0) return;
  uint32_t stop = c->stop;
  if (L) {
    for (uint32_t j = 0; j < L; ++j) {
      c->recv += rows[j][ST_RECV];
      c->crashed += rows[j][ST_CRASH];
      c->pending += rows[j][ST_SCHED] - rows[j][ST_FIRED];
    }
    const uint32_t tl = t0 + L - 1;
    if (c->poll && (tl - c->pbase) % c->poll == 0 && !stop) {
      if (c->recv >= c->cover) stop = 1 + GS_RUN_COVERED;
      else if (c->pending == 0) stop = 1 + GS_RUN_QUIESCENT;
      else if (tl >= c->max_ticks) stop = 1 + GS_RUN_MAX_TICKS;
      c->stop = stop;
    }
  }
  st[0] = t0;
  st[1] = L;
  st[2] = stop;
  st[3] = *w.err;
  st[4] = L ? c->Tn : 0;
}

__global__ void k_schedule_win(const WinState w, uint32_t node, uint32_t t, uint32_t trials, uint32_t n,
                               uint32_t* __restrict__ started) {
  const uint32_t i = blockIdx.x * blockDim.x + threadIdx.x;
  if (i >= trials) return;
  uint32_t local = node;
  if (trials > 1 || node == ~0u) {
    uint32_t v = node;
    if (node == ~0u) v = uniform(philox(0, 0, 0, ctr3(K_SENDER, w.key.trial + i), w.key.k0, w.key.k1).x, n);
    local = (i << w.tlog) | v;
  }
  if (started) {
    const bool dead = (w.crash[local >> 6] >> (local & 63)) & 1;
    started[i] = dead ? 0u : 1u;
    if (dead) return;
  }
  uint32_t kn, c3;
  node_key(w.tlog, w.tmask, w.key, (uint64_t)w.base + local, K_DELAY, kn, c3);
  const uint32_t off = fire_offset(w.delay_low, w.delay_span, philox(kn, t, 0, c3, w.key.k0, w.key.k1).x);
  const uint32_t s = (t + off) % w.R;
  const uint32_t f = local >> kFineLog;
  const uint32_t pos = atomicAdd(&w.fcount[(size_t)s * w.nfine + f], 1u);
  w.flist[((size_t)s * w.nfine + f) * kFineNodes + pos] = (uint16_t)(local & (kFineNodes - 1));
}

}

hipError_t win_units_g(const WinGroup& g, uint32_t L, hipStream_t s) {
  const uint32_t blocks = std::max<uint32_t>(std::min<uint32_t>((g.nfine_max + 255) / 256, 4096), 1);
  hipLaunchKernelGGL(k_units_m, dim3(blocks, g.M), dim3(256), 0, s, g.ws, 0u, L);
  return hipGetLastError();
}

hipError_t win_cut_g(const WinGroup& g, unsigned long long budget, hipStream_t s) {
  hipLaunchKernelGGL(k_cut_m, dim3(g.M), dim3(256), 0, s, g.ws, budget);
  return hipGetLastError();
}

hipError_t win_unitscan_g(const WinGroup& g, hipStream_t s) {
  hipLaunchKernelGGL(k_unitscan_m, dim3(std::max<uint32_t>(g.ncoarse_max, 1), g.M), dim3(256), 0, s, g.ws);
  return hipGetLastError();
}

hipError_t win_units(const WinState& w, uint32_t t0, uint32_t L, hipStream_t s) {
  (void)L;
  const uint32_t blocks = std::max<uint32_t>(std::min<uint32_t>((w.nfine + 255) / 256, 4096), 1);
  hipLaunchKernelGGL(k_units, dim3(blocks), dim3(256), 0, s, w, t0, L);
  return hipGetLastError();
}

hipError_t win_cut(const WinState& w, unsigned long long budget, hipStream_t s) {
  hipLaunchKernelGGL(k_cut, dim3(1), dim3(256), 0, s, w, budget);
  return hipGetLastError();
}

hipError_t win_unitscan(const WinState& w, hipStream_t s) {
  hipLaunchKernelGGL(k_unitscan, dim3(w.ncoarse), dim3(256), 0, s, w);
  return hipGetLastError();
}

hipError_t win_close(const WinState& w, uint32_t slot, hipStream_t s) {
  hipLaunchKernelGGL(k_close, dim3(1), dim3(kMaxWindow * kStatFields * kCloseLanes), 0, s, w, slot);
  return hipGetLastError();
}

hipError_t win_scan_units(const WinState& w, uint32_t L, void* tmp, size_t& tmp_bytes, hipStream_t s) {
  return hipcub::DeviceScan::ExclusiveSum(tmp, tmp_bytes, (const unsigned long long*)w.usize,
                                          w.unit_off, (int)(L * w.nfine + 1), s);
}

hipError_t win_groupmap(const WinState& w, uint32_t L, hipStream_t s) {
  const uint32_t units = L * w.nfine;
  const uint32_t blocks = std::min<uint32_t>((units + 255) / 256, 4096);
  hipLaunchKernelGGL(k_groupmap, dim3(blocks ? blocks : 1), dim3(256), 0, s, w, L);
  return hipGetLastError();
}

hipError_t win_stats_reduce(const WinState& w, uint32_t t0, uint32_t L, hipStream_t s) {
  hipLaunchKernelGGL(k_stats_reduce, dim3(1), dim3(kMaxWindow * kStatFields * kCloseLanes), 0, s, w, t0, L);
  return hipGetLastError();
}

hipError_t win_schedule(const WinState& w, uint32_t node, uint32_t tick, uint32_t trials, uint32_t n,
                        hipStream_t s, uint32_t* started) {
  hipLaunchKernelGGL(k_schedule_win, dim3((trials + 255) / 256), dim3(256), 0, s, w, node, tick, trials, n, started);
  return hipGetLastError();
}

}
```

include/gossip.h:

```cpp
#ifndef GOSSIP_H
#define GOSSIP_H
#include <stddef.h>
#include <stdint.h>

#ifdef __cplusplus
extern "C" {
#endif

#define GS_ABI_VERSION 6

enum {
  GS_OK = 0,
  GS_EINVAL = -1,
  GS_ELIVELOCK = -2,
  GS_EREJECT = -3,
  GS_ENOMEM = -4,
  GS_EDEVICE = -5,
  GS_EOVERFLOW = -6
};

#define GS_FLAG_TIMING 1u
#define GS_FLAG_TICK_ENGINE 2u
#define GS_FLAG_PP_L2_ONLY 4u
#define GS_FLAG_PP_DENSE 8u
#define GS_FLAG_PP_EARLY 16u
#define GS_FLAG_PP_TOPDOWN 32u
#define GS_FLAG_PP_BOTTOM 64u
#define GS_FLAG_PP_ANSWER 128u

#define GS_MODEL_FLOOD 0u
#define GS_MODEL_PUSHPULL 1u
#define GS_MODEL_RUMOR 2u

#define GS_RUMOR_BLIND 1u
#define GS_RUMOR_COIN 2u
#define GS_RUMOR_PULL 4u

typedef struct gs_params {
  uint64_t n;
  int32_t fanout;
  int32_t fanin;
  int32_t delay_low;
  int32_t delay_high;
  double drop_rate;
  double crash_rate;
  uint64_t seed;
  uint32_t trial;
  int32_t device;
  uint32_t flags;
  uint32_t model;
  uint32_t trials;
  uint32_t rumor_k;
  uint32_t rumor_mode;
  uint32_t reserved32_;
  uint64_t reserved_[4];
} gs_params;

typedef struct gs_tick_stats {
  uint64_t tick;
  uint64_t fired;
  uint64_t sent;
  uint64_t messages;
  uint64_t received;
  uint64_t crashed;
  uint64_t pending;
} gs_tick_stats;

typedef struct gs_window {
  uint64_t tick;
  uint64_t makeups;
  uint64_t breakups;
} gs_window;

typedef struct gs_timing {
  double deliver_ms;
  double resolve_ms;
  uint64_t deliver_launches;
  uint64_t resolve_launches;
  double overlay_ms;
  double expand_ms;
  double part_ms;
  uint64_t windows;
  uint64_t exact_redos;
  double prep_ms;
  uint64_t pp_early_rounds;
  uint64_t pp_bottom_rounds;
  uint64_t pp_answer_rounds;
  uint64_t dd_fallbacks;
  uint64_t pp_rev_part;
  uint64_t ov_part_ticks;
  uint64_t ov_sort_ticks;
  uint64_t ov_part_fallbacks;
  double alloc_ms;
  double largest_alloc_ms;
  double free_ms;
  uint64_t alloc_calls;
  uint64_t alloc_cache_hits;
  uint64_t cached_bytes;
  uint64_t coarse_redos;
} gs_timing;

enum { GS_RUN_COVERED = 0, GS_RUN_QUIESCENT = 1, GS_RUN_MAX_TICKS = 2, GS_RUN_RUNNING = -1 };

typedef struct gs_trial_stats {
  uint64_t trial;
  uint64_t tick_99;
  uint64_t tick;
  uint64_t fired, sent, messages, received, crashed;
  int32_t status;
  int32_t reserved_;
} gs_trial_stats;

typedef struct gs_ctx gs_ctx;

int gs_version(void);
const char* gs_strerror(int code);

int gs_create(const gs_params* params, gs_ctx** out);

int gs_create_multi(const gs_params* params, const int* devices, int ndev, gs_ctx** out);
#define GS_COMM_ID_BYTES 128
int gs_comm_unique_id(uint8_t id[GS_COMM_ID_BYTES]);
int gs_create_rank(const gs_params* params, int device, int nranks, int rank,
                   const uint8_t* id, gs_ctx** out);
typedef struct gs_exchange {
  void* user;
  int (*all_gather)(void* user, const void* send, void* recv, size_t bytes);
  int (*all_reduce_sum_u64)(void* user, uint64_t* buf, size_t count);
  int (*all_to_allv)(void* user, const void* send, const size_t* send_bytes, void* recv,
                     const size_t* recv_bytes);
} gs_exchange;
int gs_create_rank_exchange(const gs_params* params, int device, int nranks, int rank, const gs_exchange* ex,
                            gs_ctx** out);
int gs_shard_info(const gs_ctx* ctx, uint32_t index, uint32_t* nshards, uint64_t* lo, uint64_t* hi);
void gs_destroy(gs_ctx* ctx);
const char* gs_last_error(const gs_ctx* ctx);
int gs_pp_trials_max_n(int device, uint64_t* n_max);
int gs_pp_trials_max_n_masked(int device, uint64_t* n_max);
int gs_create_trials(const gs_params* params, gs_ctx** out);
int gs_rumor_trials_max_n(int device, uint32_t rumor_mode, uint64_t* n_max);

int gs_load_peers(gs_ctx* ctx, const uint8_t* deg, const uint32_t* ids, uint32_t stride);
int gs_load_peers_device(gs_ctx* ctx, const void* d_deg, const void* d_ids, uint32_t stride);
int gs_read_peers(gs_ctx* ctx, uint8_t* deg, uint32_t* ids, uint32_t* stride_out);

int gs_build_overlay(gs_ctx* ctx, uint64_t max_ticks, gs_window* win, size_t cap,
                     size_t* nwin, uint64_t* final_tick);

int gs_set_failed(gs_ctx* ctx, const uint64_t* words, size_t nwords);

int gs_broadcast_begin(gs_ctx* ctx, int64_t sender);
int gs_step(gs_ctx* ctx, uint32_t ticks, gs_tick_stats* out);
int gs_run(gs_ctx* ctx, uint32_t poll, uint64_t max_ticks, gs_tick_stats* out,
           size_t cap, size_t* nout, int32_t* status);
int gs_totals(gs_ctx* ctx, gs_tick_stats* out);

int gs_trial_results(gs_ctx* ctx, gs_trial_stats* out, size_t cap, size_t* nout);

int gs_read_received(gs_ctx* ctx, uint64_t* words, size_t nwords);
int gs_read_crashed(gs_ctx* ctx, uint64_t* words, size_t nwords);
int gs_read_removed(gs_ctx* ctx, uint64_t* words, size_t nwords);

int gs_timing_get(gs_ctx* ctx, gs_timing* out);
int gs_shard_timing(gs_ctx* ctx, uint32_t index, gs_timing* out);
int gs_set_trial(gs_ctx* ctx, uint32_t trial);
int gs_set_flags(gs_ctx* ctx, uint32_t flags);
int gs_reset(gs_ctx* ctx);

int gs_set_stream(gs_ctx* ctx, void* hip_stream);
int gs_trim(int device, size_t* released);
int gs_memory_stats(gs_timing* out);

size_t gs_format_float32(float x, char* buf, size_t cap);
size_t gs_format_float64(double x, char* buf, size_t cap);
size_t gs_format_duration(int64_t ns, char* buf, size_t cap);
int32_t gs_threshold(double rate);
void gs_philox(const uint32_t ctr[4], const uint32_t key[2], uint32_t out[4]);

#ifdef __cplusplus
}
#endif
#endif
```

Before: 85.24 billion msgs/s.

## Split rare large-bucket resolve path into its own kernel to shrink resolve LDS

The resolve kernel's LDS union carried a per-node count array for the rare path where a bucket has very many messages. That path is moved into a separate k_resolve_large kernel fed by a device-side list of deferred buckets. The main resolve LDS is capped at 40 KB so four workgroups can fit per CU, and the infection list is processed in chunks that fit the reused bitmap space. The resolve kernel is also templated on block size (256 or 512 via an env var) and a counter of large buckets is exported in timing. The cost is an extra kernel launch per window plus the chunking loop and more complex code.

```diff
diff --git a/gossip_simulator_amd/_lib.py b/gossip_simulator_amd/_lib.py
--- a/gossip_simulator_amd/_lib.py
+++ b/gossip_simulator_amd/_lib.py
@@ -90,7 +90,7 @@
                 ("ov_part_ticks", C.c_uint64), ("ov_sort_ticks", C.c_uint64), ("ov_part_fallbacks", C.c_uint64),
                 ("alloc_ms", C.c_double), ("largest_alloc_ms", C.c_double), ("free_ms", C.c_double),
                 ("alloc_calls", C.c_uint64), ("alloc_cache_hits", C.c_uint64), ("cached_bytes", C.c_uint64),
-                ("coarse_redos", C.c_uint64)]
+                ("coarse_redos", C.c_uint64), ("resolve_large_buckets", C.c_uint64)]
 
 
 ALL_GATHER_FN = C.CFUNCTYPE(C.c_int, C.c_void_p, C.c_void_p, C.c_void_p, C.c_size_t)
diff --git a/gossip_simulator_amd/csrc/gs_api.cpp b/gossip_simulator_amd/csrc/gs_api.cpp
--- a/gossip_simulator_amd/csrc/gs_api.cpp
+++ b/gossip_simulator_amd/csrc/gs_api.cpp
@@ -725,6 +725,15 @@
     out->pp_answer_rounds = h.nanswer;
   }
   if (c->pp && c->begun) out->pp_early_rounds += c->rs.rep_rounds;
+  out->resolve_large_buckets = 0;
+  for (gs_ctx* m : shards_of(c)) {
+    if (!m->win || !m->ws.lglist) continue;
+    uint32_t handed = 0;
+    CK(m, hipSetDevice(m->dev));
+    CK(m, hipMemcpyAsync(&handed, m->ws.lglist + 1, 4, hipMemcpyDeviceToHost, m->stream));
+    CK(m, hipStreamSynchronize(m->stream));
+    out->resolve_large_buckets += handed;
+  }
   fill_devmem(out);
   return GS_OK;
 }
diff --git a/gossip_simulator_amd/csrc/gs_ctx.cpp b/gossip_simulator_amd/csrc/gs_ctx.cpp
--- a/gossip_simulator_amd/csrc/gs_ctx.cpp
+++ b/gossip_simulator_amd/csrc/gs_ctx.cpp
@@ -132,6 +132,11 @@
   if (dev_malloc(&c->wn.d_rlmsg, (size_t)w.nfine * kRolledCap * 4) != hipSuccess)
     return fail(c, GS_ENOMEM, "cannot allocate the rolled-receipt lists");
   w.rlmsg = (uint32_t*)c->wn.d_rlmsg;
+  if (dev_malloc(&c->wn.d_lglist, ((size_t)w.nfine + 2) * 4) != hipSuccess)
+    return fail(c, GS_ENOMEM, "cannot allocate the large-path bucket list");
+  w.lglist = (uint32_t*)c->wn.d_lglist;
+  if (hipMemsetAsync(w.lglist, 0, ((size_t)w.nfine + 2) * 4, c->stream) != hipSuccess)
+    return fail(c, GS_EDEVICE, "memset of the large-path bucket list failed");
   w.dbg = nullptr;
   if (getenv("GS_STAMPS") && dev_malloc(&w.dbg, kDbgWords * 8) == hipSuccess)
     (void)hipMemset(w.dbg, 0, kDbgWords * 8);
@@ -154,7 +159,7 @@
 
 void release_window(gs_ctx* c) {
   WinEngine& e = c->wn;
-  for (void* p : {e.d_win, e.d_flist, e.d_rlmsg, (void*)e.d_rtab, (void*)c->ws.dbg})
+  for (void* p : {e.d_win, e.d_flist, e.d_rlmsg, e.d_lglist, (void*)e.d_rtab, (void*)c->ws.dbg})
     if (p) (void)dev_free(p);
   for (Buf* b : {&e.gmap, &e.cmsg, &e.fmsg, &e.tmp}) release(*b);
   for (void* p : {(void*)e.h_cap, (void*)e.h_misc, (void*)e.h_err, (void*)e.h_rtab})
diff --git a/gossip_simulator_amd/csrc/gs_ctx.h b/gossip_simulator_amd/csrc/gs_ctx.h
--- a/gossip_simulator_amd/csrc/gs_ctx.h
+++ b/gossip_simulator_amd/csrc/gs_ctx.h
@@ -35,6 +35,7 @@
   void* d_win = nullptr;
   void* d_flist = nullptr;
   void* d_rlmsg = nullptr;
+  void* d_lglist = nullptr;
   size_t fcount_bytes = 0;
   Buf gmap, cmsg, fmsg, tmp;
   unsigned long long* h_cap = nullptr;
diff --git a/gossip_simulator_amd/csrc/gs_internal.h b/gossip_simulator_amd/csrc/gs_internal.h
--- a/gossip_simulator_amd/csrc/gs_internal.h
+++ b/gossip_simulator_amd/csrc/gs_internal.h
@@ -103,6 +103,7 @@
   uint32_t* rollw;
   uint32_t* rlmsg;
   uint32_t* rlcnt;
+  uint32_t* lglist;
   unsigned long long* stats;
   uint32_t* err;
   uint32_t* fcount;
diff --git a/gossip_simulator_amd/csrc/gs_win_dev.h b/gossip_simulator_amd/csrc/gs_win_dev.h
--- a/gossip_simulator_amd/csrc/gs_win_dev.h
+++ b/gossip_simulator_amd/csrc/gs_win_dev.h
@@ -12,6 +12,7 @@
 constexpr uint32_t kExpandBlock6 = 512;
 constexpr uint32_t kExpandNpt = 4;
 constexpr uint32_t kResolveBlock = 512;
+constexpr uint32_t kResolveBlockDefault = 512;
 #ifndef GS_RESOLVE_WAVES
 #define GS_RESOLVE_WAVES 4
 #endif
diff --git a/gossip_simulator_amd/csrc/gs_win_resolve.hip b/gossip_simulator_amd/csrc/gs_win_resolve.hip
--- a/gossip_simulator_amd/csrc/gs_win_resolve.hip
+++ b/gossip_simulator_amd/csrc/gs_win_resolve.hip
@@ -17,19 +17,14 @@
 constexpr uint32_t kRolledBlock = GS_ROLLED_BLOCK;
 
 constexpr uint32_t kBitWords = kFineNodes / 32;
+constexpr uint32_t kInfCap = 6144;
 struct ResolveLds {
   union {
     struct {
       uint32_t b1[kBitTicks][kBitWords];
       uint2 cr0[kBitWords];
     };
-    struct {
-      uint32_t cnt[kFineNodes];
-      uint32_t recv[kBitWords];
-      uint32_t crash[kBitWords];
-      uint32_t nrecv[kBitWords];
-      uint32_t ncrash[kBitWords];
-    };
+    uint32_t inf[kInfCap];
   };
   uint32_t fc[kWinMaxRing];
   uint32_t st[kMaxWindow][4];
@@ -46,7 +41,21 @@
   unsigned long long tlast;
 };
 static_assert(kBitTicks <= kMaxWindow, "window ticks fit the message format");
-static_assert(sizeof(uint32_t) * kFineNodes <= sizeof(((ResolveLds*)0)->cnt), "the infection list fits");
+static_assert(sizeof(uint32_t) * kInfCap <= sizeof(uint32_t) * kBitTicks * kBitWords + sizeof(uint2) * kBitWords,
+              "the infection list fits the dead bitmaps");
+static_assert(sizeof(ResolveLds) <= 40 * 1024, "four resolve workgroups fit a CU's 160 KB of LDS");
+
+struct LargeLds {
+  uint32_t cnt[kFineNodes];
+  uint32_t recv[kBitWords];
+  uint32_t crash[kBitWords];
+  uint32_t nrecv[kBitWords];
+  uint32_t ncrash[kBitWords];
+  uint32_t fc[kWinMaxRing];
+  uint32_t st[kMaxWindow][4];
+  uint32_t err;
+};
+constexpr uint32_t kLargeGrid = 64;
 
 __device__ __forceinline__ void stamp(const WinState& w, ResolveLds& sm, uint32_t i) {
   if (w.dbg && threadIdx.x == 0) {
@@ -63,7 +72,7 @@
 #endif
 
 
-__device__ __forceinline__ void resolve_node(const WinState& w, ResolveLds& sm, uint32_t f,
+__device__ __forceinline__ void resolve_node(const WinState& w, LargeLds& sm, uint32_t f,
                                              uint32_t loc, uint32_t kk, uint32_t ones, uint32_t t,
                                              uint32_t& cm, uint32_t& cr, uint32_t& cc, uint32_t& cs) {
   const uint32_t bit = 1u << (loc & 31), wi = loc >> 5;
@@ -92,7 +101,7 @@
 }
 
 template <class Src>
-__device__ __forceinline__ void resolve_tick(const WinState& w, ResolveLds& sm, uint32_t f,
+__device__ __forceinline__ void resolve_tick(const WinState& w, LargeLds& sm, uint32_t f,
                                              const Src& src, uint32_t lo, uint32_t hi, uint32_t k,
                                              uint32_t t) {
   const uint32_t tid = threadIdx.x;
@@ -119,21 +128,11 @@
   __syncthreads();
 }
 
-__device__ __forceinline__ void flush_counts(const WinState& w, ResolveLds& sm, uint32_t (&acc_ni)[kBitTicks / 2],
-                                             uint32_t L, uint32_t trial) {
-#pragma unroll
-  for (uint32_t k = 0; k < kBitTicks; ++k) {
-    if (k >= L) continue;
-    const uint32_t sr = wave_sum((acc_ni[k / 2] >> (16 * (k & 1))) & 0xFFFFu);
-    if (lane_id() == 0 && sr) atomicAdd(&sm.st[k][1], sr);
-  }
-#pragma unroll
-  for (uint32_t k = 0; k < kBitTicks / 2; ++k) acc_ni[k] = 0;
-  __syncthreads();
+__device__ __forceinline__ void flush_st(const WinState& w, uint32_t (*st)[4], uint32_t L, uint32_t trial) {
   const uint32_t tid = threadIdx.x;
   if (tid < L * 3) {
     const uint32_t k = tid / 3, fld = tid - k * 3;
-    const uint32_t v = sm.st[k][fld];
+    const uint32_t v = st[k][fld];
     unsigned long long* row = shard_row(w, k);
     if (v && fld == 0) atomicAdd(&row[ST_MSGS], 0ull - (unsigned long long)v);
     if (v && fld == 1) {
@@ -142,18 +141,35 @@
     }
     if (v && fld == 2) atomicAdd(&row[ST_CRASH], (unsigned long long)v);
     if (v && trial != ~0u) atomicAdd(&w.tstat[((size_t)trial * kMaxWindow + w.tofs + k) * kTStatFields + TS_DEAD + fld], v);
-    sm.st[k][fld] = 0;
+    st[k][fld] = 0;
   }
   __syncthreads();
 }
 
+__device__ __forceinline__ void flush_counts(const WinState& w, ResolveLds& sm, uint32_t (&acc_ni)[kBitTicks / 2],
+                                             uint32_t L, uint32_t trial) {
+#pragma unroll
+  for (uint32_t k = 0; k < kBitTicks; ++k) {
+    if (k >= L) continue;
+    const uint32_t sr = wave_sum((acc_ni[k / 2] >> (16 * (k & 1))) & 0xFFFFu);
+    if (lane_id() == 0 && sr) atomicAdd(&sm.st[k][1], sr);
+  }
+#pragma unroll
+  for (uint32_t k = 0; k < kBitTicks / 2; ++k) acc_ni[k] = 0;
+  __syncthreads();
+  flush_st(w, sm.st, L, trial);
+}
+
+template <uint32_t B>
 __device__ __forceinline__ void resolve_body(const WinState& w, uint32_t t0, uint32_t L) {
   __shared__ ResolveLds sm;
   const uint32_t tid = threadIdx.x, G = gridDim.x;
   L = win_live(w, t0, L);
   if (!L) return;
-  static_assert(kBitWords == kResolveBlock, "one bit word per thread");
-  static_assert(kWinMaxRing <= kResolveBlock, "one ring slot per thread");
+  constexpr uint32_t kW = kBitWords / B;
+  static_assert(kBitWords % B == 0, "whole bit words per thread");
+  static_assert(kWinMaxRing <= B, "one ring slot per thread");
+  static_assert(kResolveMaxBuckets <= B, "one bucket descriptor per thread");
   if (tid < kMaxWindow * 4) (&sm.st[0][0])[tid] = 0;
   if (tid == 0) { sm.nb = 0; sm.cls = 0; }
   if (tid < 2 * kStampPhases) (&sm.stamp[0][0])[tid] = 0;
@@ -181,26 +197,34 @@
   uint32_t acc_ni[kBitTicks / 2];
 #pragma unroll
   for (uint32_t k = 0; k < kBitTicks / 2; ++k) acc_ni[k] = 0;
-  static_assert(kBitTicks % 2 == 0 && 32 * kResolveMaxBuckets < 65536, "two 16-bit counts per register");
+  static_assert(kBitTicks % 2 == 0 && 32 * kW * kResolveMaxBuckets < 65536, "two 16-bit counts per register");
   constexpr uint32_t kU = 8;
-  constexpr uint32_t kBatch = kResolveBlock * kU;
+  constexpr uint32_t kBatch = B * kU;
   auto ld = [&](const uint32_t* gm, uint32_t M, uint32_t p0, uint32_t (&m)[kU]) {
 #pragma unroll
     for (uint32_t u = 0; u < kU; ++u) {
-      const uint32_t p = p0 + u * kResolveBlock + tid;
+      const uint32_t p = p0 + u * B + tid;
       m[u] = *reinterpret_cast<const uint32_t*>(reinterpret_cast<const char*>(gm) + ((p < M ? p : M - 1) << 2));
     }
   };
-  uint32_t pm[kU], p_recv0 = 0, p_crash0 = 0, p_roll0 = 0, p_fcv = 0;
-  bool p_in = false;
+  uint32_t pm[kU], p_recv0[kW], p_crash0[kW], p_roll0[kW], p_fcv = 0;
+  bool p_in[kW];
+#pragma unroll
+  for (uint32_t j = 0; j < kW; ++j) {
+    p_recv0[j] = p_crash0[j] = p_roll0[j] = 0;
+    p_in[j] = false;
+  }
   auto prefetch = [&](uint32_t f, uint32_t M, unsigned long long mb) {
-    const uint64_t wi = ((uint64_t)(f << kFineLog) >> 5) + tid;
-    const bool in = wi < w.W * 2;
-    const uint64_t wc = in ? wi : w.W * 2 - 1;
-    p_in = in;
-    p_recv0 = rwg[wc];
-    p_crash0 = cwg[wc];
-    p_roll0 = w.rollw[wc];
+#pragma unroll
+    for (uint32_t j = 0; j < kW; ++j) {
+      const uint64_t wi = ((uint64_t)(f << kFineLog) >> 5) + tid + j * B;
+      const bool in = wi < w.W * 2;
+      const uint64_t wc = in ? wi : w.W * 2 - 1;
+      p_in[j] = in;
+      p_recv0[j] = rwg[wc];
+      p_crash0[j] = cwg[wc];
+      p_roll0[j] = w.rollw[wc];
+    }
     p_fcv = w.fcount[(size_t)(tid < w.R ? tid : 0u) * w.nfine + f];
     ld(w.fmsg + mb, M, 0, pm);
   };
@@ -209,20 +233,30 @@
     const uint32_t f = fB, M = MB;
     const unsigned long long mb = mbB;
     const uint32_t node0 = f << kFineLog;
-    const uint64_t wi = ((uint64_t)node0 >> 5) + tid;
+    const uint64_t wi0 = ((uint64_t)node0 >> 5) + tid;
     uint32_t knode0, c3order;
     node_key(w.tlog, w.tmask, w.key, (uint64_t)w.base + node0, K_ORDER, knode0, c3order);
     const uint32_t c3delay = (c3order & 0xFFFFFFu) | (K_DELAY << 24);
-    const bool in = wi < w.W * 2;
-    const uint32_t recv0 = p_in ? p_recv0 : 0u, crash0 = p_in ? p_crash0 : 0u, roll0 = p_in ? p_roll0 : 0u;
+    bool in[kW];
+    uint32_t recv0[kW], crash0[kW], rollw[kW];
+#pragma unroll
+    for (uint32_t j = 0; j < kW; ++j) {
+      in[j] = p_in[j];
+      recv0[j] = p_in[j] ? p_recv0[j] : 0u;
+      crash0[j] = p_in[j] ? p_crash0[j] : 0u;
+      const uint32_t roll0 = p_in[j] ? p_roll0[j] : 0u;
+      if (roll0) w.rollw[wi0 + j * B] = 0u;
+      rollw[j] = roll0 & ~crash0[j];
+    }
     const uint32_t fcv = tid < w.R ? p_fcv : 0u;
     if (i + 1 < nb) next_bucket(i + 1);
-    if (roll0) w.rollw[wi] = 0u;
-    const uint32_t rollw = roll0 & ~crash0;
-#pragma unroll
-    for (uint32_t k = 0; k < kBitTicks; ++k)
-      if (k < L) sm.b1[k][tid] = 0;
-    sm.cr0[tid] = make_uint2(crash0, rollw);
+#pragma unroll
+    for (uint32_t j = 0; j < kW; ++j) {
+#pragma unroll
+      for (uint32_t k = 0; k < kBitTicks; ++k)
+        if (k < L) sm.b1[k][tid + j * B] = 0;
+      sm.cr0[tid + j * B] = make_uint2(crash0[j], rollw[j]);
+    }
     if (tid < w.R) sm.fc[tid] = fcv;
     if (tid < kMaxWindow) sm.dead[tid] = 0;
     if (tid == 0) { sm.ndup = 0; sm.ninf = 0; sm.err = M >= (1u << 28) ? 3 : 0; sm.cls = M >= 1024 ? 1 : 0; }
@@ -288,7 +322,7 @@
       for (uint32_t p0 = 0, nbat = 0; p0 < (sm.err == 3 ? 0u : M); p0 += kBatch, ++nbat) {
         uint32_t mn[kU];
         if (p0 + kBatch < M) ld(gm, M, p0 + kBatch, mn);
-        GS_RESOLVE_BATCH(m, p0 + u * kResolveBlock + tid < M)
+        GS_RESOLVE_BATCH(m, p0 + u * B + tid < M)
 #pragma unroll
         for (uint32_t u = 0; u < kU; ++u) m[u] = mn[u];
       }
@@ -298,25 +332,39 @@
     stamp(w, sm, 2);
     __syncthreads();
     if (i + 1 < nb) prefetch(fB, MB, mbB);
-    if (tid == 0) w.rlcnt[f] = sm.err == 3 ? 0u : min(sm.ndup, kRolledCap);
+    const bool large = sm.err == 3;
+    if (tid == 0) {
+      w.rlcnt[f] = large ? 0u : min(sm.ndup, kRolledCap);
+      if (large) {
+        w.lglist[2 + atomicAdd(&w.lglist[0], 1u)] = f;
+        atomicAdd(&w.lglist[1], 1u);
+      }
+    }
     stamp(w, sm, 3);
-    uint32_t rw = recv0, cw = crash0;
-    if (sm.err != 3) {
+    uint32_t rw[kW];
+#pragma unroll
+    for (uint32_t j = 0; j < kW; ++j) rw[j] = recv0[j];
+    if (!large) {
       if (tid < L && sm.dead[tid]) atomicAdd(&sm.st[tid][0], sm.dead[tid]);
-      uint32_t infk[kBitTicks], ninf = 0;
-      const uint32_t plain = ~(crash0 | rollw);
+      uint32_t infk[kBitTicks][kW], ninf = 0;
+#pragma unroll
+      for (uint32_t j = 0; j < kW; ++j) {
+        const uint32_t plain = ~(crash0[j] | rollw[j]);
+#pragma unroll
+        for (uint32_t k = 0; k < kBitTicks; ++k) {
+          infk[k][j] = 0;
+          if (k >= L) continue;
+          const uint32_t infS = sm.b1[k][tid + j * B] & plain & ~rw[j];
+          rw[j] |= infS;
+          infk[k][j] = infS;
+        }
+      }
+      stamp(w, sm, 4);
 #pragma unroll
       for (uint32_t k = 0; k < kBitTicks; ++k) {
-        infk[k] = 0;
-        if (k >= L) continue;
-        const uint32_t infS = sm.b1[k][tid] & plain & ~rw;
-        rw |= infS;
-        infk[k] = infS;
-      }
-      stamp(w, sm, 4);
-#pragma unroll
-      for (uint32_t k = 0; k < kBitTicks; ++k) {
-        const uint32_t ni = __popc(infk[k]);
+        uint32_t ni = 0;
+#pragma unroll
+        for (uint32_t j = 0; j < kW; ++j) ni += __popc(infk[k][j]);
         acc_ni[k / 2] += ni << (16 * (k & 1));
         ninf += ni;
       }
@@ -331,61 +379,103 @@
         const uint32_t pos = atomicAdd(&sm.fc[slot], 1u);
         w.flist[((size_t)slot * w.nfine + f) * kFineNodes + pos] = (uint16_t)loc;
       };
-      uint32_t* inf = &sm.cnt[0];
-      {
-        uint32_t pre = 0, tot = 0;
-#pragma unroll
-        for (uint32_t b = 0; b < 9; ++b) {
-          const unsigned long long bal = __ballot((ninf >> b) & 1u);
-          pre += lanes_below(bal) << b;
-          tot += (uint32_t)__popcll(bal) << b;
-        }
-        uint32_t base = 0;
-        if (tot && lane_id() == 0) base = atomicAdd(&sm.ninf, tot);
-        uint32_t at = __builtin_amdgcn_readfirstlane(base) + pre;
+      uint32_t pre = 0, tot = 0;
+      static_assert(32 * kW < 128, "a node is informed once in a window: ninf in 7 bits");
+#pragma unroll
+      for (uint32_t b = 0; b < 7; ++b) {
+        const unsigned long long bal = __ballot((ninf >> b) & 1u);
+        pre += lanes_below(bal) << b;
+        tot += (uint32_t)__popcll(bal) << b;
+      }
+      uint32_t base = 0;
+      if (tot && lane_id() == 0) base = atomicAdd(&sm.ninf, tot);
+      const uint32_t at0 = __builtin_amdgcn_readfirstlane(base) + pre;
+#pragma unroll 1
+      for (uint32_t lo = 0;; lo += kInfCap) {
+        uint32_t at = at0 - lo;
 #pragma unroll
         for (uint32_t k = 0; k < kBitTicks; ++k)
-          for (uint32_t x = k < L ? infk[k] : 0u; x; x &= x - 1)
-            inf[at++] = (tid * 32 + __builtin_ctz(x)) | (k << kFineLog);
-      }
-      __syncthreads();
-      stamp(w, sm, 7);
-      const uint32_t ni_all = sm.ninf;
-      for (uint32_t q = tid; q < ni_all; q += kResolveBlock) bcast(inf[q]);
-    } else {
-      __syncthreads();
-      uint4* c4 = reinterpret_cast<uint4*>(sm.cnt);
-      for (uint32_t q = tid; q < kFineNodes / 4; q += kResolveBlock) c4[q] = make_uint4(0, 0, 0, 0);
-      sm.recv[tid] = recv0;
-      sm.crash[tid] = crash0;
-      sm.nrecv[tid] = 0;
-      sm.ncrash[tid] = 0;
-      __syncthreads();
-      for (uint32_t k = 0; k < L; ++k) resolve_tick(w, sm, f, gm, 0, M, k, t0 + k);
-      rw = sm.recv[tid] | sm.nrecv[tid];
-      cw = sm.crash[tid] | sm.ncrash[tid];
-      if (tid == 0 && sm.err == 1) atomicOr(w.err, kErrArrivals);
+#pragma unroll
+          for (uint32_t j = 0; j < kW; ++j)
+            for (uint32_t x = k < L ? infk[k][j] : 0u; x; x &= x - 1, ++at)
+              if (at < kInfCap) sm.inf[at] = ((tid + j * B) * 32 + __builtin_ctz(x)) | (k << kFineLog);
+        __syncthreads();
+        if (lo == 0) stamp(w, sm, 7);
+        const uint32_t ni_all = sm.ninf;
+        const uint32_t nr = min(ni_all - lo, kInfCap);
+        for (uint32_t q = tid; q < nr; q += B) bcast(sm.inf[q]);
+        if (lo + kInfCap >= ni_all) break;
+        __syncthreads();
+      }
     }
     __syncthreads();
     stamp(w, sm, 8);
+#pragma unroll
+    for (uint32_t j = 0; j < kW; ++j)
+      if (in[j] && rw[j] != recv0[j]) rwg[wi0 + j * B] = rw[j];
+    if (!large && tid < w.R) w.fcount[(size_t)tid * w.nfine + f] = sm.fc[tid];
+    stamp(w, sm, 9);
+    if (w.dbg && tid == 0) sm.stamp[sm.cls][0] += 1;
+    if (w.tstat) flush_counts(w, sm, acc_ni, L, (uint32_t)(((uint64_t)w.base + node0) >> w.tlog));
+  }
+  if (w.dbg && tid < 2 * kStampPhases) atomicAdd(&w.dbg[tid], (&sm.stamp[0][0])[tid]);
+  if (!w.tstat) flush_counts(w, sm, acc_ni, L, ~0u);
+}
+template <uint32_t B>
+__global__ __launch_bounds__(B, GS_RESOLVE_WAVES) void k_resolve(const WinState w, uint32_t t0, uint32_t L) {
+  resolve_body<B>(w, t0, L);
+}
+template <uint32_t B>
+__global__ __launch_bounds__(B, GS_RESOLVE_WAVES) void k_resolve_m(const WinState* __restrict__ ws, uint32_t L) {
+  resolve_body<B>(ws[blockIdx.y], 0u, L);
+}
+
+__device__ __forceinline__ void resolve_large_body(const WinState& w, uint32_t t0, uint32_t L) {
+  __shared__ LargeLds sm;
+  const uint32_t tid = threadIdx.x;
+  static_assert(kBitWords == kResolveBlock, "one bit word per thread");
+  static_assert(kWinMaxRing <= kResolveBlock && kMaxWindow * 4 <= kResolveBlock, "one ring slot, one counter per thread");
+  L = win_live(w, t0, L);
+  if (!L) return;
+  const uint32_t nl = w.lglist[0];
+  if (blockIdx.x >= nl) return;
+  if (tid < kMaxWindow * 4) (&sm.st[0][0])[tid] = 0;
+  uint32_t* rwg = (uint32_t*)w.recv;
+  uint32_t* cwg = (uint32_t*)w.crash;
+  for (uint32_t i = blockIdx.x; i < nl; i += gridDim.x) {
+    const uint32_t f = w.lglist[2 + i];
+    const uint32_t M = (uint32_t)w.ffill[f];
+    const uint32_t* gm = w.fmsg + w.fstart[f];
+    const uint64_t wi = ((uint64_t)(f << kFineLog) >> 5) + tid;
+    const bool in = wi < w.W * 2;
+    const uint32_t recv0 = in ? rwg[wi] : 0u, crash0 = in ? cwg[wi] : 0u;
+    uint4* c4 = reinterpret_cast<uint4*>(sm.cnt);
+    for (uint32_t q = tid; q < kFineNodes / 4; q += kResolveBlock) c4[q] = make_uint4(0, 0, 0, 0);
+    sm.recv[tid] = recv0;
+    sm.crash[tid] = crash0;
+    sm.nrecv[tid] = 0;
+    sm.ncrash[tid] = 0;
+    if (tid < w.R) sm.fc[tid] = w.fcount[(size_t)tid * w.nfine + f];
+    if (tid == 0) sm.err = 0;
+    __syncthreads();
+    for (uint32_t k = 0; k < L; ++k) resolve_tick(w, sm, f, gm, 0, M, k, t0 + k);
+    const uint32_t rw = sm.recv[tid] | sm.nrecv[tid], cw = sm.crash[tid] | sm.ncrash[tid];
+    if (tid == 0 && sm.err == 1) atomicOr(w.err, kErrArrivals);
     if (in) {
       if (rw != recv0) rwg[wi] = rw;
       if (cw != crash0) cwg[wi] = cw;
     }
     if (tid < w.R) w.fcount[(size_t)tid * w.nfine + f] = sm.fc[tid];
-    stamp(w, sm, 9);
-    if (w.dbg && tid == 0) sm.stamp[sm.cls][0] += 1;
-    if (w.tstat) flush_counts(w, sm, acc_ni, L, (uint32_t)(((uint64_t)w.base + node0) >> w.tlog));
-  }
-  if (w.dbg && tid < 2 * kStampPhases) atomicAdd(&w.dbg[tid], (&sm.stamp[0][0])[tid]);
-  if (!w.tstat) flush_counts(w, sm, acc_ni, L, ~0u);
-}
-__global__ __launch_bounds__(kResolveBlock, GS_RESOLVE_WAVES) void k_resolve(const WinState w, uint32_t t0, uint32_t L) {
-  resolve_body(w, t0, L);
-}
-__global__ __launch_bounds__(kResolveBlock, GS_RESOLVE_WAVES) void k_resolve_m(const WinState* __restrict__ ws,
-                                                                                uint32_t L) {
-  resolve_body(ws[blockIdx.y], 0u, L);
+    if (w.tstat) flush_st(w, sm.st, L, (uint32_t)(((uint64_t)w.base + (f << kFineLog)) >> w.tlog));
+    __syncthreads();
+  }
+  if (!w.tstat) flush_st(w, sm.st, L, ~0u);
+}
+__global__ __launch_bounds__(kResolveBlock) void k_resolve_large(const WinState w, uint32_t t0, uint32_t L) {
+  resolve_large_body(w, t0, L);
+}
+__global__ __launch_bounds__(kResolveBlock) void k_resolve_large_m(const WinState* __restrict__ ws, uint32_t L) {
+  resolve_large_body(ws[blockIdx.y], 0u, L);
 }
 
 template <uint32_t E, bool ROLLED>
@@ -574,15 +664,26 @@
 
 }
 
+static uint32_t resolve_block() {
+  static const uint32_t b = [] {
+    const char* e = getenv("GS_RESOLVE_BLOCK");
+    const int v = e ? atoi(e) : 0;
+    return v == 256 || v == 512 ? (uint32_t)v : kResolveBlockDefault;
+  }();
+  return b;
+}
+
 hipError_t win_resolve(const WinState& w, uint32_t t0, uint32_t L, hipStream_t s) {
-  const uint32_t cus = device_cus();
+  const uint32_t cus = device_cus(), B = resolve_block();
   static const uint32_t per_cu = [] { const char* e = getenv("GS_RESOLVE_PER_CU"); return e ? (uint32_t)std::max(atoi(e), 1) : 2u; }();
-  uint32_t G = std::min<uint32_t>(w.nfine, per_cu * cus);
+  uint32_t G = std::min<uint32_t>(w.nfine, per_cu * (kResolveBlock / B) * cus);
   G = std::max<uint32_t>(G, (w.nfine + kResolveMaxBuckets - 1) / kResolveMaxBuckets);
   const uint32_t gs = (w.nfine + kSmallBlock / 64 - 1) / (kSmallBlock / 64);
   hipLaunchKernelGGL(k_resolve_small<false>, dim3(gs), dim3(kSmallBlock), 0, s, w, t0, L);
   static_assert(kSmallMax == 64 * 4, "the two bodies cover 1..kSmallMax");
-  hipLaunchKernelGGL(k_resolve, dim3(G), dim3(kResolveBlock), 0, s, w, t0, L);
+  if (B == 256) hipLaunchKernelGGL(k_resolve<256>, dim3(G), dim3(256), 0, s, w, t0, L);
+  else hipLaunchKernelGGL(k_resolve<512>, dim3(G), dim3(512), 0, s, w, t0, L);
+  hipLaunchKernelGGL(k_resolve_large, dim3(kLargeGrid), dim3(kResolveBlock), 0, s, w, t0, L);
   hipLaunchKernelGGL(k_resolve_small<true>, dim3((w.nfine + kRolledBlock / 64 - 1) / (kRolledBlock / 64)),
                      dim3(kRolledBlock), 0, s, w, t0, L);
   return hipGetLastError();
@@ -590,11 +691,14 @@
 
 hipError_t win_resolve_g(const WinGroup& g, uint32_t L, hipStream_t s) {
   const uint32_t cus = device_cus();
-  uint32_t G = std::min<uint32_t>(g.nfine_max, (2 * cus + g.M - 1) / g.M);
+  const uint32_t B = resolve_block();
+  uint32_t G = std::min<uint32_t>(g.nfine_max, (2 * (kResolveBlock / B) * cus + g.M - 1) / g.M);
   G = std::max<uint32_t>(G, (g.nfine_max + kResolveMaxBuckets - 1) / kResolveMaxBuckets);
   const uint32_t gs = (g.nfine_max + kSmallBlock / 64 - 1) / (kSmallBlock / 64);
   hipLaunchKernelGGL(k_resolve_small_m<false>, dim3(gs, g.M), dim3(kSmallBlock), 0, s, g.wr, L);
-  hipLaunchKernelGGL(k_resolve_m, dim3(G, g.M), dim3(kResolveBlock), 0, s, g.wr, L);
+  if (B == 256) hipLaunchKernelGGL(k_resolve_m<256>, dim3(G, g.M), dim3(256), 0, s, g.wr, L);
+  else hipLaunchKernelGGL(k_resolve_m<512>, dim3(G, g.M), dim3(512), 0, s, g.wr, L);
+  hipLaunchKernelGGL(k_resolve_large_m, dim3(kLargeGrid, g.M), dim3(kResolveBlock), 0, s, g.wr, L);
   hipLaunchKernelGGL(k_resolve_small_m<true>, dim3((g.nfine_max + kRolledBlock / 64 - 1) / (kRolledBlock / 64), g.M),
                      dim3(kRolledBlock), 0, s, g.wr, L);
   return hipGetLastError();
diff --git a/gossip_simulator_amd/csrc/gs_win_units.hip b/gossip_simulator_amd/csrc/gs_win_units.hip
--- a/gossip_simulator_amd/csrc/gs_win_units.hip
+++ b/gossip_simulator_amd/csrc/gs_win_units.hip
@@ -64,6 +64,7 @@
   if (threadIdx.x < L && s_t[threadIdx.x]) atomicAdd(&w.tfires[threadIdx.x], (unsigned long long)s_t[threadIdx.x]);
   for (uint32_t i = tid; i < kRegions; i += nth) { w.chist[i] = 0; w.cfill[i] = 0; }
   for (uint32_t i = tid; i < w.nfine; i += nth) w.ffill[i] = 0;
+  if (tid == 0) w.lglist[0] = 0;
   if (w.dd && tid == 0) {
     w.cfill[kRegions] = 0;
     w.cfill[kRegions + 1] = w.ctl->fmsg_cap;
diff --git a/include/gossip.h b/include/gossip.h
--- a/include/gossip.h
+++ b/include/gossip.h
@@ -98,6 +98,7 @@
   uint64_t alloc_cache_hits;
   uint64_t cached_bytes;
   uint64_t coarse_redos;
+  uint64_t resolve_large_buckets;
 } gs_timing;
 
 enum { GS_RUN_COVERED = 0, GS_RUN_QUIESCENT = 1, GS_RUN_MAX_TICKS = 2, GS_RUN_RUNNING = -1 };
```

Result: no change. 85.03 billion msgs/s, median of 2 (-0.2%).
